# flybirdxx/ComfyUI-SDMatte

Hardware: AMD Instinct MI355X
Metric: alpha mattes/sec at 1024x1024 (higher is better)
Workload: dtype f16x3

## Files before the change

### comfyui-sdmatte_amd/csrc/k_attn.h

```cpp
#pragma once
#include "sdm_common.h"
#include "k_gemm.h"

struct AttnParams {
  const half_t* q; long q_bs; int ldq;
  const half_t* k; long k_bs; int ldk;
  const half_t* vt; long vt_bs; long vt_hs; int ldvt;
  const float* bias; long bias_bs;
  half_t* o; long o_bs; int ldo;
  int o_f32;
  int o_p3; long o_xl_off;
  long q_lo, k_lo, vt_lo;
  int Lq, Lk;
  float scale_log2e;
  const int* tiles; int tiles_bs;
  int nsplit; long part_stride; float* part_ml;
  int batch, heads, nq_blocks, q_chunks;
  int pp_flags;
  int ablate;
};

#define SDM_NEG_BIG (-1.0e30f)
#define SDM_ATTN_SKIP_MARGIN 2000.0f

SDM_DEV_INLINE void attn_store_p3(const AttnParams& p, const unsigned char* stf, int ps, int b, int q0, int head, int lane) {
  unsigned char* base = (unsigned char*)p.o;
#pragma unroll
  for (int pass = 0; pass < 4; ++pass) {
    const int row = (pass >> 1) * 16 + (lane & 15), cch = (pass & 1) * 32 + (lane >> 4) * 8;
    const f32x4 a = *(const f32x4*)(stf + row * ps + cch * 4), c = *(const f32x4*)(stf + row * ps + cch * 4 + 16);
    const float y[8] = {a[0], a[1], a[2], a[3], c[0], c[1], c[2], c[3]};
    if (q0 + row < p.Lq) p3_store8(y, base, base + p.o_xl_off, (size_t)b * p.Lq + q0 + row, p.ldo, head * 64 + cch);
  }
}

#define ATTN64_PK 144
#define ATTN64_PV 136
#define ATTN64_BUF (64 * ATTN64_PK + 64 * ATTN64_PV + 256)
#define ATTN64_SMEM (2 * ATTN64_BUF)
#define ATTN64P_BUF (2 * 64 * ATTN64_PK + 2 * 64 * ATTN64_PV + 256)
#define ATTN64P_SMEM (2 * ATTN64P_BUF)

SDM_DEV_INLINE bool attn_block_coords(const AttnParams& p, int bid, int& b, int& head, int& qblk) {
  const int units = p.batch * p.heads * p.q_chunks;
  const int upx = units / 8;
  const int qb = (p.nq_blocks + p.q_chunks - 1) / p.q_chunks;
  const int xcd = bid & 7, s = bid >> 3;
  const int unit = xcd * upx + s / qb;
  const int bh = unit / p.q_chunks, chunk = unit % p.q_chunks;
  qblk = chunk * qb + s % qb;
  b = bh / p.heads; head = bh % p.heads;
  return qblk < p.nq_blocks;
}

SDM_DEV_INLINE void attn_split_range(const AttnParams& p, const int* tl, int ntiles, int nwalk_all, int sp, int& i0, int& nwalk) {
  i0 = 0; nwalk = nwalk_all;
  if (p.nsplit <= 1) return;
  const int per = (ntiles + p.nsplit - 1) / p.nsplit, t0 = sp * per, t1 = (t0 + per < ntiles) ? t0 + per : ntiles;
  if (!tl) { i0 = t0 < ntiles ? t0 : ntiles; nwalk = t1 > i0 ? t1 - i0 : 0; return; }
// ... 40 lines not shown
  i32x8 q8p[2];
#pragma unroll
  for (int qt = 0; qt < QT; ++qt) {
    int qrow = q0 + qt * 32 + l31;
    if (qrow > p.Lq - 1) qrow = p.Lq - 1;
    const half_t* qp = p.q + (size_t)b * p.q_bs + (size_t)qrow * p.ldq + head * 64 + hi * 8;
#pragma unroll
    for (int ks = 0; ks < 4; ++ks) qf[qt][ks] = *(const f16x8*)(qp + ks * 16);
    if (PREC && !F8Q) {
#pragma unroll
      for (int ks = 0; ks < 4; ++ks) qfl[PREC ? qt : 0][ks] = *(const f16x8*)(qp + p.q_lo + ks * 16);
    }
    if (F8Q) {
      const half_t* qb = p.q + (size_t)b * p.q_bs + p.q_lo + (size_t)qrow * p.ldq + head * 64 + hi * 16;
#pragma unroll
      for (int m = 0; m < 2; ++m) {
        const i32x4 r0 = *(const i32x4*)(qb + m * 32), r1 = *(const i32x4*)(qb + m * 32 + 8);
        q8p[m] = i32x8{r0[1], r0[0], r0[3], r0[2], r1[1], r1[0], r1[3], r1[2]};
      }
    }
    if (p.scale_log2e != 1.0f && !F8Q) {
#pragma unroll
      for (int ks = 0; ks < 4; ++ks)
#pragma unroll
        for (int j = 0; j < 8; ++j) {
          if (PREC) {
            const float qs = ((float)qf[qt][ks][j] + (float)qfl[PREC ? qt : 0][ks][j]) * p.scale_log2e;
            const half_t h = (half_t)qs;
            qf[qt][ks][j] = h;
            qfl[PREC ? qt : 0][ks][j] = (half_t)(qs - (float)h);
          } else {
            qf[qt][ks][j] = (half_t)((float)qf[qt][ks][j] * p.scale_log2e);
          }
        }
    }
  }
  f32x16 o[QT][2], ls[QT];
  float m_i[QT];
  float lsum = 0.0f;
#pragma unroll
  for (int qt = 0; qt < QT; ++qt) {
    m_i[qt] = SDM_NEG_BIG;
#pragma unroll
    for (int r = 0; r < 16; ++r) ls[qt][r] = 0.0f;
#pragma unroll
    for (int dt = 0; dt < 2; ++dt)
#pragma unroll
      for (int r = 0; r < 16; ++r) o[qt][dt][r] = 0.0f;
  }
  f16x8 ones;
#pragma unroll
  for (int j = 0; j < 8; ++j) ones[j] = (half_t)1.0f;

  const half_t* kbase = p.k + (size_t)b * p.k_bs + head * 64;
  const half_t* vbase = p.vt + (size_t)b * p.vt_bs + (size_t)head * p.vt_hs;
  const float* bbase = p.bias ? p.bias + (size_t)b * p.bias_bs : nullptr;
  const int ntiles = (p.Lk + 63) / 64;

  struct Raw {
    f16x8 k[VPT], v[VPT], kl[PREC ? VPT : 1], vl[PVS ? VPT : 1];
    float b;
    bool in;
  };
  constexpr bool AHEAD2 = F8Q && QT == 1 && NW == 8;
  Raw ra, rb;
  ra.b = 0.0f; ra.in = true; rb.b = 0.0f; rb.in = true;
  const float* bsrc = bbase ? bbase : (const float*)(p.k + (size_t)b * p.k_bs);
  auto prefetch = [&](int t, Raw& r) {
    const int k0 = t * 64;
#pragma unroll
    for (int i = 0; i < VPT; ++i) {
      const int v = tid + i * NTH;
      const int row = v >> 3, part = v & 7;
      int kr = k0 + row;
      if (kr > p.Lk - 1) kr = p.Lk - 1;
      r.k[i] = *(const f16x8*)(kbase + (size_t)kr * p.ldk + part * 8);
      r.v[i] = *(const f16x8*)(vbase + (size_t)row * p.ldvt + k0 + part * 8);
      if (PREC) r.kl[PREC ? i : 0] = *(const f16x8*)(kbase + p.k_lo + (size_t)kr * p.ldk + part * 8);
      if (PVS) r.vl[PVS ? i : 0] = *(const f16x8*)(vbase + p.vt_lo + (size_t)row * p.ldvt + k0 + part * 8);
    }
    int kb = k0 + (tid & 63);
    r.in = kb < p.Lk;
    if (!r.in) kb = p.Lk - 1;
    r.b = bsrc[kb];
  };
  auto stage = [&](int buf, const Raw& r) {
    unsigned char* base = smem + buf * BUF;
#pragma unroll
    for (int i = 0; i < VPT; ++i) {
      const int v = tid + i * NTH;
      const int row = v >> 3, part = v & 7;
      *(f16x8*)(base + row * PK + part * 16) = r.k[i];
      f16x4 lo, hi4;
#pragma unroll
      for (int e = 0; e < 4; ++e) { lo[e] = r.v[i][e]; hi4[e] = r.v[i][4 + e]; }
      *(f16x4*)(base + VOFF + row * PV + part * 16) = lo;
      *(f16x4*)(base + VOFF + row * PV + part * 16 + 8) = hi4;
      if (PREC) *(f16x8*)(base + KLO + row * PK + part * 16) = r.kl[PREC ? i : 0];
      if (PVS) {
#pragma unroll
        for (int e = 0; e < 4; ++e) { lo[e] = r.vl[PVS ? i : 0][e]; hi4[e] = r.vl[PVS ? i : 0][4 + e]; }
        *(f16x4*)(base + VOFF + VLO + row * PV + part * 16) = lo;
        *(f16x4*)(base + VOFF + VLO + row * PV + part * 16 + 8) = hi4;
      }
    }
    if (tid < 64) ((float*)(base + BOFF))[tid] = r.in ? (bbase ? r.b : 0.0f) : SDM_NEG_BIG;
  };
// ... 241 lines not shown
    for (int pass = 0; pass < 4; ++pass) {
      const int row = pass * 8 + (lane >> 3), part = lane & 7;
      const int qg = q0 + qt * 32 + row;
      if (qg < p.Lq)
        *(f16x8*)(p.o + (size_t)b * p.o_bs + (size_t)qg * p.ldo + head * 64 + part * 8) = *(const f16x8*)(stg + row * PK + part * 16);
    }
    SDM_WAVE_SYNC();
  }
}

#define ATTN64PIPE_SMEM (3 * ATTN64P_BUF)
#define ATTN64PIPE4_KB (2 * 64 * ATTN64_PK + 256)
#define ATTN64PIPE4_VB (64 * ATTN64_PV)
#define ATTN64PIPE4_SMEM (2 * ATTN64PIPE4_KB + 3 * ATTN64PIPE4_VB)
template <int NW>
__global__ void __launch_bounds__(64 * NW, 2) attn_d64_pipe_kernel(AttnParams p) {
  constexpr int NTH = 64 * NW, VPT = 512 / NTH;
  constexpr bool SPLITBUF = NW == 4;
  SDM_DYN_SMEM(smem);
  constexpr int PK = ATTN64_PK, PV = ATTN64_PV, BUF = ATTN64P_BUF;
  constexpr int KLO = 64 * PK, VOFF = 2 * 64 * PK, BOFF = VOFF + 64 * PV;
  auto k_of = [&](int b3, int b2) { return SPLITBUF ? smem + b2 * ATTN64PIPE4_KB : smem + b3 * BUF; };
  auto v_of = [&](int b3) { return SPLITBUF ? smem + 2 * ATTN64PIPE4_KB + b3 * ATTN64PIPE4_VB : smem + b3 * BUF + VOFF; };
  auto bias_of = [&](int b3, int b2) { return (float*)(SPLITBUF ? smem + b2 * ATTN64PIPE4_KB + 2 * 64 * PK : smem + b3 * BUF + BOFF); };
  const int tid = threadIdx.x, lane = tid & 63, wave = tid >> 6;
  const int hi = lane >> 5, l31 = lane & 31;
  int b, head, qblk;
  if (!attn_block_coords(p, blockIdx.x, b, head, qblk)) return;
  const int q0 = qblk * (32 * NW) + wave * 32;

  f16x8 qf[4];
  i32x8 q8p[2];
  {
    int qrow = q0 + l31;
    if (qrow > p.Lq - 1) qrow = p.Lq - 1;
    const half_t* qp = p.q + (size_t)b * p.q_bs + (size_t)qrow * p.ldq + head * 64 + hi * 8;
#pragma unroll
    for (int ks = 0; ks < 4; ++ks) qf[ks] = *(const f16x8*)(qp + ks * 16);
    const half_t* qb = p.q + (size_t)b * p.q_bs + p.q_lo + (size_t)qrow * p.ldq + head * 64 + hi * 16;
#pragma unroll
    for (int m = 0; m < 2; ++m) {
      const i32x4 r0 = *(const i32x4*)(qb + m * 32), r1 = *(const i32x4*)(qb + m * 32 + 8);
      q8p[m] = i32x8{r0[1], r0[0], r0[3], r0[2], r1[1], r1[0], r1[3], r1[2]};
    }
  }
  f32x16 o[2], ls;
  float m_i = SDM_NEG_BIG;
#pragma unroll
  for (int r = 0; r < 16; ++r) { ls[r] = 0.0f; o[0][r] = 0.0f; o[1][r] = 0.0f; }
  f16x8 ones;
#pragma unroll
  for (int j = 0; j < 8; ++j) ones[j] = (half_t)1.0f;

  const half_t* kbase = p.k + (size_t)b * p.k_bs + head * 64;
  const half_t* vbase = p.vt + (size_t)b * p.vt_bs + (size_t)head * p.vt_hs;
  const float* bbase = p.bias ? p.bias + (size_t)b * p.bias_bs : nullptr;
  const float* bsrc = bbase ? bbase : (const float*)(p.k + (size_t)b * p.k_bs);
  const int ntiles = (p.Lk + 63) / 64;
  const int* tl = p.tiles ? p.tiles + (size_t)b * p.tiles_bs : nullptr;
  const int sp = p.nsplit > 1 ? (int)blockIdx.y : 0;
  int i0, nwalk;
  attn_split_range(p, tl, ntiles, tl ? tl[0] : ntiles, sp, i0, nwalk);
  if (nwalk <= 0) { attn_write_empty_part(p, sp, b, head, q0, lane); return; }
  auto tile_at = [&](int i) { return tl ? tl[1 + i0 + i] : i0 + i; };

  f16x8 rk[VPT], rkl[VPT], rv[VPT];
  float rb = 0.0f;
  bool rin = true;
  auto prefetch = [&](int t) {
    const int k0 = t * 64;
#pragma unroll
    for (int i = 0; i < VPT; ++i) {
      const int v = tid + i * NTH, srow = v >> 3, spart = v & 7;
      int kr = k0 + srow;
      if (kr > p.Lk - 1) kr = p.Lk - 1;
      rk[i] = *(const f16x8*)(kbase + (size_t)kr * p.ldk + spart * 8);
      rv[i] = *(const f16x8*)(vbase + (size_t)srow * p.ldvt + k0 + spart * 8);
      rkl[i] = *(const f16x8*)(kbase + p.k_lo + (size_t)kr * p.ldk + spart * 8);
    }
    int kb = k0 + (tid & 63);
    rin = kb < p.Lk;
    if (!rin) kb = p.Lk - 1;
    rb = bsrc[kb];
  };
  auto stage = [&](int b3, int b2) {
    unsigned char* kb_ = k_of(b3, b2);
    unsigned char* vb_ = v_of(b3);
#pragma unroll
    for (int i = 0; i < VPT; ++i) {
      const int v = tid + i * NTH, srow = v >> 3, spart = v & 7;
      *(f16x8*)(kb_ + srow * PK + spart * 16) = rk[i];
      f16x4 lo, hi4;
#pragma unroll
      for (int e = 0; e < 4; ++e) { lo[e] = rv[i][e]; hi4[e] = rv[i][4 + e]; }
      *(f16x4*)(vb_ + srow * PV + spart * 16) = lo;
      *(f16x4*)(vb_ + srow * PV + spart * 16 + 8) = hi4;
      *(f16x8*)(kb_ + KLO + srow * PK + spart * 16) = rkl[i];
    }
    if (tid < 64) bias_of(b3, b2)[tid] = rin ? (bbase ? rb : 0.0f) : SDM_NEG_BIG;
  };
  auto qk = [&](int b3, int b2, f32x16 (&s)[2]) {
    const unsigned char* Ks = k_of(b3, b2);
    const float* Bs = bias_of(b3, b2);
#pragma unroll
    for (int kt = 0; kt < 2; ++kt)
#pragma unroll
      for (int g = 0; g < 4; ++g) {
// ... 99 lines not shown
#pragma unroll
      for (int e = 0; e < 4; ++e) h[e] = o[dt][4 * g + e] * inv;
      *(f32x4*)(stf + l31 * PS + (dt * 32 + 8 * g + 4 * hi) * 4) = h;
    }
  SDM_WAVE_SYNC();
  if (p.o_p3 && p.nsplit <= 1) { attn_store_p3(p, stf, PS, b, q0, head, lane); return; }
#pragma unroll
  for (int pass = 0; pass < 8; ++pass) {
    const int row = pass * 4 + (lane >> 4), part = lane & 15;
    const int qg = q0 + row;
    if (qg < p.Lq)
      *(f32x4*)(obase + (size_t)qg * p.ldo + head * 64 + part * 4) = *(const f32x4*)(stf + row * PS + part * 16);
  }
}

#define ATTN64PP_SLOT (3 * 8192 + 256)
#define ATTN64PP_SMEM (6 * ATTN64PP_SLOT)
template <int ABL = 0, int BIAS = 1, int LIST = 1, int KE = 0, int DS = 1, int OB = 1>
__global__ void __launch_bounds__(512, 2) attn_d64_pp_kernel(AttnParams p) {
  SDM_DYN_SMEM(smem);
  constexpr int SLOT = ATTN64PP_SLOT, KLO = 8192, VOFF = 16384, BOFF = 24576;
  constexpr int R = KE < 0 ? 4 : 6, D = KE < 0 ? 3 : 4;
  constexpr int NDMA = BIAS ? 4 : 3;
  const int tid = threadIdx.x, lane = tid & 63, wave = SDM_UNIFORM_I(tid >> 6);
  const int grp = wave >> 2;
  const int hi = lane >> 5, l31 = lane & 31;
  int b, head, qblk;
  if (!attn_block_coords(p, blockIdx.x, b, head, qblk)) return;
  const int q0 = qblk * 256 + wave * 32;

  f16x8 qf[4];
  i32x8 q8p[2];
  {
    int qrow = q0 + l31;
    if (qrow > p.Lq - 1) qrow = p.Lq - 1;
    const half_t* qp = p.q + (size_t)b * p.q_bs + (size_t)qrow * p.ldq + head * 64 + hi * 8;
#pragma unroll
    for (int ks = 0; ks < 4; ++ks) qf[ks] = *(const f16x8*)(qp + ks * 16);
    const half_t* qb = p.q + (size_t)b * p.q_bs + p.q_lo + (size_t)qrow * p.ldq + head * 64 + hi * 16;
#pragma unroll
    for (int m = 0; m < 2; ++m) {
      const i32x4 r0 = *(const i32x4*)(qb + m * 32), r1 = *(const i32x4*)(qb + m * 32 + 8);
      q8p[m] = i32x8{r0[1], r0[0], r0[3], r0[2], r1[1], r1[0], r1[3], r1[2]};
    }
  }
  f32x16 o[2], ls;
  float m_i = SDM_NEG_BIG;
#pragma unroll
  for (int r = 0; r < 16; ++r) { ls[r] = 0.0f; o[0][r] = 0.0f; o[1][r] = 0.0f; }
  f16x8 ones;
#pragma unroll
  for (int j = 0; j < 8; ++j) ones[j] = (half_t)1.0f;

  const half_t* kbase = p.k + (size_t)b * p.k_bs + head * 64;
  const half_t* vbase = p.vt + (size_t)b * p.vt_bs + (size_t)head * p.vt_hs;
  const int ntiles = p.Lk / 64;
  const int* tl = (LIST && p.tiles) ? p.tiles + (size_t)b * p.tiles_bs : nullptr;
  const int sp = p.nsplit > 1 ? (int)blockIdx.y : 0;
  int i0, nwalk;
  attn_split_range(p, tl, ntiles, tl ? tl[0] : ntiles, sp, i0, nwalk);
  if (nwalk <= 0) { attn_write_empty_part(p, sp, b, head, q0, lane); return; }
  const int* tlp = tl ? tl + 1 + i0 : nullptr;
  auto tile_at = [&](int i) { if (i > nwalk - 1) i = nwalk - 1; return LIST ? tlp[i] : i0 + i; };

  const sdm_rsrc rsK = sdm_make_rsrc(kbase, (unsigned int)(((size_t)(p.Lk - 1) * p.ldk + 64) * 2));
  const sdm_rsrc rsK8 = sdm_make_rsrc(kbase + p.k_lo, (unsigned int)(((size_t)(p.Lk - 1) * p.ldk + 64) * 2));
  const sdm_rsrc rsV = sdm_make_rsrc(vbase, (unsigned int)(((size_t)63 * p.ldvt + p.Lk) * 2));
  const sdm_rsrc rsB = sdm_make_rsrc(BIAS ? p.bias + (size_t)b * p.bias_bs : (const float*)kbase, (unsigned int)p.Lk * 4u);
  const int rho = 8 * wave + (lane >> 3), cpos = lane & 7;
  const int csrc = cpos ^ ((rho >> 1) & 7);
  const int rr = rho & 31;
  const int pir = (rr & 0x13) | (((rr >> 2) & 1) << 3) | (((rr >> 3) & 1) << 2);
  const unsigned int voffK = (unsigned int)(((rho & 32) + pir) * p.ldk * 2 + csrc * 16);
  const unsigned int voffV = (unsigned int)(rho * p.ldvt * 2 + csrc * 16);
  const int lr = lane & 31;
  const unsigned int voffB = (unsigned int)(((lane & 32) + ((lr & 0x13) | (((lr >> 2) & 1) << 3) | (((lr >> 3) & 1) << 2))) * 4);
  auto dma = [&](int tile, int slot, int from = 0, int to = 4) {
    if (ABL & 8) return;
    unsigned char* sb = smem + slot * SLOT + wave * 1024;
    const unsigned int k0 = (unsigned int)tile * 64u;
    int i = 0;
    if (i >= from && i < to) sdm_glds16_buf(rsV, voffV, k0 * 2u, sb + VOFF);
    ++i;
    if (BIAS) { if (i >= from && i < to) sdm_glds4_buf(rsB, voffB, k0 * 4u, smem + slot * SLOT + BOFF); ++i; }
    if (i >= from && i < to) sdm_glds16_buf(rsK8, voffK, k0 * (unsigned int)(p.ldk * 2), sb + KLO);
    ++i;
    if (i >= from && i < to) sdm_glds16_buf(rsK, voffK, k0 * (unsigned int)(p.ldk * 2), sb);
  };
  const int kxor = (l31 >> 1) & 7;
  const int kx = l31 * 128 + ((hi ^ kxor) << 4);
  const int k8x = l31 * 128 + (((2 * hi) ^ kxor) << 4);
  const int vx = l31 * 128 + ((hi ^ kxor) << 4);
  struct KFrag { f16x8 h[4]; i32x8 f8[2]; };
  auto load_bias = [&](int slot, f32x16 (&s)[2]) {
    if (!BIAS) {
#pragma unroll
      for (int kt = 0; kt < 2; ++kt)
#pragma unroll
        for (int r = 0; r < 16; ++r) s[kt][r] = 0.0f;
      return;
    }
    if (ABL & 32) return;
    const float* Bs = (const float*)(smem + slot * SLOT + BOFF);
#pragma unroll
    for (int kt = 0; kt < 2; ++kt)
#pragma unroll
      for (int g = 0; g < 4; ++g) {
// ... 554 lines not shown
```

### comfyui-sdmatte_amd/csrc/k_misc.h

```cpp
#pragma once
#include "sdm_common.h"

template <typename F>
SDM_DEV_INLINE float resize_aa_sample(F fetch, int in_h, int in_w, int out_h, int out_w, int oy, int ox) {
  const float sy = (float)in_h / (float)out_h, sx = (float)in_w / (float)out_w;
  const float supy = sy >= 1.0f ? sy : 1.0f, supx = sx >= 1.0f ? sx : 1.0f;
  const float invy = sy >= 1.0f ? 1.0f / sy : 1.0f, invx = sx >= 1.0f ? 1.0f / sx : 1.0f;
  const float cy = sy * ((float)oy + 0.5f), cx = sx * ((float)ox + 0.5f);
  int ymin = (int)(cy - supy + 0.5f); if (ymin < 0) ymin = 0;
  int ymax = (int)(cy + supy + 0.5f); if (ymax > in_h) ymax = in_h;
  int xmin = (int)(cx - supx + 0.5f); if (xmin < 0) xmin = 0;
  int xmax = (int)(cx + supx + 0.5f); if (xmax > in_w) xmax = in_w;
  float wys = 0.0f, wxs = 0.0f;
  for (int y = ymin; y < ymax; ++y) { float w = 1.0f - fabsf(((float)y - cy + 0.5f) * invy); wys += w > 0.0f ? w : 0.0f; }
  for (int x = xmin; x < xmax; ++x) { float w = 1.0f - fabsf(((float)x - cx + 0.5f) * invx); wxs += w > 0.0f ? w : 0.0f; }
  float acc = 0.0f;
  for (int y = ymin; y < ymax; ++y) {
    float wy = 1.0f - fabsf(((float)y - cy + 0.5f) * invy); wy = wy > 0.0f ? wy / wys : 0.0f;
    float row = 0.0f;
    for (int x = xmin; x < xmax; ++x) {
      float wx = 1.0f - fabsf(((float)x - cx + 0.5f) * invx); wx = wx > 0.0f ? wx / wxs : 0.0f;
      row += wx * fetch(y, x);
    }
    acc += wy * row;
// ... 65 lines not shown
  const int j = i % wk, ii = (i / wk) % hk, b = i / ((long)hk * wk);
  const float t = plane[((size_t)b * SH + (size_t)8 * s * ii) * SW + 8 * s * j];
  const float m = (t + 1.0f) / 2.0f;
  bias[i] = ((1.0f - m) * mask_value) * mult;
}

__global__ void alpha_out_kernel(const float* __restrict__ dec, float* __restrict__ alpha, long npix) {
  const long i = (long)blockIdx.x * blockDim.x + threadIdx.x;
  if (i >= npix) return;
  const f32x4 d = *(const f32x4*)(dec + (size_t)i * 4);
  float m = (d[0] + d[1] + d[2]) / 3.0f;
  m = fminf(fmaxf(m, -1.0f), 1.0f);
  alpha[i] = (m + 1.0f) / 2.0f;
}

__global__ void resize_planes_kernel(const float* __restrict__ in, float* __restrict__ out, int P, int Hin, int Win, int Hout,
                                     int Wout, int clamp01) {
  const long i = (long)blockIdx.x * blockDim.x + threadIdx.x;
  if (i >= (long)P * Hout * Wout) return;
  const int ox = i % Wout, oy = (i / Wout) % Hout, b = i / ((long)Hout * Wout);
  const float* pl = in + (size_t)b * Hin * Win;
  float x;
  if (Hin == Hout && Win == Wout) x = pl[(size_t)oy * Win + ox];
  else x = resize_aa_sample([&](int y, int xx) { return pl[(size_t)y * Win + xx]; }, Hin, Win, Hout, Wout, oy, ox);
  if (clamp01) x = fminf(fmaxf(x, 0.0f), 1.0f);
  out[i] = x;
}

__global__ void refine_compose_kernel(const float* __restrict__ img, const float* __restrict__ tri, float* __restrict__ alpha,
                                      float* __restrict__ matted, long npix, int mode, int refine, float c, float one_minus_c) {
  const long i = (long)blockIdx.x * blockDim.x + threadIdx.x;
  if (i >= npix) return;
  float a = alpha[i];
  const float t = (refine || mode == 2) ? tri[i] : 0.0f;
  if (refine) {
    const bool fg = t > c, bg = t < one_minus_c, unk = !(fg || bg);
    if (bg) a = 0.0f;
    if (fg) a = fminf(fmaxf(a * 1.2f, 0.0f), 1.0f);
    if (a < 0.3f && unk) a = 0.0f;
    alpha[i] = a;
  }
  const float r = img[i * 3 + 0], g = img[i * 3 + 1], b = img[i * 3 + 2];
  if (mode == 1) {
    f32x4 o = {r, g, b, a};
    *(f32x4*)(matted + i * 4) = o;
  } else if (mode == 2) {
    const float gate = (t > 0.2f && a > 0.1f) ? 1.0f : 0.0f;
    matted[i * 3 + 0] = r * gate; matted[i * 3 + 1] = g * gate; matted[i * 3 + 2] = b * gate;
  } else {
    matted[i * 3 + 0] = 0.0f; matted[i * 3 + 1] = 0.0f; matted[i * 3 + 2] = 0.0f;
  }
}

__global__ void split_planes_kernel(const float* __restrict__ x, half_t* __restrict__ hi, half_t* __restrict__ lo, long n, float mult, int mode) {
  const long i4 = ((long)blockIdx.x * blockDim.x + threadIdx.x) * 4;
  if (i4 >= n) return;
  f16x4 oh, ol;
  float xx[4], xl[4];
#pragma unroll
  for (int e = 0; e < 4; ++e) {
    float y = (i4 + e < n) ? x[i4 + e] * mult : 0.0f;
    if (mode == 3) y = fminf(fmaxf(y, -57344.0f), 57344.0f);
    oh[e] = (half_t)y;
    ol[e] = (half_t)(y - (float)oh[e]);
    xx[e] = y; xl[e] = (y - (float)oh[e]) * 2048.0f;
  }
  *(f16x4*)(hi + i4) = oh;
  if (mode == 3) {
    int a = SDM_CVT_PK_BF8(xx[0], xx[1], 0, false), b = SDM_CVT_PK_BF8(xl[0], xl[1], 0, false);
    a = SDM_CVT_PK_BF8(xx[2], xx[3], a, true); b = SDM_CVT_PK_BF8(xl[2], xl[3], b, true);
    u32x2 pr;
    pr[0] = (unsigned int)a; pr[1] = (unsigned int)b;
    *(u32x2*)(lo + i4) = pr;
  } else {
    *(f16x4*)(lo + i4) = ol;
  }
}

__global__ void scale_copy_kernel(const float* __restrict__ in, float* __restrict__ out, long n, float mult) {
  const long i = (long)blockIdx.x * blockDim.x + threadIdx.x;
  if (i < n) out[i] = in[i] * mult;
}

__global__ void fill_random_f16_kernel(half_t* __restrict__ p, long n, unsigned int seed, float amp) {
  for (long i = (long)blockIdx.x * blockDim.x + threadIdx.x; i < n; i += (long)gridDim.x * blockDim.x) {
    unsigned int h = (unsigned int)i * 2654435761u + seed;
    h ^= h >> 15; h *= 2246822519u; h ^= h >> 13; h *= 3266489917u; h ^= h >> 16;
    p[i] = (half_t)(((float)(h & 0xFFFF) * (1.0f / 32768.0f) - 1.0f) * amp);
  }
}
__global__ void fill_random_f32_kernel(float* __restrict__ p, long n, unsigned int seed, float amp) {
  for (long i = (long)blockIdx.x * blockDim.x + threadIdx.x; i < n; i += (long)gridDim.x * blockDim.x) {
    unsigned int h = (unsigned int)i * 2654435761u + seed;
    h ^= h >> 15; h *= 2246822519u; h ^= h >> 13; h *= 3266489917u; h ^= h >> 16;
    p[i] = ((float)(h & 0xFFFF) * (1.0f / 32768.0f) - 1.0f) * amp;
  }
}

#define SDM_CMASK_EMPTY 0xFFFFFFFFu

__global__ __launch_bounds__(256) void cmask_table_kernel(const float* __restrict__ plane, unsigned int* __restrict__ table, int n0, int H, int W) {
  SDM_SHARED unsigned int tb[4];
  const int b = blockIdx.x, tid = threadIdx.x;
  if (tid < 4) tb[tid] = SDM_CMASK_EMPTY;
  __syncthreads();
  const float* pl = plane + (size_t)b * H * W;
  for (int i = tid; i < 64 * 64; i += 256) {
    const int y = (int)(((long)(i >> 6) * H) >> 6), x = (int)(((long)(i & 63) * W) >> 6);
    const unsigned int bits = __builtin_bit_cast(unsigned int, pl[(size_t)y * W + x]);
    for (int k = 0; k < 4; ++k) {
      unsigned int cur = tb[k];
      if (cur == SDM_CMASK_EMPTY) cur = atomicCAS(&tb[k], SDM_CMASK_EMPTY, bits);
      if (cur == SDM_CMASK_EMPTY || cur == bits) break;
    }
  }
  __syncthreads();
  if (tid < 4) table[(size_t)(n0 + b) * 4 + tid] = tb[tid];
}

__global__ void cmask_init_kernel(const float* __restrict__ plane, unsigned char* __restrict__ mask, const unsigned int* __restrict__ table, int n0, int B, long HW) {
  const long i = (long)blockIdx.x * blockDim.x + threadIdx.x;
  if (i >= (long)B * HW) return;
  const int b = (int)(i / HW);
  const unsigned int bits = __builtin_bit_cast(unsigned int, plane[i]);
  const unsigned int* tb = table + (size_t)(n0 + b) * 4;
  int cls = 0;
#pragma unroll
  for (int k = 3; k >= 0; --k)
// ... 61 lines not shown
```

### comfyui-sdmatte_amd/csrc/sdm_engine.cpp

```cpp
#include "sdm_common.h"
#include "k_conv.h"
#include "k_gemm.h"
#include "k_norm.h"
#include "k_attn.h"
#include "k_misc.h"
#include "k_trimap.h"
#include "k_cclabel.h"
#include "k_foreground.h"
#include "k_guided.h"
#include "k_roi.h"
#include "k_canvas.h"
#include "k_boxes.h"
#include "../../include/sdmatte.h"

#include <algorithm>
#include <cmath>
#include <cstdio>
#include <cstdlib>
#include <cstring>
#include <atomic>
#include <map>
#include <mutex>
#include <shared_mutex>
#include <string>
#include <unordered_map>
#include <vector>

#ifdef SDM_EMU
#include <chrono>
static int dev_malloc(void** p, size_t n) { *p = aligned_alloc(256, ((n + 255) / 256) * 256 + 256); return *p ? 0 : -1; }
static void dev_free(void* p) { free(p); }
static int dev_memcpy_h2d(void* d, const void* s, size_t n, void*) { memcpy(d, s, n); return 0; }
static int dev_memcpy_d2h(void* d, const void* s, size_t n, void*) { memcpy(d, s, n); return 0; }
static int dev_memcpy_d2d(void* d, const void* s, size_t n, void*) { memcpy(d, s, n); return 0; }
static int dev_memset(void* d, int v, size_t n, void*) { memset(d, v, n); return 0; }
static int dev_sync(void*) { return 0; }
static const char* dev_errstr(int) { return "emu"; }
#define SDM_SET_SMEM(kernel, bytes) ((void)0)
#else
static int dev_malloc(void** p, size_t n) { return (int)hipMalloc(p, n); }
static void dev_free(void* p) { (void)hipFree(p); }
static int dev_memcpy_h2d(void* d, const void* s, size_t n, void* st) { return (int)hipMemcpyAsync(d, s, n, hipMemcpyHostToDevice, (hipStream_t)st); }
static int dev_memcpy_d2h(void* d, const void* s, size_t n, void* st) { return (int)hipMemcpyAsync(d, s, n, hipMemcpyDeviceToHost, (hipStream_t)st); }
static int dev_memcpy_d2d(void* d, const void* s, size_t n, void* st) { return (int)hipMemcpyAsync(d, s, n, hipMemcpyDeviceToDevice, (hipStream_t)st); }
static int dev_memset(void* d, int v, size_t n, void* st) { return (int)hipMemsetAsync(d, v, n, (hipStream_t)st); }
static int dev_sync(void* st) { return (int)hipStreamSynchronize((hipStream_t)st); }
static const char* dev_errstr(int e) { return hipGetErrorString((hipError_t)e); }
#define SDM_SET_SMEM(kernel, bytes)                                                                              \
  do {                                                                                                           \
    if ((bytes) > 48 * 1024) {                                                                                   \
      static std::atomic<unsigned long long> done_{0ull};                                                        \
      int dev_ = 0;                                                                                              \
      (void)hipGetDevice(&dev_);                                                                                 \
      const unsigned long long bit_ = 1ull << (dev_ & 63);                                                       \
      if (!(done_.load(std::memory_order_relaxed) & bit_)) {                                                     \
        const hipError_t r_ = hipFuncSetAttribute((const void*)(kernel), hipFuncAttributeMaxDynamicSharedMemorySize, (int)(bytes)); \
        if (r_ != hipSuccess) fprintf(stderr, "[sdmatte] hipFuncSetAttribute(%d bytes of LDS) failed: %s\n", (int)(bytes), hipGetErrorString(r_)); \
        else done_.fetch_or(bit_, std::memory_order_relaxed);                                                    \
      }                                                                                                          \
    }                                                                                                            \
  } while (0)
#endif

static inline int rup(int a, int b) { return ((a + b - 1) / b) * b; }
#ifdef SDM_EMU
static inline void dev_use(int) {}
#else
static inline void dev_use(int device) {
  const hipError_t r = hipSetDevice(device);
  if (r != hipSuccess) fprintf(stderr, "[sdmatte] hipSetDevice(%d) failed: %s\n", device, hipGetErrorString(r));
}
#endif
static inline size_t rupz(size_t a, size_t b) { return ((a + b - 1) / b) * b; }

struct OptEntry { const char* name; int value; int def; const char* what; };
static OptEntry g_opts[] = {
  {"conv_f8", 1, 1, "residual terms of the wide split-precision 3x3 convs on fp8 MFMAs (read when a model is built)"},
  {"gemm_f8", 1, 1, "the same for Linear / 1x1 layers with K >= gemm_f8_min_k (read when a model is built)"},
  {"gemm_f8_min_k", 1024, 1024, "smallest K of a GEMM that takes the 8-wave fp8-residual kernel"},
  {"gemm_p3", 1, 1, "transformer-block Linear layers on the plane-fed GEMM (k_gemm.h): pre-split operand planes from LayerNorm / GroupNorm / attention / GEGLU, LDS-DMA only (the W3 weight copies are built when a model is built)"},
  {"gemm_p3_tile", 0, 0, "row tile of the plane-fed GEMM: 0 by shape, 256 / 128 / 64 forced"},
  {"gemm_p3_attn", 1, 1, "d=64 attention cores write the operand planes of to_out themselves (0: fp32 result + one conversion pass)"},
  {"gemm_p3_persist", 1, 1, "plane-fed GEMM: persistent blocks that prefetch the next tile's first chunk underneath the epilogue (0: one block per tile, n > 1: a grid of n blocks - tests)"},
  {"gemm_p3_ablate", 0, 0, "bench only: 1 no MFMAs, 2 no DMAs behind the prologue, 4 no epilogue (sdm_bench_gemm_p3)"},
  {"conv_up_phase", 1, 1, "up-sampling 3x3 convs (Upsample2D) as four 2x2-tap phase convs on the plane-fed GEMM (k_gemm.h, UP): 0 off (the 3x3 kernels on the up-sampled image), 1 the launches with at least two 256-row tiles per CU (up_phase_wins: measured), 2 every eligible launch (tests).  0 / non-0 is read when a model is built: the phase matrices are a derived weight layout"},
  {"conv_epi", 4, 4, "F8 kernels' epilogue: 4 register-direct stores + residual as accumulator init, 3 residual init only, 0 LDS-staged"},
  {"conv_xtile", 1, 1, "F8 3x3: cross-tile prefetch by the producer waves"},
  {"conv_f8_tpb", 0, 0, "F8: tiles per block (0 = by queue depth)"},
  {"conv_dma", 1, 1, "3x3 stride-1 256x128 tile: weights by LDS-DMA"},
  {"conv_dma_all", 0, 0, "keep a stage-ordered weight copy for every wide 3x3 layer, not only the split-precision ones (read when a model is built)"},
  {"conv_pc", -1, -1, "producer / consumer form of the split-precision DMA kernel: -1 by channel count, 0 off, 1 on"},
  {"conv_pc_min_cin", 256, 256, "conv_pc = -1: smallest Cin that takes the producer / consumer form"},
  {"conv_db", 0, 0, "512x128 double-buffered tile where the queue is deep"},
  {"trimap_skip", 1, 1, "VAE encoder, trimap images: output tiles inside a constant region of the trimap are not multiplied (k_misc.h cmask_*; exact). 0 = every tile"},
  {"conv_band_rows", 0, 0, "tile rows per XCD band of the convs that leave constant tiles out (0 = by image height)"},
  {"trimap_skip_min_rows", 512, 512, "smallest output height at which constant tiles are left out (measured at 1024^2: the 1024- and 512-row levels gain 3.7 + 1.6 ms, the 256-row level loses 0.7: too few of its 32 x 128-pixel tiles lie inside one region)"},
  {"conv_splitk", -1, -1, "split-K of the register-staged conv / GEMM kernels: -1 by shape (few tiles, long K), 0 off, n >= 2 forced where the shape allows"},
  {"force_cfg0", 0, 0, "always the 256x128 tile for 3x3 stride 1 (tests: fused GroupNorm at tiny sizes)"},
  {"no_gn_fuse", 0, 0, "never fuse the GroupNorm apply into the consuming conv"},
  {"split_lds_pad", 0, 0, "extra dynamic LDS of the register-staged split kernels (forces one block per CU)"},
  {"attn_f8", 1, 1, "Q.K^T residual terms of the d=64 split-precision attention on fp8 MFMAs"},
  {"attn_dense", 0, 0, "walk every key tile of the trimap-biased self-attention"},
  {"attn_pv_split", 0, 0, "residual terms of P.V too (fully split attention; tests)"},
  {"attn_nw", 0, 0, "waves per d=64 attention block: 0 by launch size, 4, 8"},
  {"attn_pipe", 1, 1, "8-wave split-precision d=64 attention: two-tile software pipeline"},
  {"attn_pipe4", 1, 1, "the same pipeline for the 4-wave launches (two K / three V^T buffers)"},
  {"attn_pp", 1, 1, "split-precision d=64 attention with fp32 output as a ping-pong of the block's wave halves (attn_d64_pp_kernel, 256 query rows per block): 0 off, 1 on, 2 on without the static priority of the younger half, 3 on with per-segment priority flips"},
  {"attn_pp_min_blocks", 128, 128, "attn_pp: launches with fewer 256-row blocks than this keep the 4-wave pipelines (0 in tests: the ping-pong kernel at any size)"},
  {"attn_ksplit", 0, 0, "key split of the d=64 split-precision attention: 0 by launch size (blocks that do not fill the chip's block slots a whole number of times), 1 off, 2 / 4 forced, 3 forced on the ping-pong kernel (ignored elsewhere: those launches run unsplit)"},
  {"precise_mask", -1, -1, "stages in split precision (-1 = the config's own mask; per-stage attribution experiments; read at sdm_create)"},
#ifdef SDM_EMU
  {"emu_arena_extra", 0, 0, "emulator build only, self-test of the arena check: the launch pass of a stand-alone op allocates one block its sizing pass did not"},
#endif
};
static OptEntry* opt_find(const char* name) {
  for (auto& o : g_opts) if (name && strcmp(o.name, name) == 0) return &o;
  return nullptr;
}
static int opt(const char* name) { OptEntry* o = opt_find(name); return o ? o->value : 0; }
static std::shared_mutex g_opt_mu;
struct OptReadLock { std::shared_lock<std::shared_mutex> l; OptReadLock() : l(g_opt_mu) {} };
static std::mutex g_count_mu;
static std::map<std::string, long> g_kernel_counts;
static void count_kernel(const char* name) { std::lock_guard<std::mutex> g(g_count_mu); g_kernel_counts[name] += 1; }

template <int NTAPS, int STRIDE, int TH, int TW, int BN, int KC, int WM, int WN, int DB = 0, int GNOK = 0>
static void launch_conv_t(const ConvParams& p_in, void* stream) {
  using C = ConvCfg<NTAPS, STRIDE, TH, TW, BN, KC, WM, WN, DB>;
  ConvParams p = p_in;
  p.tiles_m = (NTAPS == 9) ? sdm_cdiv(p.Wout, TW) * sdm_cdiv(p.Hout, TH)
                           : (int)(((p.rows_per_img ? (long)p.rows_per_img : p.M) + C::BM - 1) / C::BM);
  p.tiles_n = sdm_cdiv(p.Cout_pad, BN);
  const long total_m = (long)p.tiles_m * ((NTAPS == 9 || p.rows_per_img) ? p.N : 1);
  p.xcd_chunk = (int)((total_m + 7) / 8);
  const dim3 grid((unsigned)(8L * p.xcd_chunk * p.tiles_n), (unsigned)(p.ksplit > 1 ? p.ksplit : 1), 1);
  const size_t gn_extra = (size_t)(p.C0 + p.C1) * 8;
  if constexpr (!DB) {
    if (p.w_lo) {
      using CS = ConvCfg<NTAPS, STRIDE, TH, TW, BN, KC, WM, WN, 0, 1>;
      const size_t lds_pad = (size_t)opt("split_lds_pad");
      if (GNOK && p.gn_scale) {
        auto k = conv_mfma_kernel<NTAPS, STRIDE, TH, TW, BN, KC, WM, WN, 1, 0, GNOK, 1>;
        SDM_SET_SMEM(k, 160 * 1024);
        SDM_LAUNCH(k, grid, dim3(CS::NTHREADS), (size_t)CS::SMEM + gn_extra + lds_pad, stream, p);
      } else {
        auto k = conv_mfma_kernel<NTAPS, STRIDE, TH, TW, BN, KC, WM, WN, 1, 0, 0, 1>;
        SDM_SET_SMEM(k, 160 * 1024);
        SDM_LAUNCH(k, grid, dim3(CS::NTHREADS), CS::SMEM + lds_pad, stream, p);
      }
      return;
    }
  }
  if (GNOK && p.gn_scale) {
    const size_t smem = (size_t)C::SMEM + gn_extra;
    if (p.in_f32) {
      auto k = conv_mfma_kernel<NTAPS, STRIDE, TH, TW, BN, KC, WM, WN, 1, DB, GNOK>;
      SDM_SET_SMEM(k, C::SMEM + 1024 * 8);
      SDM_LAUNCH(k, grid, dim3(C::NTHREADS), smem, stream, p);
    } else {
      auto k = conv_mfma_kernel<NTAPS, STRIDE, TH, TW, BN, KC, WM, WN, 0, DB, GNOK>;
      SDM_SET_SMEM(k, C::SMEM + 1024 * 8);
      SDM_LAUNCH(k, grid, dim3(C::NTHREADS), smem, stream, p);
// ... 316 lines not shown
  int up = 0;
  size_t wup_off = 0, wup_bytes = 0;
  unsigned char* wup = nullptr;
  int up_exp = 8;
  size_t w_bytes() const { return (size_t)Cin_pad * ntaps * Cout_pad * 2; }
  size_t b_bytes() const { return (size_t)Cout_pad * 4; }
};
static const int kSplitWeightExp = 8;

static ConvL make_layer(const std::string& name, int ntaps, int I, int O, int geglu, int split) {
  ConvL L;
  L.name = name; L.ntaps = ntaps; L.I = I; L.O = O; L.geglu = geglu;
  L.Cin_pad = rup(I, 16);
  L.Cout_pad = rup(O, geglu ? 64 : 32);
  L.split = split ? 1 : 0;
  L.w_exp = split ? kSplitWeightExp : 0;
  return L;
}

static bool layer_takes_dma3x3(const ConvL& L) { return L.ntaps == 9 && L.Cout_pad >= 128 && !L.geglu; }
static bool layer_takes_gemm_f8(const ConvL& L) {
  return L.ntaps == 1 && L.split && L.Cout_pad >= 128 && L.Cin_pad % 32 == 0 && conv_f8_enabled() && gemm_f8_enabled();
}
static bool layer_takes_w3(const ConvL& L) { return L.ntaps == 1 && L.split && L.Cin_pad % 32 == 0 && L.Cin_pad >= 32; }
static bool layer_takes_up_phase(const ConvL& L) {
  return L.ntaps == 9 && L.split && !L.geglu && L.Cin_pad % 32 == 0 && L.Cin_pad >= 32 && conv_f8_enabled() && opt("conv_up_phase") != 0;
}
static bool up_phase_wins(int N, int H, int W, int Cout_pad) {
  if (opt("conv_up_phase") >= 2) return true;
  const long tiles = (long)N * sdm_cdiv((H + 2) * (W + 2), 256) * 4 * sdm_cdiv(Cout_pad, 128);
  return tiles >= 2L * device_cus();
}
static void layer_choose_layouts(ConvL& L, bool want_dma3x3, bool want_gemm_f8, bool want_w3, bool want_up_phase = false) {
  if (want_up_phase && layer_takes_up_phase(L)) L.wup_bytes = (size_t)16 * L.Cin_pad * L.Cout_pad * 4;
  if (want_dma3x3 && layer_takes_dma3x3(L)) {
    L.wdma_bytes = L.w_bytes() * (L.split ? 2 : 1);
    L.f8 = (L.split && L.Cin_pad % 32 == 0 && conv_f8_enabled()) ? 1 : 0;
  }
  if (want_gemm_f8 && layer_takes_gemm_f8(L)) { L.wdma_bytes = L.w_bytes() * 2; L.f8 = 1; }
  if (want_w3 && layer_takes_w3(L)) L.w3_bytes = L.w_bytes() * 2;
}
struct NormL {
  int C = 0;
  size_t g_off = 0, b_off = 0;
  float* g = nullptr;
  float* b = nullptr;
};
enum SlotKind { SLOT_CONV_W, SLOT_CONV_B, SLOT_NORM_G, SLOT_NORM_B, SLOT_HOST };
struct Slot {
  int kind = 0, layer = -1, co_off = 0, ci_off = 0;
  float w_scale = 1.0f;
  std::vector<int64_t> shape;
  size_t host_off = 0;
  bool loaded = false;
};
struct ResB { int norm1 = -1, conv1 = -1, norm2 = -1, conv2 = -1, sc = -1, temb = -1, cin = 0, cout = 0; };
struct VaeAttnB { int gn = -1, qkv = -1, out = -1, C = 0; };
struct TfB { int gn, proj_in, ln1, qkv1, o1, ln2, q2, kv2, o2, ln3, ff1, ff2, proj_out, C, heads; size_t k_hoff, v_hoff; };
struct TembL { size_t w_hoff = 0, b_hoff = 0, cb_hoff = 0; int cout = 0, cout_pad = 0; float* table = nullptr; };

struct T {
  size_t off = 0, bytes = 0;
  void* p = nullptr;
  int N = 0, H = 0, W = 0, C = 0, f32 = 0;
  bool want_stats = false;
  float* stats = nullptr;
  int srows = 0;
  size_t soff = 0, sbytes = 0;
  unsigned char* cmask = nullptr;
  size_t cm_off = 0, cm_bytes = 0;
  int cm_n0 = 0;
  long rows() const { return (long)N * H * W; }
};

static const int kFmtP3 = 4;
static inline size_t fmt_bytes(int f) { return f == kFmtP3 ? 3 : (f ? 4 : 2); }
static const int kMinVariantRows = 8;
struct Variant {
  int trans = 0, kind = 0;
  std::vector<float> c;
  bool operator==(const Variant& o) const { return trans == o.trans && kind == o.kind && c == o.c; }
};

struct ProfRec { std::string name, desc; double flops, bytes;
#ifndef SDM_EMU
  hipEvent_t e0, e1;
#endif
};

struct sdm_ctx {
  sdm_config cfg;
  int device = 0;
  const unsigned char* dbg_cmask = nullptr;
  void* stream = nullptr;
  bool own_stream = false;
  std::string err;
  std::vector<ConvL> convs;
  std::vector<NormL> norms;
  std::unordered_map<std::string, Slot> slots;
  std::vector<std::string> slot_order;
  unsigned char* warena = nullptr;
  size_t warena_bytes = 0, canon_bytes = 0;
  std::vector<float> hostblob;
  int64_t n_loaded = 0, n_ignored = 0;
  std::vector<std::string> missing;
  bool finalized = false;
  void* stage = nullptr;
  size_t stage_bytes = 0;
  struct LoadSlot {
    void* host = nullptr; void* dev = nullptr; size_t cap = 0; bool busy = false;
#ifndef SDM_EMU
// ... 51 lines not shown

#define SDM_FAIL(ctx, code, ...)                       \
  do {                                                 \
    char buf_[512];                                    \
    snprintf(buf_, sizeof(buf_), __VA_ARGS__);         \
    (ctx)->err = buf_;                                 \
    return (code);                                     \
  } while (0)

#define SDM_CHECK_DEV(ctx, expr)                                                              \
  do {                                                                                        \
    int e_ = (expr);                                                                          \
    if (e_ != 0) SDM_FAIL(ctx, SDM_ERR_HIP, "%s failed: %s (%s:%d)", #expr, dev_errstr(e_), __FILE__, __LINE__); \
  } while (0)

#define TRY(x) do { int rc_ = (x); if (rc_) return rc_; } while (0)

struct Builder {
  sdm_ctx* e;
  size_t woff = 0;
  size_t doff = 0;
  int stage = 0;
  explicit Builder(sdm_ctx* c) : e(c) {}
  int conv(const std::string& name, int ntaps, int I_pad16_src, int O, int geglu = 0, int up = 0) {
    ConvL L = make_layer(name, ntaps, I_pad16_src, O, geglu, e->cfg.precise_mask & stage);
    L.stage = stage; L.up = up;
    L.w_off = woff; woff += rupz(L.w_bytes(), 256);
    L.b_off = woff; woff += rupz(L.b_bytes(), 256);
    if (L.split) { L.wlo_off = woff; woff += rupz(L.w_bytes(), 256); }
    layer_choose_layouts(L, L.split || opt("conv_dma_all") != 0, L.Cin_pad >= gemm_f8_min_k(), conv_f8_enabled() && opt("gemm_p3") != 0, up != 0);
    if (L.wdma_bytes) { L.wdma_off = doff; doff += rupz(L.wdma_bytes, 256); }
    if (L.w3_bytes) { L.w3_off = doff; doff += rupz(L.w3_bytes, 256); }
    if (L.wup_bytes) { L.wup_off = doff; doff += rupz(L.wup_bytes, 256); }
    e->convs.push_back(L);
    return (int)e->convs.size() - 1;
  }
  int norm(int C) {
    NormL n; n.C = C;
    n.g_off = woff; woff += rupz((size_t)C * 4, 256);
    n.b_off = woff; woff += rupz((size_t)C * 4, 256);
    e->norms.push_back(n);
    return (int)e->norms.size() - 1;
  }
  void slot(const std::string& key, int kind, int layer, std::vector<int64_t> shape, int co_off = 0, int ci_off = 0) {
    Slot s; s.kind = kind; s.layer = layer; s.co_off = co_off; s.ci_off = ci_off; s.shape = std::move(shape);
    if (kind == SLOT_HOST) {
      size_t n = 1; for (auto d : s.shape) n *= (size_t)d;
      s.host_off = e->hostblob.size();
      e->hostblob.resize(e->hostblob.size() + n, 0.0f);
    }
    e->slots[key] = s;
    e->slot_order.push_back(key);
  }
  int conv_named(const std::string& p, int ntaps, int I, int O, bool bias = true, int ci_off = 0, int Ipad = 0, int up = 0) {
    int id = conv(p, ntaps, Ipad ? Ipad : I, O, 0, up);
    if (ntaps == 9) slot(p + ".weight", SLOT_CONV_W, id, {O, I, 3, 3}, 0, ci_off);
    else slot(p + ".weight", SLOT_CONV_W, id, {O, I}, 0, ci_off);
    if (bias) slot(p + ".bias", SLOT_CONV_B, id, {O});
    return id;
  }
  int norm_named(const std::string& p, int C) {
    int id = norm(C);
    slot(p + ".weight", SLOT_NORM_G, id, {C});
    slot(p + ".bias", SLOT_NORM_B, id, {C});
    return id;
  }
  ResB resnet(const std::string& p, int cin, int cout, int temb_dim) {
    ResB r; r.cin = cin; r.cout = cout;
    r.norm1 = norm_named(p + ".norm1", cin);
    if (temb_dim > 0) {
      r.conv1 = conv(p + ".conv1", 9, cin, cout);
      slot(p + ".conv1.weight", SLOT_CONV_W, r.conv1, {cout, cin, 3, 3});
      TembL t; t.cout = cout; t.cout_pad = e->convs[r.conv1].Cout_pad;
      slot(p + ".conv1.bias", SLOT_HOST, -1, {cout}); t.cb_hoff = e->slots[p + ".conv1.bias"].host_off;
      slot(p + ".time_emb_proj.weight", SLOT_HOST, -1, {cout, temb_dim}); t.w_hoff = e->slots[p + ".time_emb_proj.weight"].host_off;
      slot(p + ".time_emb_proj.bias", SLOT_HOST, -1, {cout}); t.b_hoff = e->slots[p + ".time_emb_proj.bias"].host_off;
      e->tembs.push_back(t);
      r.temb = (int)e->tembs.size() - 1;
    } else {
      r.conv1 = conv_named(p + ".conv1", 9, cin, cout);
    }
    r.norm2 = norm_named(p + ".norm2", cout);
    r.conv2 = conv_named(p + ".conv2", 9, cout, cout);
    if (cin != cout) r.sc = conv_named(p + ".conv_shortcut", 1, cin, cout);
    return r;
  }
  VaeAttnB vae_attn(const std::string& p, int C) {
    const int outer = stage;
    stage = SDM_PRECISE_VAE_ATTN_LIN;
    struct Restore { int& s; int v; ~Restore() { s = v; } } restore{stage, outer};
    VaeAttnB a; a.C = C;
    a.gn = norm_named(p + ".group_norm", C);
    a.qkv = conv(p + ".qkv", 1, C, 3 * C);
    const char* nm[3] = {"to_q", "to_k", "to_v"};
    for (int i = 0; i < 3; ++i) {
      slot(p + "." + nm[i] + ".weight", SLOT_CONV_W, a.qkv, {C, C}, i * C);
      slot(p + "." + nm[i] + ".bias", SLOT_CONV_B, a.qkv, {C}, i * C);
    }
    a.out = conv_named(p + ".to_out.0", 1, C, C);
    return a;
  }
  TfB transformer(const std::string& p, int C, int heads, int ctx) {
    const int outer = stage;
    stage = SDM_PRECISE_UNET_TF;
    struct Restore { int& s; int v; ~Restore() { s = v; } } restore{stage, outer};
    TfB t; t.C = C; t.heads = heads;
    t.gn = norm_named(p + ".norm", C);
    t.proj_in = conv_named(p + ".proj_in", 1, C, C);
    const std::string b = p + ".transformer_blocks.0";
    t.ln1 = norm_named(b + ".norm1", C);
    t.ln2 = norm_named(b + ".norm2", C);
    t.ln3 = norm_named(b + ".norm3", C);
    t.qkv1 = conv(b + ".attn1.qkv", 1, C, 3 * C);
    slot(b + ".attn1.to_q.weight", SLOT_CONV_W, t.qkv1, {C, C}, 0);
    slot(b + ".attn1.to_k.weight", SLOT_CONV_W, t.qkv1, {C, C}, C);
    slot(b + ".attn1.to_v.weight", SLOT_CONV_W, t.qkv1, {C, C}, 2 * C);
    t.o1 = conv_named(b + ".attn1.to_out.0", 1, C, C);
    t.q2 = conv_named(b + ".attn2.to_q", 1, C, C, false);
    e->slots[b + ".attn1.to_q.weight"].w_scale = e->slots[b + ".attn2.to_q.weight"].w_scale = 0.125f * SDM_LOG2E;
    t.kv2 = conv(b + ".attn2.kv_folded", 9, 16, 2 * C);
    slot(b + ".attn2.to_k.weight", SLOT_HOST, -1, {C, ctx}); t.k_hoff = e->slots[b + ".attn2.to_k.weight"].host_off;
    slot(b + ".attn2.to_v.weight", SLOT_HOST, -1, {C, ctx}); t.v_hoff = e->slots[b + ".attn2.to_v.weight"].host_off;
    t.o2 = conv_named(b + ".attn2.to_out.0", 1, C, C);
    t.ff1 = conv(b + ".ff.net.0.proj", 1, C, 8 * C, 1);
    slot(b + ".ff.net.0.proj.weight", SLOT_CONV_W, t.ff1, {8 * C, C});
    slot(b + ".ff.net.0.proj.bias", SLOT_CONV_B, t.ff1, {8 * C});
    t.ff2 = conv_named(b + ".ff.net.2", 1, 4 * C, C);
    t.proj_out = conv_named(p + ".proj_out", 1, C, C);
    return t;
  }
};

static std::string S(int i) { return std::to_string(i); }

static void build_model(sdm_ctx* e) {
  Builder B(e);
  const sdm_config& c = e->cfg;
  const int* vc = c.vae_channels;
  const int lc = 4;
  B.stage = SDM_PRECISE_VAE_ENC;
  e->enc_conv_in = B.conv_named("vae.encoder.conv_in", 9, 3, vc[0]);
  int cprev = vc[0];
  e->enc_res.resize(4);
  for (int i = 0; i < 4; ++i) {
    for (int j = 0; j < c.vae_layers_per_block; ++j)
      e->enc_res[i].push_back(B.resnet("vae.encoder.down_blocks." + S(i) + ".resnets." + S(j), j == 0 ? cprev : vc[i], vc[i], 0));
    cprev = vc[i];
    if (i < 3) e->enc_down.push_back(B.conv_named("vae.encoder.down_blocks." + S(i) + ".downsamplers.0.conv", 9, vc[i], vc[i]));
  }
  const int cm = vc[3];
  e->enc_mid0 = B.resnet("vae.encoder.mid_block.resnets.0", cm, cm, 0);
  e->enc_attn = B.vae_attn("vae.encoder.mid_block.attentions.0", cm);
  e->enc_mid1 = B.resnet("vae.encoder.mid_block.resnets.1", cm, cm, 0);
  e->enc_norm_out = B.norm_named("vae.encoder.conv_norm_out", cm);
  e->enc_conv_out = B.conv_named("vae.encoder.conv_out", 9, cm, 2 * lc);
  e->quant = B.conv_named("vae.quant_conv", 1, 2 * lc, 2 * lc);
  B.stage = SDM_PRECISE_VAE_DEC;
  e->post_quant = B.conv_named("vae.post_quant_conv", 1, lc, lc);
  e->dec_conv_in = B.conv_named("vae.decoder.conv_in", 9, lc, cm);
  e->dec_mid0 = B.resnet("vae.decoder.mid_block.resnets.0", cm, cm, 0);
  e->dec_attn = B.vae_attn("vae.decoder.mid_block.attentions.0", cm);
  e->dec_mid1 = B.resnet("vae.decoder.mid_block.resnets.1", cm, cm, 0);
  e->dec_res.resize(4);
  cprev = vc[3];
  for (int i = 0; i < 4; ++i) {
    const int co = vc[3 - i];
    for (int j = 0; j < c.vae_layers_per_block + 1; ++j)
      e->dec_res[i].push_back(B.resnet("vae.decoder.up_blocks." + S(i) + ".resnets." + S(j), j == 0 ? cprev : co, co, 0));
    cprev = co;
    if (i < 3) e->dec_up.push_back(B.conv_named("vae.decoder.up_blocks." + S(i) + ".upsamplers.0.conv", 9, co, co, true, 0, 0, 1));
  }
  e->dec_norm_out = B.norm_named("vae.decoder.conv_norm_out", vc[0]);
  e->dec_conv_out = B.conv_named("vae.decoder.conv_out", 9, vc[0], 3);
  B.stage = SDM_PRECISE_UNET_RES;
  const int* uc = c.unet_channels;
  const int te = uc[0] * 4, ctx = c.cross_attention_dim;
// ... 316 lines not shown
    const int pc_opt = opt("conv_pc"), pc_min_cin = opt("conv_pc_min_cin");
    if (p.w_dma && L.split) p.pc = pc_opt >= 0 ? (pc_opt == 1) : (L.Cin_pad >= pc_min_cin);
    if (p.w_dma && L.f8) {
      if (p.C1 > 0 && (p.C0 % 32)) { p.w_dma = nullptr; p.pc = 0; }
      else p.f8 = 1;
    }
    if (L.ntaps == 1 && L.f8 && L.w_dma && cfg == 4 && p.in_f32 && gemm_f8_enabled()) { p.w_dma = L.w_dma; p.f8 = 1; }
    if (p.f8) { p.f8_sa = 127 - 11; p.f8_sb = 127 - L.f8_exp; p.acc_scale = 1.0f; }
  }
  int ksplit = 1;
  if (!p.w_dma && !L.geglu && p.out_f32 <= 1 && (L.ntaps == 9 || p.M == (long)p.N * p.Hout * p.Wout)) ksplit = conv_pick_ksplit(L.ntaps, a.stride, cfg, p);
  T ws; ws.bytes = 0;
  const int sk_bpi = sdm_cdiv(p.Hout * p.Wout, kSplitKRows);
  if (ksplit > 1 && (size_t)ksplit * p.M * p.Cout_pad >= (1ull << 31)) ksplit = 1;
  if (a.out->want_stats) {
    if (L.geglu || a.out_ch_off || p.out_f32 >= 2) SDM_FAIL(e, SDM_ERR_INVALID, "conv %s: fused statistics unsupported with this epilogue", L.name.c_str());
    const ConvCfgInfo& ci = conv_cfg_table(L.ntaps, a.stride)[cfg];
    const long tiles = (L.ntaps == 9) ? (long)sdm_cdiv(p.Hout, ci.TH) * sdm_cdiv(p.Wout, ci.TW)
                                      : ((long)p.Hout * p.Wout + ci.TH * ci.TW - 1) / (ci.TH * ci.TW);
    a.out->srows = ksplit > 1 ? sk_bpi : (int)(tiles * ci.WM);
    T sb = talloc(e, 1, 1, 1, (int)((size_t)p.N * a.out->srows * a.out->C * 2), 1);
    a.out->soff = sb.off; a.out->sbytes = sb.bytes; a.out->stats = (float*)sb.p;
    p.stats = a.out->stats;
  }
  if (ksplit > 1) ws = talloc(e, 1, 1, 1, (int)((size_t)ksplit * p.M * p.Cout_pad), 1);
  const bool cm_prop = a.in0->cm_bytes != 0 && !a.in1 && L.ntaps == 9 && !a.up && opt("trimap_skip") != 0 && p.Hout >= opt("trimap_skip_min_rows");
  bool cm_skip = false;
  T cm_flag, cm_rep;
  const int cm_tiles = sdm_cdiv(p.Hout, 8) * sdm_cdiv(p.Wout, 32);
  if (cm_prop) {
    T mb = talloc(e, 1, 1, 1, (int)(((size_t)p.N * p.Hout * p.Wout + 3) / 4), 1);
    a.out->cmask = (unsigned char*)mb.p; a.out->cm_off = mb.off; a.out->cm_bytes = mb.bytes; a.out->cm_n0 = a.in0->cm_n0;
    cm_skip = p.f8 && p.w_dma && cfg == 0 && a.stride == 1 && p.Hout % 8 == 0 && p.Wout % 32 == 0 && p.out_f32 == 1 && !L.geglu && p.out_scale == 1.0f &&
              p.Cout_valid == p.Cout_pad && p.Cout_pad % 128 == 0 && p.Cout_store == p.Cout_pad && p.out_ch_off == 0 && (!p.res || p.res_f32) && ksplit == 1;
    if (cm_skip) {
      cm_flag = talloc(e, 1, 1, 1, (p.N * cm_tiles + 3) / 4, 1);
      cm_rep = talloc(e, 1, 1, 1, p.N * 8, 1);
      p.tile_flag = (const unsigned char*)cm_flag.p; p.tile_rep = (const int*)cm_rep.p;
    }
  }
  if (e->dry) { if (ksplit > 1) tfree(e, ws); if (cm_skip) { tfree(e, cm_rep); tfree(e, cm_flag); } return 0; }
  const double flops = 2.0 * (double)p.M * L.O * L.I * L.ntaps;
  const double bytes = (double)a.in0->rows() * L.Cin_pad * (p.in_f32 ? 4 : 2) + (double)p.M * p.Cout_valid * (p.out_f32 ? 4 : 2) +
                       (double)L.Cin_pad * L.ntaps * L.Cout_pad * 2 + (a.res ? (double)p.M * p.Cout_valid * (p.res_f32 ? 4 : 2) : 0.0);
  if (e->prof_on) {
    char d[256];
    snprintf(d, sizeof(d), "%s N=%d Hout=%d Wout=%d Cin=%d Cout=%d s=%d up=%d f32in=%d cfg=%d", L.name.c_str(), p.N, p.Hout, p.Wout, L.Cin_pad, L.O, a.stride,
             a.up, p.in_f32, cfg);
    const bool thin = (L.ntaps == 9) && (L.I <= 16 || L.O <= 16);
    prof_begin(e, L.ntaps == 9 ? (thin ? "conv3x3_thin" : "conv3x3_mfma") : "gemm_mfma", flops, bytes, d);
  } else {
    prof_begin(e, "conv", flops, bytes);
  }
  int rc = 0;
  if (L.ntaps == 1 && p.stats && p.N > 1) p.rows_per_img = p.Hout * p.Wout;
  if (cm_prop) {
    const int n0 = a.in0->cm_n0;
    if (cm_skip) {
      SDM_CHECK_DEV(e, dev_memset(cm_rep.p, 0x7f, (size_t)p.N * 8 * 4, e->stream));
      if (n0 > 0) SDM_CHECK_DEV(e, dev_memset(cm_flag.p, 0, (size_t)n0 * cm_tiles, e->stream));
    }
    SDM_LAUNCH(cmask_conv_kernel, dim3((unsigned)cm_tiles, (unsigned)(p.N - n0), 1), dim3(256), 0, e->stream, (const unsigned char*)a.in0->cmask, a.in0->H, a.in0->W, a.out->cmask,
               p.Hout, p.Wout, a.stride, p.pad_t, p.pad_l, cm_skip ? (unsigned char*)cm_flag.p : (unsigned char*)nullptr, cm_skip ? (int*)cm_rep.p : (int*)nullptr, n0);
    if (cm_skip) count_kernel("conv3x3_f8_const_tiles");
  }
  if (ksplit > 1) {
    count_kernel(L.ntaps == 9 ? "conv3x3_splitk" : "gemm_splitk");
    rc = launch_conv_splitk(L.ntaps, a.stride, cfg, p, ksplit, (float*)ws.p, e->stream);
    tfree(e, ws);
  } else {
    rc = launch_conv(L.ntaps, a.stride, cfg, p, e->stream);
  }
  if (cm_skip) {
    if (rc == 0) SDM_LAUNCH(const_tile_fill_kernel, dim3((unsigned)cm_tiles, (unsigned)(p.N - a.in0->cm_n0), 1), dim3(256), 0, e->stream, (float*)p.out, p.Cout_store, p.Hout, p.Wout,
                            p.tile_flag, p.tile_rep, p.stats, 2, a.in0->cm_n0);
    tfree(e, cm_rep); tfree(e, cm_flag);
  }
  if (rc != 0) SDM_FAIL(e, SDM_ERR_INVALID, "conv %s: bad cfg", L.name.c_str());
#ifndef SDM_EMU
  { const hipError_t le = hipGetLastError(); if (le != hipSuccess) SDM_FAIL(e, SDM_ERR_HIP, "conv %s: launch failed: %s", L.name.c_str(), hipGetErrorString(le)); }
#endif
  prof_end(e);
  return 0;
}

struct GnGeometry { int threads, ppb, nb, slots; };
static GnGeometry gn_geometry(int C, int N, int HW) {
  GnGeometry g;
  const int CV = C / 8;
  g.slots = std::max(1, 256 / CV);
  g.threads = rup(CV * g.slots, 64);
  g.ppb = rup(std::max(g.slots * 8, sdm_cdiv(HW, 2048 / std::max(1, N))), g.slots);
  g.nb = sdm_cdiv(HW, g.ppb);
  return g;
}

static int gn_scale_shift(sdm_ctx* e, const void* in0, const void* in1, int C0, int C1, int in_f32, int N, int HW, int groups, const float* gamma,
                          const float* beta, float eps, const float* st0, int rows0, const float* st1, int rows1, bool have_stats, T* scratch,
                          float** scale_out, float** shift_out) {
  const int C = C0 + C1;
  if (C % 8 || (C / groups) * groups != C || C0 % 8) SDM_FAIL(e, SDM_ERR_INVALID, "groupnorm: bad channels %d+%d", C0, C1);
  const size_t sum_bytes = (size_t)N * std::max(groups, C) * 16;
  *scratch = talloc(e, 1, 1, 1, (int)((sum_bytes + (size_t)N * C * 8 + 3) / 4), 1);
  *scale_out = nullptr; *shift_out = nullptr;
  if (e->dry) return 0;
  double* sums = (double*)scratch->p;
// ... 18 lines not shown
  return 0;
}

static int op_groupnorm_raw(sdm_ctx* e, const void* in0, const void* in1, int C0, int C1, int in_f32, int N, int HW, int groups,
                            const float* gamma, const float* beta, float eps, int silu, void* out, int out_f32, const float* st0 = nullptr,
                            int rows0 = 0, const float* st1 = nullptr, int rows1 = 0, bool have_stats = false) {
  const int C = C0 + C1;
  T scratch; float* scale; float* shift;
  TRY(gn_scale_shift(e, in0, in1, C0, C1, in_f32, N, HW, groups, gamma, beta, eps, st0, rows0, st1, rows1, have_stats, &scratch, &scale, &shift));
  if (!e->dry) {
    GnSrc s; s.in0 = in0; s.in1 = in1; s.C0 = C0; s.C1 = C1; s.in_f32 = in_f32; s.HW = HW;
    const GnGeometry g = gn_geometry(C, N, HW);
    prof_begin(e, "gn_apply", 0, (double)N * HW * C * (in_f32 ? 4 : 2) + (double)N * HW * C * (double)fmt_bytes(out_f32));
    if (out_f32 == kFmtP3)
      SDM_LAUNCH(gn_apply_p3_kernel, dim3((unsigned)(((long)N * HW + 15) / 16)), dim3(256), 0, e->stream, s, (const float*)scale, (const float*)shift, (unsigned char*)out,
                 silu, (long)N * HW);
    else
    SDM_LAUNCH(gn_apply_kernel, dim3(g.nb, N), dim3(g.threads), 0, e->stream, s, (const float*)scale, (const float*)shift, out, out_f32, silu, g.ppb);
    prof_end(e);
  }
  tfree(e, scratch);
  return 0;
}

static int op_gn(sdm_ctx* e, const NormL& n, const T& x, const T* x2, int silu, float eps, T* out, int out_fmt = -1) {
  const int C = x.C + (x2 ? x2->C : 0);
  if (C != n.C) SDM_FAIL(e, SDM_ERR_INVALID, "groupnorm: C %d != %d", C, n.C);
  *out = talloc(e, x.N, x.H, x.W, C, out_fmt >= 0 ? out_fmt : e->act_f32);
  const bool hs = x.sbytes && (!x2 || x2->sbytes);
  return op_groupnorm_raw(e, x.p, x2 ? x2->p : nullptr, x.C, x2 ? x2->C : 0, x.f32, x.N, x.H * x.W, e->cfg.groups, n.g, n.b, eps, silu,
                          out->p, out->f32, x.stats, x.srows, x2 ? x2->stats : nullptr, x2 ? x2->srows : 0, hs);
}

static int op_ln(sdm_ctx* e, const NormL& n, const T& x, float eps, T* out, int out_fmt = -1) {
  if (x.C != n.C || x.C % 64 || x.C > 64 * SDM_LN_MAXV) SDM_FAIL(e, SDM_ERR_INVALID, "layernorm: unsupported C %d", x.C);
  *out = talloc(e, x.N, x.H, x.W, x.C, out_fmt >= 0 ? out_fmt : e->act_f32);
  if (e->dry) return 0;
  const long rows = x.rows();
  if (out->f32 == kFmtP3) {
    if (x.f32 != 1 || x.C > 128 * SDM_LNP_MAXI) SDM_FAIL(e, SDM_ERR_INVALID, "layernorm (P3): fp32 input, C <= %d expected", 128 * SDM_LNP_MAXI);
    prof_begin(e, "layernorm", 0, (double)rows * x.C * 7);
    SDM_LAUNCH(layernorm_p3_kernel, dim3((unsigned)((rows + 15) / 16)), dim3(256), 0, e->stream, (const float*)x.p, (const float*)n.g, (const float*)n.b,
               (unsigned char*)out->p, rows, x.C, eps);
    prof_end(e);
    return 0;
  }
  prof_begin(e, "layernorm", 0, (double)rows * x.C * ((x.f32 ? 4 : 2) + (out->f32 ? 4 : 2)));
  SDM_LAUNCH(layernorm_kernel, dim3((unsigned)((rows + 3) / 4)), dim3(256), 0, e->stream, (const void*)x.p, x.f32, (const float*)n.g,
             (const float*)n.b, out->p, out->f32, rows, x.C, eps);
  prof_end(e);
  return 0;
}

struct AttnPrec { int prec = 0; long q_lo = 0, k_lo = 0, v_lo = 0; int out_f32 = 0; int out_p3 = 0; bool has_bias = false, has_tiles = false; };

enum AttnKernel { kAttnPP, kAttnPPBias, kAttnPPTiles, kAttnPipe8, kAttnPipe4, kAttnP3W8, kAttnP3W4, kAttnP1W8, kAttnP1W4, kAttnP2W8, kAttnP2W4,
                  kAttnF16W8, kAttnF16W4, kAttnD512 };
struct AttnPlan {
  AttnKernel kernel;
  const char* spec_counter;
  const char* combine_counter;
  int qrows;
  unsigned nblk;
  int nsplit;
  bool walk_tiles, own_list;
  bool pv_split;
  int pp_flags;
};
struct AttnKernelInfo { const char* counter; int threads; size_t smem; void (*launch)(const AttnKernelInfo&, const AttnPlan&, const AttnParams&, void*); };
template <auto K, int LDS_LIMIT = 160 * 1024>
static void attn_launch_t(const AttnKernelInfo& ki, const AttnPlan& pl, const AttnParams& p, void* stream) {
  if constexpr (LDS_LIMIT > 0) SDM_SET_SMEM(K, LDS_LIMIT);
  SDM_LAUNCH(K, dim3(pl.nblk, (unsigned)pl.nsplit, 1), dim3(ki.threads), ki.smem, stream, p);
}
static const AttnKernelInfo kAttnKernels[] = {
  {"attn_d64_pp", 512, ATTN64PP_SMEM, attn_launch_t<attn_d64_pp_kernel<0, 0, 0>>},
  {"attn_d64_pp", 512, ATTN64PP_SMEM, attn_launch_t<attn_d64_pp_kernel<0, 1, 0>>},
  {"attn_d64_pp", 512, ATTN64PP_SMEM, attn_launch_t<attn_d64_pp_kernel<0, 1, 1>>},
  {"attn_d64_pipe<8>", 512, ATTN64PIPE_SMEM, attn_launch_t<attn_d64_pipe_kernel<8>>},
  {"attn_d64_pipe<4>", 256, ATTN64PIPE4_SMEM, attn_launch_t<attn_d64_pipe_kernel<4>>},
  {"attn_d64<prec3,8>", 512, ATTN64P_SMEM, attn_launch_t<attn_d64_kernel<1, 3, 8>>},
  {"attn_d64<prec3,4>", 256, ATTN64P_SMEM, attn_launch_t<attn_d64_kernel<1, 3, 4>>},
  {"attn_d64<prec1,8>", 512, ATTN64P_SMEM, attn_launch_t<attn_d64_kernel<1, 1, 8>>},
  {"attn_d64<prec1,4>", 256, ATTN64P_SMEM, attn_launch_t<attn_d64_kernel<1, 1, 4>>},
  {"attn_d64<prec2,8>", 512, ATTN64P_SMEM, attn_launch_t<attn_d64_kernel<1, 2, 8>>},
  {"attn_d64<prec2,4>", 256, ATTN64P_SMEM, attn_launch_t<attn_d64_kernel<1, 2, 4>>},
  {"attn_d64<fp16,8>", 512, ATTN64P_SMEM, attn_launch_t<attn_d64_kernel<1, 0, 8>>},
  {"attn_d64<fp16,4>", 256, ATTN64_SMEM, attn_launch_t<attn_d64_kernel<1, 0, 4>, 0>},
  {"attn_d512", 512, ATTN512P_SMEM, attn_launch_t<attn_d512_kernel<0>, ATTN512P_SMEM>},
};
static AttnPlan attn_plan(int B, int heads, int Lq, int Lk, int D, int prec, int out_f32, bool has_bias, bool has_tiles, int cus) {
  AttnPlan pl;
  memset(&pl, 0, sizeof(pl));
  pl.nsplit = 1;
  bool nw8 = true, pp = false;
  if (D != 64) {
    pl.kernel = kAttnD512; pl.qrows = 128;
  } else {
    pl.walk_tiles = has_bias && opt("attn_dense") == 0;
    pl.own_list = pl.walk_tiles && !has_tiles;
    pl.pv_split = prec == 1 && opt("attn_pv_split") != 0;
    const int force_nw = opt("attn_nw");
    const long blocks256 = (long)B * heads * sdm_cdiv(Lq, 256);
    pp = prec == 2 && out_f32 && opt("attn_pp") != 0 && !force_nw && Lk % 64 == 0 &&
         blocks256 >= opt("attn_pp_min_blocks");
    nw8 = pp || (force_nw ? (force_nw == 8) : (prec && blocks256 >= 1024));
    pl.qrows = nw8 ? 256 : 128;
    if (prec == 2) {
      const bool pipe = out_f32 && opt(nw8 ? "attn_pipe" : "attn_pipe4") != 0;
      if (pp) pl.kernel = pl.walk_tiles ? kAttnPPTiles : (has_bias ? kAttnPPBias : kAttnPP);
      else if (pipe) pl.kernel = nw8 ? kAttnPipe8 : kAttnPipe4;
      else pl.kernel = nw8 ? kAttnP3W8 : kAttnP3W4;
    } else if (prec) {
      pl.kernel = pl.pv_split ? (nw8 ? kAttnP1W8 : kAttnP1W4) : (nw8 ? kAttnP2W8 : kAttnP2W4);
    } else {
      pl.kernel = nw8 ? kAttnF16W8 : kAttnF16W4;
    }
    if (pp) {
      pl.spec_counter = pl.walk_tiles ? "attn_pp<0,1,1>" : (has_bias ? "attn_pp<0,1,0>" : "attn_pp<0,0,0>");
      pl.pp_flags = opt("attn_pp") == 1 ? 1 : (opt("attn_pp") == 3 ? 2 : 0);
    }
  }
  pl.nblk = (unsigned)(B * heads * 8 * sdm_cdiv(sdm_cdiv(Lq, pl.qrows), 8));
  if (D == 64 && prec && out_f32 && !pl.pv_split) {
    const long blocks = pl.nblk, slots = (long)cus * (nw8 ? 1 : 2);
    const int o = opt("attn_ksplit"), ntiles64 = sdm_cdiv(Lk, 64);
    if (o >= 2) pl.nsplit = (o == 2 || o == 4 || (o == 3 && pp)) ? o : 1;
    else if (o == 0) {
      auto rounds = [&](int s) { return (double)((blocks * s + slots - 1) / slots) / s; };
      for (int s = 2; s <= 4; ++s)
        if ((s != 3 || pp) && ntiles64 / s >= 32 && rounds(s) < 0.85 * rounds(pl.nsplit)) pl.nsplit = s;
    }
    if (pl.nsplit > 1) pl.combine_counter = pl.nsplit == 2 ? "attn_combine/n=2" : (pl.nsplit == 3 ? "attn_combine/n=3" : "attn_combine/n=4");
  }
  return pl;
}

static int op_attention_raw(sdm_ctx* e, const half_t* q, int ldq, const half_t* k, int ldk, const half_t* v, int ldv, const float* bias_l2,
                            int B, int heads, int Lq, int Lk, int D, void* out, int ldo, bool q_prescaled = false, const int* tiles = nullptr,
                            AttnPrec ap = AttnPrec()) {
  if (!(D == 64 || (D == 512 && heads == 1))) SDM_FAIL(e, SDM_ERR_INVALID, "attention: unsupported head dim %d x %d heads", D, heads);
  if ((ldq | ldk | ldv | ldo) % 8) SDM_FAIL(e, SDM_ERR_INVALID, "attention: row strides must be multiples of 8");
  if (ap.prec && D != 64) SDM_FAIL(e, SDM_ERR_INVALID, "attention: the split-precision variant exists for head dim 64 only");
  if (ap.prec == 2 && !q_prescaled) SDM_FAIL(e, SDM_ERR_INVALID, "attention: the fp8-residual form takes pre-scaled queries");
  if (!e->dry && (ap.has_bias != (bias_l2 != nullptr) || ap.has_tiles != (tiles != nullptr)))
    SDM_FAIL(e, SDM_ERR_STATE, "attention: bias / tile list do not match what the sizing pass was told");
  const AttnPlan pl = attn_plan(B, heads, Lq, Lk, D, ap.prec, ap.out_f32, ap.has_bias, ap.has_tiles, device_cus());
  const AttnKernelInfo& ki = kAttnKernels[pl.kernel];
  const int nsplit = pl.nsplit;
  const int ldvt = rup(Lk, 64);
  T vt = talloc(e, (ap.prec ? 2 : 1) * B, heads, D, ldvt, 0);
  const int ntiles64 = sdm_cdiv(Lk, 64);
  T tl_own, part_o, part_ml;
  if (pl.own_list) tl_own = talloc(e, B, 1, 1, ntiles64 + 1, 1);
  if (nsplit > 1) {
    part_o = talloc(e, nsplit * B, Lq, 1, ldo, 1);
    part_ml = talloc(e, nsplit * B, heads, Lq, 2, 1);
  }
  if (!e->dry) {
    if (pl.own_list) {
      SDM_LAUNCH(attn_active_tiles_kernel, dim3(B), dim3(256), 0, e->stream, bias_l2, Lk, ntiles64, (int*)tl_own.p, ntiles64 + 1, SDM_ATTN_SKIP_MARGIN);
      tiles = (const int*)tl_own.p;
    }
    if (!pl.walk_tiles) tiles = nullptr;
    const long vt_hs = (long)D * ldvt, vt_bs = (long)heads * vt_hs;
    prof_begin(e, "transpose_v", 0, (double)B * Lk * heads * D * 4);
    SDM_LAUNCH(transpose_v_kernel, dim3(ldvt / 64, heads * (D / 64), B), dim3(256), 0, e->stream, v, (long)Lk * ldv, ldv, (half_t*)vt.p, vt_bs,
               vt_hs, ldvt, Lk, D);
    if (pl.pv_split)
      SDM_LAUNCH(transpose_v_kernel, dim3(ldvt / 64, heads * (D / 64), B), dim3(256), 0, e->stream, v + ap.v_lo, (long)Lk * ldv, ldv,
                 (half_t*)vt.p + (size_t)B * vt_bs, vt_bs, vt_hs, ldvt, Lk, D);
    prof_end(e);
    AttnParams p;
    memset(&p, 0, sizeof(p));
    p.q = q; p.q_bs = (long)Lq * ldq; p.ldq = ldq;
    p.k = k; p.k_bs = (long)Lk * ldk; p.ldk = ldk;
    p.vt = (const half_t*)vt.p; p.vt_bs = vt_bs; p.vt_hs = vt_hs; p.ldvt = ldvt;
    p.bias = bias_l2; p.bias_bs = Lk;
    p.tiles = tiles; p.tiles_bs = ntiles64 + 1;
    p.o = (half_t*)out; p.o_bs = (long)Lq * ldo; p.ldo = ldo; p.o_f32 = ap.out_f32;
    if (ap.out_p3) {
      if (!ap.out_f32 || Lq % 32 || ldo % 32 || D != 64) SDM_FAIL(e, SDM_ERR_INVALID, "attention: plane output needs d = 64, Lq %% 32 == 0 and C %% 32 == 0");
      p.o_p3 = 1; p.o_xl_off = (long)(p3_rows_pad((size_t)B * Lq) * ldo * 2);
    }
    p.q_lo = ap.q_lo; p.k_lo = ap.k_lo; p.vt_lo = (long)B * vt_bs;
    p.Lq = Lq; p.Lk = Lk;
    p.scale_log2e = q_prescaled ? 1.0f : (1.0f / sqrtf((float)D)) * SDM_LOG2E;
    if (nsplit > 1) { p.nsplit = nsplit; p.o = (half_t*)part_o.p; p.part_stride = (long)B * p.o_bs; p.part_ml = (float*)part_ml.p; }
    p.batch = B; p.heads = heads; p.nq_blocks = sdm_cdiv(Lq, pl.qrows); p.q_chunks = 8;
    p.pp_flags = pl.pp_flags;
    double flops = 4.0 * B * heads * (double)Lq * Lk * D;
    const double bytes = 2.0 * B * heads * D * (2.0 * Lq + 2.0 * Lk);
    std::string adesc = "B=" + std::to_string(B) + " h=" + std::to_string(heads) + " Lq=" + std::to_string(Lq) + " Lk=" + std::to_string(Lk);
    if (e->prof_on && tiles) {
      std::vector<int> hl((size_t)B * (ntiles64 + 1));
      (void)dev_sync(e->stream);
      (void)dev_memcpy_d2h(hl.data(), tiles, hl.size() * sizeof(int), e->stream);
      (void)dev_sync(e->stream);
      long act = 0;
      for (int bi = 0; bi < B; ++bi) act += hl[(size_t)bi * (ntiles64 + 1)];
      const double frac = (double)act / ((double)B * ntiles64);
      flops *= frac;
      char fb[48];
      snprintf(fb, sizeof(fb), " active_key_tiles=%.3f", frac);
      adesc += fb;
    }
    if (D == 64) {
      prof_begin(e, "attn_d64", flops, bytes, adesc);
      count_kernel(ki.counter);
      if (pl.spec_counter) count_kernel(pl.spec_counter);
      ki.launch(ki, pl, p, e->stream);
      if (nsplit > 1) {
        count_kernel("attn_combine");
        count_kernel(pl.combine_counter);
        if (ap.out_p3) count_kernel("attn_combine_p3");
        const long nthr = (long)B * Lq * heads * 16;
        if (ap.out_p3)
          SDM_LAUNCH(attn_combine_p3_kernel, dim3((unsigned)((nthr / 2 + 255) / 256)), dim3(256), 0, e->stream, (const float*)part_o.p, (const float*)part_ml.p,
                     (unsigned char*)out, (long)(p3_rows_pad((size_t)B * Lq) * ldo * 2), nsplit, (long)B * (long)Lq * ldo, B, heads, Lq, (long)Lq * ldo, ldo);
        else
        SDM_LAUNCH(attn_combine_kernel, dim3((unsigned)((nthr + 255) / 256)), dim3(256), 0, e->stream, (const float*)part_o.p, (const float*)part_ml.p, (float*)out,
                   nsplit, (long)B * (long)Lq * ldo, B, heads, Lq, (long)Lq * ldo, ldo);
      }
      prof_end(e);
    } else {
      prof_begin(e, "attn_d512", flops, bytes);
      ki.launch(ki, pl, p, e->stream);
      prof_end(e);
    }
  }
  if (nsplit > 1) { tfree(e, part_ml); tfree(e, part_o); }
  if (pl.own_list) tfree(e, tl_own);
  tfree(e, vt);
  return 0;
}


static int conv_simple(sdm_ctx* e, int layer, const T& in, T* out, int Cout_store, int out_f32, int stride = 1, int pad_mode = 0, int up = 0,
                       const T* res = nullptr, float scale = 1.0f, bool want_stats = false, int lo_cols = -1) {
  const ConvL& L = e->convs[layer];
  int Ho = in.H << up, Wo = in.W << up;
  if (stride == 2) { Ho /= 2; Wo /= 2; }
  *out = talloc(e, in.N, Ho, Wo, Cout_store, out_f32);
  if (want_stats) TRY(tstats(e, *out));
  ConvArgs a; a.in0 = &in; a.out = out; a.stride = stride; a.pad_mode = pad_mode; a.up = up; a.res = res; a.out_scale = scale; a.lo_cols = lo_cols;
  return op_conv(e, L, a);
}

static int gn_conv(sdm_ctx* e, const NormL& n, const ConvL& L, const T& x, const T* x2, int silu, float eps, ConvArgs a) {
  const int C = x.C + (x2 ? x2->C : 0);
  if (C != n.C) SDM_FAIL(e, SDM_ERR_INVALID, "groupnorm: C %d != %d", C, n.C);
  int cfg = -1;
  if (!opt("no_gn_fuse") && L.ntaps == 9 && a.stride == 1 && C <= 1024 && C == L.Cin_pad) {
    ConvParams p;
    memset(&p, 0, sizeof(p));
    conv_shape_params(p, L, x, x2, *a.out, a.stride);
    cfg = conv_pick_cfg(L.ntaps, a.stride, p);
  }
  if (cfg == 0 || cfg == 4 || cfg == 5) {
    const bool hs = x.sbytes && (!x2 || x2->sbytes);
    T scratch; float* scale; float* shift;
    TRY(gn_scale_shift(e, x.p, x2 ? x2->p : nullptr, x.C, x2 ? x2->C : 0, x.f32, x.N, x.H * x.W, e->cfg.groups, n.g, n.b, eps, x.stats, x.srows,
                       x2 ? x2->stats : nullptr, x2 ? x2->srows : 0, hs, &scratch, &scale, &shift));
    a.in0 = &x; a.in1 = x2;
    a.gn_scale = e->dry ? (const float*)16 : scale; a.gn_shift = shift; a.gn_silu = silu;
    a.force_cfg = cfg;
    int rc = op_conv(e, L, a);
    tfree(e, scratch);
    return rc;
  }
  T h;
  TRY(op_gn(e, n, x, x2, silu, eps, &h));
  a.in0 = &h; a.in1 = nullptr;
  int rc = op_conv(e, L, a);
  tfree(e, h);
  return rc;
}

static int resblock(sdm_ctx* e, const ResB& r, const T& x, const T* x2, float eps, T* out) {
  const int sf = e->cfg.stream_f32;
  T h1 = talloc(e, x.N, x.H, x.W, r.cout, e->act_f32);
  TRY(tstats(e, h1));
  {
    ConvArgs a; a.out = &h1;
    if (r.temb >= 0) { a.bias_override = e->tembs[r.temb].table; a.bias_sel = e->d_bias_sel; }
    TRY(gn_conv(e, e->norms[r.norm1], e->convs[r.conv1], x, x2, 1, eps, a));
// ... 62 lines not shown
    prof_begin(e, "conv", flops, bytes);
  }
  count_kernel("gemm_p3");
  launch_gemm_p3(p, epi, e->stream);
#ifndef SDM_EMU
  { const hipError_t le = hipGetLastError(); if (le != hipSuccess) SDM_FAIL(e, SDM_ERR_HIP, "gemm %s: launch failed: %s", L.name.c_str(), hipGetErrorString(le)); }
#endif
  prof_end(e);
  return 0;
}

static int op_to_p3(sdm_ctx* e, const T& x, T* out) {
  if (x.f32 != 1 || x.C % 32) SDM_FAIL(e, SDM_ERR_INVALID, "to_p3: fp32 input with C %% 32 == 0 expected (C = %d)", x.C);
  *out = talloc(e, x.N, x.H, x.W, x.C, kFmtP3);
  if (e->dry) return 0;
  const long units = ((x.rows() + 31) / 32) * (x.C / 32);
  prof_begin(e, "to_p3", 0, (double)x.rows() * x.C * 7);
  SDM_LAUNCH(to_p3_kernel, dim3((unsigned)std::min<long>((units + 3) / 4, 1 << 20)), dim3(256), 0, e->stream, (const float*)x.p, (unsigned char*)out->p, x.rows(), x.C);
  prof_end(e);
  return 0;
}

static int linear(sdm_ctx* e, int layer, const T& in, T* out, int Cout, int out_f32, const T* res = nullptr, bool want_stats = false, int lo_cols = -1) {
  *out = talloc(e, in.N, in.H, in.W, Cout, out_f32);
  if (want_stats) TRY(tstats(e, *out));
  if (in.f32 == kFmtP3) return op_gemm_p3(e, e->convs[layer], in, out, res, lo_cols);
  ConvArgs a; a.in0 = &in; a.out = out; a.res = res; a.lo_cols = lo_cols;
  return op_conv(e, e->convs[layer], a);
}

static int vae_attention(sdm_ctx* e, const VaeAttnB& a, const T& x, T* out) {
  T hn, qkv, ao;
  const int pa = ((e->cfg.precise_mask & SDM_PRECISE_UNET_ATTN) && a.C == 64) ? 1 : 0;
  const int pf = pa ? 2 : 0;
  const bool need_vlo = pf == 2 && opt("attn_pv_split") != 0;
  const int L = x.H * x.W;
  const bool p3 = pf == 0 && e->cfg.stream_f32 == 1 && L % 32 == 0 && a.C % 32 == 0 && p3_ok(e, e->convs[a.qkv]) && p3_ok(e, e->convs[a.out]);
  TRY(op_gn(e, e->norms[a.gn], x, nullptr, 0, e->cfg.vae_eps, &hn, p3 ? kFmtP3 : -1));
  TRY(linear(e, a.qkv, hn, &qkv, 3 * a.C, pf, nullptr, false, need_vlo ? -1 : 2 * a.C));
  tfree(e, hn);
  ao = talloc(e, x.N, x.H, x.W, a.C, e->act_f32);
  const half_t* q = (const half_t*)qkv.p;
  AttnPrec ap; ap.out_f32 = ao.f32; ap.prec = pa ? pf - 1 : 0;
  ap.q_lo = ap.k_lo = ap.v_lo = (long)qkv.rows() * qkv.C;
  TRY(op_attention_raw(e, q, 3 * a.C, q ? q + a.C : nullptr, 3 * a.C, q ? q + 2 * a.C : nullptr, 3 * a.C, nullptr, x.N, 1, L, L, a.C,
                       ao.p, a.C, false, nullptr, ap));
  tfree(e, qkv);
  if (p3) { T ap3; TRY(op_to_p3(e, ao, &ap3)); tfree(e, ao); ao = ap3; }
  TRY(linear(e, a.out, ao, out, a.C, e->cfg.stream_f32, &x, true));
  tfree(e, ao);
  return 0;
}

static int transformer(sdm_ctx* e, const TfB& t, const T& x, const T& uin, bool masked, const float* bias, const int* tiles, T* out) {
  const int sf = e->cfg.stream_f32;
  const int C = t.C, L = x.H * x.W, L0 = uin.H * uin.W;
  T hn, h, n, qkv, ao, h2, q2, kv, f;
  const int pa = (e->cfg.precise_mask & SDM_PRECISE_UNET_ATTN) ? 1 : 0;
  const int pf = pa ? (attn_f8_enabled() ? 3 : 2) : 0;
  const bool need_vlo = pf == 2 && opt("attn_pv_split") != 0;
  bool p3 = sf == 1 && pf == 3 && C % 32 == 0;
  for (int l : {t.proj_in, t.qkv1, t.o1, t.q2, t.o2, t.ff1, t.ff2, t.proj_out}) p3 = p3 && p3_ok(e, e->convs[l]);
  const int nf = p3 ? kFmtP3 : -1;
  const bool p3a = p3 && L % 32 == 0 && opt("gemm_p3_attn") != 0;
  auto attn_out = [&](T& a) -> int {
    if (!p3 || p3a) return 0;
    T ap;
    TRY(op_to_p3(e, a, &ap));
    tfree(e, a);
    a = ap;
    return 0;
  };
  TRY(op_gn(e, e->norms[t.gn], x, nullptr, 0, e->cfg.unet_tf_gn_eps, &hn, nf));
  TRY(linear(e, t.proj_in, hn, &h, C, sf));
  tfree(e, hn);
  TRY(op_ln(e, e->norms[t.ln1], h, e->cfg.unet_ln_eps, &n, nf));
  TRY(linear(e, t.qkv1, n, &qkv, 3 * C, pf, nullptr, false, need_vlo ? -1 : 2 * C));
  tfree(e, n);
  ao = talloc(e, x.N, x.H, x.W, C, p3a ? kFmtP3 : e->act_f32);
  {
    const half_t* q = (const half_t*)qkv.p;
    AttnPrec ap; ap.prec = pa ? pf - 1 : 0; ap.out_f32 = p3a ? 1 : ao.f32; ap.out_p3 = p3a ? 1 : 0; ap.has_bias = ap.has_tiles = masked;
    ap.q_lo = ap.k_lo = ap.v_lo = (long)qkv.rows() * qkv.C;
    TRY(op_attention_raw(e, q, 3 * C, q ? q + C : nullptr, 3 * C, q ? q + 2 * C : nullptr, 3 * C, bias, x.N, t.heads, L, L, 64, ao.p, C, true, tiles, ap));
  }
  tfree(e, qkv);
  TRY(attn_out(ao));
  TRY(linear(e, t.o1, ao, &h2, C, sf, &h));
  tfree(e, ao); tfree(e, h);
  TRY(op_ln(e, e->norms[t.ln2], h2, e->cfg.unet_ln_eps, &n, nf));
  TRY(linear(e, t.q2, n, &q2, C, pf));
  tfree(e, n);
  TRY(conv_simple(e, t.kv2, uin, &kv, 2 * C, pf, 1, 0, 0, nullptr, 1.0f, false, need_vlo ? -1 : C));
  ao = talloc(e, x.N, x.H, x.W, C, p3a ? kFmtP3 : e->act_f32);
  {
    const half_t* kk = (const half_t*)kv.p;
    AttnPrec ap; ap.prec = pa ? pf - 1 : 0; ap.out_f32 = p3a ? 1 : ao.f32; ap.out_p3 = p3a ? 1 : 0;
    ap.q_lo = (long)q2.rows() * q2.C; ap.k_lo = ap.v_lo = (long)kv.rows() * kv.C;
    TRY(op_attention_raw(e, (const half_t*)q2.p, C, kk, 2 * C, kk ? kk + C : nullptr, 2 * C, nullptr, x.N, t.heads, L, L0, 64, ao.p, C, true, nullptr, ap));
  }
  tfree(e, q2); tfree(e, kv);
  TRY(attn_out(ao));
  TRY(linear(e, t.o2, ao, &h, C, sf, &h2));
  tfree(e, ao); tfree(e, h2);
  TRY(op_ln(e, e->norms[t.ln3], h, e->cfg.unet_ln_eps, &n, nf));
  TRY(linear(e, t.ff1, n, &f, 4 * C, p3 ? kFmtP3 : e->act_f32));
  tfree(e, n);
  TRY(linear(e, t.ff2, f, &h2, C, (p3 && L % 32 == 0) ? kFmtP3 : sf, &h));
  tfree(e, f); tfree(e, h);
  TRY(linear(e, t.proj_out, h2, out, C, sf, &x, true));
  tfree(e, h2);
  return 0;
}

static void sincos_embed(float t, int dim, float* out) {
  const int half = dim / 2;
  for (int i = 0; i < half; ++i) {
    const float f = expf(-logf(10000.0f) * (float)i / (float)half);
    const float a = t * f;
    out[i] = cosf(a);
    out[half + i] = sinf(a);
  }
  if (dim & 1) out[dim - 1] = 0.0f;
}
static int point_pad_len(int N, int P) {
  for (int i = N; i < P; ++i)
    if (i > 0 && P % i == 0) return i;
  return 0;
}
static void host_linear(const float* W, const float* b, const float* x, int O, int I, float* y) {
  for (int o = 0; o < O; ++o) {
    double acc = b ? (double)b[o] : 0.0;
    const float* w = W + (size_t)o * I;
    for (int i = 0; i < I; ++i) acc += (double)w[i] * (double)x[i];
    y[o] = (float)acc;
  }
}
static inline float host_silu(float x) { return x / (1.0f + expf(-x)); }

static int compute_variant_tables(sdm_ctx* e, int vidx) {
  const Variant& v = e->variants[vidx];
  const sdm_config& c = e->cfg;
  const int c0 = c.unet_channels[0], te = c0 * 4, bd = c.bbox_embeddings_input_dim;
  const float* H = e->hostblob.data();
  std::vector<float> tp(c0), t1(te), op(te), ce(bd), b1(te), aug(te), se(te);
  sincos_embed((float)v.trans, c0, tp.data());
  host_linear(H + e->h_time1w, H + e->h_time1b, tp.data(), te, c0, t1.data());
  for (auto& x : t1) x = host_silu(x);
  host_linear(H + e->h_time2w, H + e->h_time2b, t1.data(), te, te, op.data());
  if (v.kind == 0) {
    for (int k = 0; k < 4; ++k) sincos_embed(v.c[k], bd / 4, ce.data() + k * (bd / 4));
    host_linear(H + e->h_bbox1w, H + e->h_bbox1b, ce.data(), te, bd, b1.data());
    for (auto& x : b1) x = host_silu(x);
    host_linear(H + e->h_bbox2w, H + e->h_bbox2b, b1.data(), te, te, aug.data());
  } else {
    const int P = c.point_embeddings_input_dim, npad = point_pad_len((int)v.c.size(), P), ch = P / npad;
    std::vector<float> pe((size_t)P, 0.0f);
// ... 87 lines not shown
  T h, t;
  T xin = x16;
  const bool cm = plane && opt("trimap_skip") != 0 && e->act_f32 && x16.N == 2 * plane->N && plane->H == x16.H && plane->W == x16.W;
  if (cm) {
    const long hw = (long)x16.H * x16.W;
    T mb = talloc(e, 1, 1, 1, (int)(((size_t)x16.N * hw + 3) / 4), 1);
    xin.cmask = (unsigned char*)mb.p; xin.cm_off = mb.off; xin.cm_bytes = mb.bytes; xin.cm_n0 = plane->N;
    T tab = talloc(e, 1, 1, 1, x16.N * 4, 1);
    if (!e->dry) {
      SDM_LAUNCH(cmask_table_kernel, dim3((unsigned)plane->N), dim3(256), 0, e->stream, (const float*)plane->p, (unsigned int*)tab.p, plane->N, x16.H, x16.W);
      SDM_LAUNCH(cmask_init_kernel, dim3((unsigned)((plane->N * hw + 255) / 256)), dim3(256), 0, e->stream, (const float*)plane->p, xin.cmask, (const unsigned int*)tab.p,
                 plane->N, plane->N, hw);
    }
    tfree(e, tab);
  }
  TRY(conv_simple(e, e->enc_conv_in, xin, &h, e->cfg.vae_channels[0], e->cfg.stream_f32, 1, 0, 0, nullptr, 1.0f, true));
  if (cm) tfree_raw(e, xin.cm_off, xin.cm_bytes);
  for (int i = 0; i < 4; ++i) {
    for (auto& r : e->enc_res[i]) { TRY(resblock(e, r, h, nullptr, eps, &t)); tfree(e, h); h = t; }
    if (i < 3) { TRY(conv_simple(e, e->enc_down[i], h, &t, e->cfg.vae_channels[i], e->cfg.stream_f32, 2, 1, 0, nullptr, 1.0f, true)); tfree(e, h); h = t; }
  }
  TRY(resblock(e, e->enc_mid0, h, nullptr, eps, &t)); tfree(e, h); h = t;
  TRY(vae_attention(e, e->enc_attn, h, &t)); tfree(e, h); h = t;
  TRY(resblock(e, e->enc_mid1, h, nullptr, eps, &t)); tfree(e, h); h = t;
  *moments = talloc(e, h.N, h.H, h.W, 16, e->act_f32);
  { ConvArgs a; a.out = moments; TRY(gn_conv(e, e->norms[e->enc_norm_out], e->convs[e->enc_conv_out], h, nullptr, 1, eps, a)); }
  tfree(e, h);
  return 0;
}

static int vae_decode(sdm_ctx* e, const T& z, T* dec) {
  const float eps = e->cfg.vae_eps;
  T h, t;
  TRY(conv_simple(e, e->dec_conv_in, z, &h, e->cfg.vae_channels[3], e->cfg.stream_f32, 1, 0, 0, nullptr, 1.0f, true));
  TRY(resblock(e, e->dec_mid0, h, nullptr, eps, &t)); tfree(e, h); h = t;
  TRY(vae_attention(e, e->dec_attn, h, &t)); tfree(e, h); h = t;
  TRY(resblock(e, e->dec_mid1, h, nullptr, eps, &t)); tfree(e, h); h = t;
  for (int i = 0; i < 4; ++i) {
    for (auto& r : e->dec_res[i]) { TRY(resblock(e, r, h, nullptr, eps, &t)); tfree(e, h); h = t; }
    if (i < 3) { TRY(conv_simple(e, e->dec_up[i], h, &t, e->cfg.vae_channels[3 - i], e->cfg.stream_f32, 1, 0, 1, nullptr, 1.0f, true)); tfree(e, h); h = t; }
  }
  *dec = talloc(e, h.N, h.H, h.W, 4, 1);
  { ConvArgs a; a.out = dec; TRY(gn_conv(e, e->norms[e->dec_norm_out], e->convs[e->dec_conv_out], h, nullptr, 1, eps, a)); }
  tfree(e, h);
  return 0;
}

static int unet_forward(sdm_ctx* e, const T& uin, bool masked, float* const* bias_lvl, int* const* tiles_lvl, T* out) {
  const sdm_config& c = e->cfg;
  const float eps = c.unet_res_eps;
  const int sf = c.stream_f32;
  std::vector<T> skips;
  T h, t;
  TRY(conv_simple(e, e->u_conv_in, uin, &h, c.unet_channels[0], sf, 1, 0, 0, nullptr, 1.0f, true));
  skips.push_back(h);
  for (int i = 0; i < 4; ++i) {
    for (size_t j = 0; j < e->u_down_res[i].size(); ++j) {
      TRY(resblock(e, e->u_down_res[i][j], h, nullptr, eps, &t));
      if (i < 3) {
        T t2;
        TRY(transformer(e, e->u_down_tf[i][j], t, uin, masked, bias_lvl[i], tiles_lvl[i], &t2));
        tfree(e, t); t = t2;
      }
      h = t;
      skips.push_back(h);
    }
    if (i < 3) {
      TRY(conv_simple(e, e->u_down_ds[i], h, &t, c.unet_channels[i], sf, 2, 0, 0, nullptr, 1.0f, true));
      h = t;
      skips.push_back(h);
    }
  }
  TRY(resblock(e, e->u_mid0, h, nullptr, eps, &t)); h = t;
  TRY(transformer(e, e->u_midtf, h, uin, masked, bias_lvl[3], tiles_lvl[3], &t)); tfree(e, h); h = t;
  TRY(resblock(e, e->u_mid1, h, nullptr, eps, &t)); tfree(e, h); h = t;
  for (int i = 0; i < 4; ++i) {
    for (size_t j = 0; j < e->u_up_res[i].size(); ++j) {
      T s = skips.back(); skips.pop_back();
      TRY(resblock(e, e->u_up_res[i][j], h, &s, eps, &t));
      tfree(e, h); tfree(e, s); h = t;
      if (i > 0) {
        TRY(transformer(e, e->u_up_tf[i][j], h, uin, masked, bias_lvl[3 - i], tiles_lvl[3 - i], &t));
        tfree(e, h); h = t;
      }
    }
    if (i < 3) { TRY(conv_simple(e, e->u_up_us[i], h, &t, c.unet_channels[3 - i], sf, 1, 0, 1, nullptr, 1.0f, true)); tfree(e, h); h = t; }
  }
  *out = talloc(e, h.N, h.H, h.W, 16, e->act_f32);
  { ConvArgs a; a.out = out; a.out_scale = 1.0f / c.vae_scaling_factor; TRY(gn_conv(e, e->norms[e->u_norm_out], e->convs[e->u_conv_out], h, nullptr, 1, eps, a)); }
  tfree(e, h);
  return 0;
}

static int run_model(sdm_ctx* e, const T& x16, const T& plane, int B, int SH, int SW, bool use_mask, T* alpha) {
  const sdm_config& c = e->cfg;
  const int lh = SH / 8, lw = SW / 8;
  T biasbuf[4], tilebuf[4];
  float* bias_lvl[4];
  int* tiles_lvl[4];
  for (int k = 0; k < 4; ++k) {
    const int lk2 = (lh >> k) * (lw >> k), nt = sdm_cdiv(lk2, 64);
    biasbuf[k] = talloc(e, B, 1, 1, lk2, 1);
    tilebuf[k] = talloc(e, B, 1, 1, nt + 1, 1);
    bias_lvl[k] = (float*)biasbuf[k].p;
    tiles_lvl[k] = (int*)tilebuf[k].p;
    if (!e->dry && use_mask) {
      SDM_LAUNCH(mask_bias_kernel, dim3(sdm_cdiv(B * lk2, 256)), dim3(256), 0, e->stream, (const float*)plane.p, bias_lvl[k], B, SH, SW, k,
                 c.attn_mask_value, SDM_LOG2E);
      SDM_LAUNCH(attn_active_tiles_kernel, dim3(B), dim3(256), 0, e->stream, (const float*)bias_lvl[k], lk2, nt, tiles_lvl[k], nt + 1,
                 SDM_ATTN_SKIP_MARGIN);
    }
    if (!use_mask) { bias_lvl[k] = nullptr; tiles_lvl[k] = nullptr; }
  }
  T moments;
  TRY(vae_encode(e, x16, &moments, &plane));
  T uin = talloc(e, B, lh, lw, 16, e->act_f32);
  if (!e->dry) SDM_CHECK_DEV(e, dev_memset(uin.p, 0, uin.bytes, e->stream));
  for (int half = 0; half < 2; ++half) {
    T mv = moments; mv.N = B;
    if (!e->dry) mv.p = (unsigned char*)moments.p + (size_t)half * B * lh * lw * 16 * fmt_bytes(moments.f32);
    ConvArgs a; a.in0 = &mv; a.out = &uin; a.out_ch_off = half * 4; a.cout_valid = 4; a.out_scale = c.vae_scaling_factor;
    TRY(op_conv(e, e->convs[e->quant], a));
  }
  tfree(e, moments);
  T lat;
  TRY(unet_forward(e, uin, use_mask, bias_lvl, tiles_lvl, &lat));
  tfree(e, uin);
  for (int k = 3; k >= 0; --k) { tfree(e, tilebuf[k]); tfree(e, biasbuf[k]); }
  T z;
  TRY(conv_simple(e, e->post_quant, lat, &z, 16, e->act_f32)); tfree(e, lat);
  T dec;
  TRY(vae_decode(e, z, &dec)); tfree(e, z);
  *alpha = talloc(e, B, SH, SW, 1, 1);
  if (!e->dry)
    SDM_LAUNCH(alpha_out_kernel, dim3((unsigned)(((long)B * SH * SW + 255) / 256)), dim3(256), 0, e->stream, (const float*)dec.p, (float*)alpha->p,
               (long)B * SH * SW);
  tfree(e, dec);
  return 0;
}

static int trimap_check(sdm_ctx* e, int B, int H, int W, int erode_px, int dilate_px) {
  if (B <= 0 || H <= 0 || W <= 0) SDM_FAIL(e, SDM_ERR_INVALID, "trimap from mask: bad mask size %dx%dx%d", B, H, W);
  if (erode_px < 0 || erode_px > SDM_TRIMAP_MAX_RADIUS || dilate_px < 0 || dilate_px > SDM_TRIMAP_MAX_RADIUS)
// ... 348 lines not shown
  SDM_LAUNCH(pack_bias_kernel, dim3(sdm_cdiv(L.Cout_pad, 256)), dim3(256), 0, e->stream, src, L.b, n, L.Cout_pad, co_off, L.geglu);
}

int sdm_load_tensor(sdm_ctx* e, const char* name, int dtype, int ndim, const int64_t* shape, const void* host_ptr) {
  if (e) dev_use(e->device);
  if (!e || !name || !host_ptr) return SDM_ERR_INVALID;
  std::string key(name);
  static const char* legacy[4][2] = {{".query.", ".to_q."}, {".key.", ".to_k."}, {".value.", ".to_v."}, {".proj_attn.", ".to_out.0."}};
  if (key.find("mid_block.attentions.0") != std::string::npos)
    for (auto& l : legacy) { size_t pos = key.find(l[0]); if (pos != std::string::npos) key.replace(pos, strlen(l[0]), l[1]); }
  auto it = e->slots.find(key);
  if (it == e->slots.end()) { e->n_ignored++; return 0; }
  Slot& s = it->second;
  size_t n = 1, nexp = 1;
  for (int i = 0; i < ndim; ++i) n *= (size_t)shape[i];
  for (auto d : s.shape) nexp *= (size_t)d;
  bool ok = (n == nexp);
  if (ok && (s.kind == SLOT_CONV_W)) {
    ok = ndim >= 2 && shape[0] == s.shape[0] && shape[1] == s.shape[1];
  }
  if (!ok) SDM_FAIL(e, SDM_ERR_INVALID, "size mismatch for %s: checkpoint has %zu elements, model expects %zu", name, n, nexp);
  e->finalized = false;
  if (s.kind == SLOT_HOST) {
    float* dst = e->hostblob.data() + s.host_off;
    for (size_t i = 0; i < n; ++i) dst[i] = to_f32(host_ptr, dtype, i);
  } else {
    float* dsrc = nullptr;
#ifndef SDM_EMU
    sdm_ctx::LoadSlot& sl = e->load_ring[e->load_next];
    e->load_next = (e->load_next + 1) % sdm_ctx::kLoadSlots;
    if (sl.busy) { SDM_CHECK_DEV(e, (int)hipEventSynchronize(sl.done)); sl.busy = false; }
    if (sl.cap < n * 4) {
      if (sl.host) (void)hipHostFree(sl.host);
      if (sl.dev) dev_free(sl.dev);
      sl.host = sl.dev = nullptr; sl.cap = 0;
      const size_t cap = std::max(rupz(n * 4, (size_t)1 << 20), (size_t)8 << 20);
      if (hipHostMalloc(&sl.host, cap, hipHostMallocDefault) != hipSuccess || dev_malloc(&sl.dev, cap) != 0) SDM_FAIL(e, SDM_ERR_NOMEM, "weight staging alloc failed");
      sl.cap = cap;
      if (!sl.done) SDM_CHECK_DEV(e, (int)hipEventCreateWithFlags(&sl.done, hipEventDisableTiming));
    }
    float* hs = (float*)sl.host;
    if (dtype == SDM_F32) memcpy(hs, host_ptr, n * 4);
    else for (size_t i = 0; i < n; ++i) hs[i] = to_f32(host_ptr, dtype, i);
    SDM_CHECK_DEV(e, dev_memcpy_h2d(sl.dev, hs, n * 4, e->stream));
    dsrc = (float*)sl.dev;
#else
    if (ensure_buf(e, &e->stage, &e->stage_bytes, std::max(n * 4, (size_t)1 << 20)) != 0) return SDM_ERR_NOMEM;
    std::vector<float> tmp;
    const void* src = host_ptr;
    if (dtype != SDM_F32) { tmp.resize(n); for (size_t i = 0; i < n; ++i) tmp[i] = to_f32(host_ptr, dtype, i); src = tmp.data(); }
    SDM_CHECK_DEV(e, dev_memcpy_h2d(e->stage, src, n * 4, e->stream));
    dsrc = (float*)e->stage;
#endif
    if (s.kind == SLOT_CONV_W) {
      pack_layer_weight(e, e->convs[s.layer], dsrc, (int)s.shape[0], (int)s.shape[1], s.ci_off, s.co_off, s.w_scale);
    } else if (s.kind == SLOT_CONV_B) {
      pack_layer_bias(e, e->convs[s.layer], dsrc, (int)s.shape[0], s.co_off);
    } else {
      NormL& nn = e->norms[s.layer];
      SDM_CHECK_DEV(e, dev_memcpy_d2d(s.kind == SLOT_NORM_G ? nn.g : nn.b, dsrc, n * 4, e->stream));
    }
#ifndef SDM_EMU
    SDM_CHECK_DEV(e, (int)hipEventRecord(sl.done, (hipStream_t)e->stream));
    sl.busy = true;
#else
    SDM_CHECK_DEV(e, dev_sync(e->stream));
#endif
  }
  if (!s.loaded) { s.loaded = true; e->n_loaded++; }
  return 1;
}

static int fold_cross_kv(sdm_ctx* e) {
  const sdm_config& c = e->cfg;
  const int ctx = c.cross_attention_dim;
  const float* H = e->hostblob.data();
  std::vector<double> wa((size_t)36 * ctx), ba(ctx);
  for (int m = 0; m < ctx; ++m) {
    ba[m] = H[e->h_auxb + m];
    for (int j = 0; j < 36; ++j) wa[(size_t)j * ctx + m] = H[e->h_auxw + (size_t)m * 36 + j];
  }
  std::vector<const TfB*> blocks;
  for (auto& v : e->u_down_tf) for (auto& t : v) blocks.push_back(&t);
  blocks.push_back(&e->u_midtf);
  for (auto& v : e->u_up_tf) for (auto& t : v) blocks.push_back(&t);
  std::vector<float> wf, bf;
  for (const TfB* t : blocks) {
    const int C = t->C;
    ConvL& L = e->convs[t->kv2];
    wf.assign((size_t)2 * C * 36, 0.f); bf.assign((size_t)2 * C, 0.f);
    for (int o = 0; o < 2 * C; ++o) {
      const float* wrow = H + (o < C ? t->k_hoff + (size_t)o * ctx : t->v_hoff + (size_t)(o - C) * ctx);
      double b = 0.0;
      for (int m = 0; m < ctx; ++m) b += (double)wrow[m] * ba[m];
      bf[o] = (float)b;
      for (int j = 0; j < 36; ++j) {
        const double* wj = wa.data() + (size_t)j * ctx;
        double acc = 0.0;
        for (int m = 0; m < ctx; ++m) acc += (double)wrow[m] * wj[m];
        wf[(size_t)o * 36 + j] = (float)acc;
      }
    }
    if (ensure_buf(e, &e->stage, &e->stage_bytes, std::max(wf.size() * 4, (size_t)1 << 20)) != 0) return SDM_ERR_NOMEM;
    SDM_CHECK_DEV(e, dev_memset(L.w, 0, L.w_bytes(), e->stream));
    if (L.w_lo) SDM_CHECK_DEV(e, dev_memset(L.w_lo, 0, L.w_bytes(), e->stream));
    SDM_CHECK_DEV(e, dev_memcpy_h2d(e->stage, wf.data(), wf.size() * 4, e->stream));
    pack_layer_weight(e, L, (const float*)e->stage, 2 * C, 4, 4, 0, 1.0f);
    SDM_CHECK_DEV(e, dev_sync(e->stream));
    SDM_CHECK_DEV(e, dev_memcpy_h2d(e->stage, bf.data(), bf.size() * 4, e->stream));
    pack_layer_bias(e, L, (const float*)e->stage, 2 * C, 0);
    SDM_CHECK_DEV(e, dev_sync(e->stream));
  }
  return 0;
}

static int derive_layers(sdm_ctx* e, std::vector<ConvL*>& layers) {
  std::vector<ConvL*> f8;
  for (ConvL* L : layers) if ((L->w_dma && L->f8) || L->w3) f8.push_back(L);
  const size_t n_own = f8.size();
  for (ConvL* L : layers) if (L->wup) f8.push_back(L);
  if (!f8.empty()) {
    const size_t tb = rupz(f8.size() * 4, 256);
    if (ensure_buf(e, &e->stage, &e->stage_bytes, std::max(tb, (size_t)1 << 20)) != 0) return SDM_ERR_NOMEM;
    SDM_CHECK_DEV(e, dev_memset(e->stage, 0, tb, e->stream));
    for (size_t i = 0; i < f8.size(); ++i) {
      const size_t n = (size_t)f8[i]->Cin_pad * f8[i]->ntaps * f8[i]->Cout_pad;
      if (i >= n_own) {
        SDM_LAUNCH(up_phase_absmax_kernel, dim3(2048), dim3(256), 0, e->stream, (const half_t*)f8[i]->w, (const half_t*)f8[i]->w_lo, f8[i]->Cin_pad, f8[i]->Cout_pad,
                   (unsigned int*)e->stage + i);
        continue;
      }
      SDM_LAUNCH(absmax_f16_kernel, dim3((unsigned)std::min<size_t>((n + 255) / 256, 2048)), dim3(256), 0, e->stream, (const half_t*)f8[i]->w, n,
                 (unsigned int*)e->stage + i);
    }
    std::vector<float> mx(f8.size());
    SDM_CHECK_DEV(e, dev_memcpy_d2h(mx.data(), e->stage, f8.size() * 4, e->stream));
    SDM_CHECK_DEV(e, dev_sync(e->stream));
    for (size_t i = 0; i < f8.size(); ++i) {
      const float wmax = ldexpf(mx[i], -f8[i]->w_exp);
      int ex = 8;
      if (wmax > 0.0f && std::isfinite(wmax)) {
        ex = (int)floorf(log2f(448.0f / wmax));
        while (ldexpf(wmax, ex) > 448.0f) --ex;
        ex = std::max(-60, std::min(60, ex));
      }
      if (i >= n_own) f8[i]->up_exp = ex; else f8[i]->f8_exp = ex;
    }
  }
  for (ConvL* L : layers) {
    if (L->w3)
      SDM_LAUNCH(derive_gemm_w3_kernel<0>, dim3((unsigned)std::min<size_t>(((size_t)L->Cin_pad * L->Cout_pad / 4 + 255) / 256, 65535)), dim3(256), 0, e->stream,
                 (const half_t*)L->w, (const half_t*)L->w_lo, L->w3, L->Cin_pad, L->Cout_pad, ldexpf(1.0f, -L->w_exp), ldexpf(1.0f, L->f8_exp));
    if (L->wup)
      SDM_LAUNCH(derive_gemm_w3_kernel<1>, dim3((unsigned)std::min<size_t>(((size_t)L->Cin_pad * L->Cout_pad * 4 + 255) / 256, 65535)), dim3(256), 0, e->stream,
                 (const half_t*)L->w, (const half_t*)L->w_lo, L->wup, L->Cin_pad, L->Cout_pad, ldexpf(1.0f, -L->w_exp), ldexpf(1.0f, L->up_exp));
    if (!L->w_dma) continue;
    const size_t total = (size_t)L->Cin_pad * L->ntaps * L->Cout_pad;
    if (L->f8)
      SDM_LAUNCH(derive_conv_weight_f8_kernel, dim3((unsigned)std::min<size_t>((total / 4 + 255) / 256, 65535)), dim3(256), 0, e->stream,
                 (const half_t*)L->w, (const half_t*)L->w_lo, (unsigned char*)L->w_dma, L->Cin_pad, L->Cout_pad, L->ntaps, ldexpf(1.0f, -L->w_exp),
                 ldexpf(1.0f, L->f8_exp));
    else
      SDM_LAUNCH(derive_conv_weight_dma_kernel, dim3((unsigned)std::min<size_t>((total * (L->split ? 2 : 1) + 255) / 256, 65535)), dim3(256), 0, e->stream,
                 (const half_t*)L->w, (const half_t*)L->w_lo, L->w_dma, L->Cin_pad, L->Cout_pad, L->split ? 2 : 1);
// ... 688 lines not shown
```

### comfyui-sdmatte_amd/csrc/sdm_hooks.h

```cpp
#pragma once

struct DevBuf {
  void* p = nullptr;
  DevBuf() = default;
  DevBuf(DevBuf&& o) noexcept : p(o.p) { o.p = nullptr; }
  ~DevBuf() { if (p) dev_free(p); }
  int alloc(size_t n) { return dev_malloc(&p, n); }
  int alloc0(size_t n, void* stream) { const int rc = alloc(n); return rc ? rc : dev_memset(p, 0, n, stream); }
};

struct RestoreInt { int& s; int v; ~RestoreInt() { s = v; } };

struct TempLayer {
  enum { kDma = 1, kW3 = 2, kUp = 4 };
  sdm_ctx* e;
  ConvL L;
  DevBuf w, w_lo, b, w_dma, w3, wup;
  explicit TempLayer(sdm_ctx* c) : e(c) {}
  ~TempLayer() { dev_sync(e->stream); }
  int init(const char* name, int ntaps, int I, int O, int geglu, int split, int layouts, const float* wsrc, const float* bias) {
    L = make_layer(name, ntaps, I, O, geglu, split);
    layer_choose_layouts(L, layouts & kDma, layouts & kDma, layouts & kW3, layouts & kUp);
    SDM_CHECK_DEV(e, w.alloc0(L.w_bytes(), e->stream));
    SDM_CHECK_DEV(e, b.alloc0(L.b_bytes(), e->stream));
// ... 304 lines not shown
    }
    p.ablate = ablate & 255;
  }
  return time_launches(e, iters, [&]() { run(p); });
#endif
}

float sdm_bench_attn(sdm_ctx* e, int B, int heads, int Lq, int Lk, int qt, int ablate, int iters) {
  if (e) dev_use(e->device);
  if (!e) return -1.f;
#ifdef SDM_EMU
  return -1.f;
#else
  if (qt & 64) {
    const int ldvt5 = rup(Lk, 64);
    DevBuf q5, k5, v5, o5;
    if (q5.alloc((size_t)B * Lq * 512 * 2) || k5.alloc((size_t)B * Lk * 512 * 2) || v5.alloc((size_t)B * 512 * ldvt5 * 2) || o5.alloc((size_t)B * Lq * 512 * 4)) return -2.f;
    SDM_LAUNCH(fill_random_f16_kernel, dim3(4096), dim3(256), 0, e->stream, (half_t*)q5.p, (long)B * Lq * 512, 3u, 0.3f);
    SDM_LAUNCH(fill_random_f16_kernel, dim3(4096), dim3(256), 0, e->stream, (half_t*)k5.p, (long)B * Lk * 512, 7u, 0.3f);
    SDM_LAUNCH(fill_random_f16_kernel, dim3(4096), dim3(256), 0, e->stream, (half_t*)v5.p, (long)B * 512 * ldvt5, 11u, 1.0f);
    AttnParams p5;
    memset(&p5, 0, sizeof(p5));
    p5.q = (const half_t*)q5.p; p5.q_bs = (long)Lq * 512; p5.ldq = 512; p5.k = (const half_t*)k5.p; p5.k_bs = (long)Lk * 512; p5.ldk = 512;
    p5.vt = (const half_t*)v5.p; p5.vt_hs = (long)512 * ldvt5; p5.vt_bs = p5.vt_hs; p5.ldvt = ldvt5; p5.o = (half_t*)o5.p; p5.o_bs = (long)Lq * 512; p5.ldo = 512; p5.o_f32 = 1;
    p5.Lq = Lq; p5.Lk = Lk; p5.scale_log2e = 0.0441941738f * SDM_LOG2E;
    p5.batch = B; p5.heads = 1; p5.nq_blocks = sdm_cdiv(Lq, 128); p5.q_chunks = 8;
    const unsigned nb5 = (unsigned)(B * p5.q_chunks * sdm_cdiv(p5.nq_blocks, p5.q_chunks));
    return time_launches(e, iters, [&]() {
#define SDM_D512_ABL(A) case A: { auto kp = attn_d512_kernel<A>; SDM_SET_SMEM(kp, ATTN512P_SMEM); SDM_LAUNCH(kp, dim3(nb5), dim3(512), ATTN512P_SMEM, e->stream, p5); } break;
      switch (ablate) { SDM_D512_ABL(0) SDM_D512_ABL(1) SDM_D512_ABL(6) SDM_D512_ABL(7) SDM_D512_ABL(8) SDM_D512_ABL(32) SDM_D512_ABL(40) SDM_D512_ABL(41) default: break; }
#undef SDM_D512_ABL
    });
  }
  const int C = heads * 64, ldvt = rup(Lk, 64);
  const int prec = (qt & 2) ? 1 : 0, nw8 = (qt & 4) ? 1 : 0;
  DevBuf q, k, vt, o;
  if (q.alloc((size_t)B * Lq * C * 2 * (1 + prec)) || k.alloc((size_t)B * Lk * C * 2 * (1 + prec)) ||
      vt.alloc((size_t)B * heads * 64 * ldvt * 2 * (1 + prec)) || o.alloc((size_t)B * Lq * C * (prec ? 4 : 2) + 4096)) return -2.f;
  if (prec) {
    SDM_LAUNCH(fill_random_f16_kernel, dim3(4096), dim3(256), 0, e->stream, (half_t*)q.p + (size_t)B * Lq * C, (long)B * Lq * C, 13u, 0.0003f);
    SDM_LAUNCH(fill_random_f16_kernel, dim3(4096), dim3(256), 0, e->stream, (half_t*)k.p + (size_t)B * Lk * C, (long)B * Lk * C, 17u, 0.0003f);
    SDM_LAUNCH(fill_random_f16_kernel, dim3(4096), dim3(256), 0, e->stream, (half_t*)vt.p + (size_t)B * heads * 64 * ldvt, (long)B * heads * 64 * ldvt, 19u, 0.0003f);
  }
  if (prec && (qt & 16)) {
    (void)hipMemsetAsync((half_t*)q.p + (size_t)B * Lq * C, 0, (size_t)B * Lq * C * 2, (hipStream_t)e->stream);
    (void)hipMemsetAsync((half_t*)k.p + (size_t)B * Lk * C, 0, (size_t)B * Lk * C * 2, (hipStream_t)e->stream);
  }
  SDM_LAUNCH(fill_random_f16_kernel, dim3(4096), dim3(256), 0, e->stream, (half_t*)q.p, (long)B * Lq * C, 3u, 1.0f);
  SDM_LAUNCH(fill_random_f16_kernel, dim3(4096), dim3(256), 0, e->stream, (half_t*)k.p, (long)B * Lk * C, 7u, 1.0f);
  SDM_LAUNCH(fill_random_f16_kernel, dim3(4096), dim3(256), 0, e->stream, (half_t*)vt.p, (long)B * heads * 64 * ldvt, 11u, 1.0f);
  AttnParams p;
  memset(&p, 0, sizeof(p));
  p.q = (const half_t*)q.p; p.q_bs = (long)Lq * C; p.ldq = C; p.k = (const half_t*)k.p; p.k_bs = (long)Lk * C; p.ldk = C;
  p.vt = (const half_t*)vt.p; p.vt_hs = (long)64 * ldvt; p.vt_bs = heads * p.vt_hs; p.ldvt = ldvt; p.o = (half_t*)o.p; p.o_bs = (long)Lq * C; p.ldo = C;
  p.Lq = Lq; p.Lk = Lk; p.scale_log2e = 0.125f * SDM_LOG2E; p.ablate = ablate;
  if (prec) { p.q_lo = (long)B * Lq * C; p.k_lo = (long)B * Lk * C; p.vt_lo = (long)B * p.vt_bs; p.o_f32 = 1; }
  p.batch = B; p.heads = heads; p.nq_blocks = sdm_cdiv(Lq, nw8 ? 256 : 128); p.q_chunks = 8;
  const unsigned nblk = (unsigned)(B * heads * p.q_chunks * sdm_cdiv(p.nq_blocks, p.q_chunks));
  const float ms = time_launches(e, iters, [&]() {
    if (qt & 16) {
      p.pp_flags = (qt & 32) ? 0 : 1;
      p.part_ml = (float*)((unsigned char*)o.p + (size_t)B * Lq * C * 4);
      if (qt & 128) p.pp_flags |= 2;
#define SDM_PP_ABL(A) case A: { auto kp = attn_d64_pp_kernel<A, 0, 0>; SDM_SET_SMEM(kp, 160 * 1024); SDM_LAUNCH(kp, dim3(nblk), dim3(512), ATTN64PP_SMEM + 4096, e->stream, p); } break;
#define SDM_PP_DS(A, S, V) case V: { auto kp = attn_d64_pp_kernel<A, 0, 0, 0, S, 0>; SDM_SET_SMEM(kp, 160 * 1024); SDM_LAUNCH(kp, dim3(nblk), dim3(512), ATTN64PP_SMEM + 4096, e->stream, p); } break;
#define SDM_PP_KE(K, V) case V: { auto kp = attn_d64_pp_kernel<0, 0, 0, K, 1, 0>; SDM_SET_SMEM(kp, 160 * 1024); SDM_LAUNCH(kp, dim3(nblk), dim3(512), ATTN64PP_SMEM, e->stream, p); } break;
      switch (ablate) { SDM_PP_ABL(0) SDM_PP_ABL(1) SDM_PP_ABL(6) SDM_PP_ABL(7) SDM_PP_ABL(8) SDM_PP_ABL(32) SDM_PP_ABL(56) SDM_PP_ABL(63)
                        SDM_PP_KE(-1, 100) SDM_PP_KE(2, 101) SDM_PP_KE(1, 102) SDM_PP_ABL(64)
                        SDM_PP_DS(0, 0, 110) SDM_PP_DS(0, 1, 111) SDM_PP_DS(0, 2, 112) SDM_PP_DS(0, 3, 113) SDM_PP_DS(64, 0, 114) SDM_PP_DS(64, 2, 116) SDM_PP_DS(64, 3, 117) default: break; }
#undef SDM_PP_ABL
#undef SDM_PP_KE
#undef SDM_PP_DS
    }
    else if (prec && (qt & 8) && nw8) { auto kp = attn_d64_kernel<1, 2, 8>; SDM_SET_SMEM(kp, 160 * 1024); SDM_LAUNCH(kp, dim3(nblk), dim3(512), ATTN64P_SMEM, e->stream, p); }
    else if (prec && (qt & 8)) { auto kp = attn_d64_kernel<1, 2, 4>; SDM_SET_SMEM(kp, 160 * 1024); SDM_LAUNCH(kp, dim3(nblk), dim3(256), ATTN64P_SMEM, e->stream, p); }
    else if (prec && nw8) { auto kp = attn_d64_kernel<1, 1, 8>; SDM_SET_SMEM(kp, 160 * 1024); SDM_LAUNCH(kp, dim3(nblk), dim3(512), ATTN64P_SMEM, e->stream, p); }
    else if (prec) { auto kp = attn_d64_kernel<1, 1, 4>; SDM_SET_SMEM(kp, 160 * 1024); SDM_LAUNCH(kp, dim3(nblk), dim3(256), ATTN64P_SMEM, e->stream, p); }
    else if (nw8) { auto kf = attn_d64_kernel<1, 0, 8>; SDM_SET_SMEM(kf, 160 * 1024); SDM_LAUNCH(kf, dim3(nblk), dim3(512), ATTN64P_SMEM, e->stream, p); }
    else { SDM_LAUNCH((attn_d64_kernel<1, 0, 4>), dim3(nblk), dim3(256), ATTN64_SMEM, e->stream, p); }
  });
  if ((qt & 16) && (ablate == 64 || (ablate >= 114 && ablate <= 117))) {
    std::vector<unsigned long long> tr(2 * 8 * 28);
    (void)hipMemcpy(tr.data(), (unsigned char*)o.p + (size_t)B * Lq * C * 4, tr.size() * 8, hipMemcpyDeviceToHost);
    for (int g = 0; g < 2; ++g) {
      double dm = 0, sm = 0, vr = 0, wa = 0, mx = 0, wb = 0; int n = 0;
      for (int t = 5; t < 27; ++t) {
        const unsigned long long* c = &tr[(size_t)g * 224 + (size_t)t * 8];
        const unsigned long long prev3 = tr[(size_t)g * 224 + (size_t)(t - 1) * 8 + 3];
        dm += (double)(c[4] - prev3); sm += (double)(c[5] - c[4]); vr += (double)(c[0] - c[5]); wa += (double)(c[1] - c[0]); mx += (double)(c[2] - c[1]); wb += (double)(c[3] - c[2]); ++n;
      }
      fprintf(stderr, "[attn_pp trace] wave %d: DMA issue %.0f | softmax VALU %.0f | V^T reads + lgkmcnt(0) %.0f | wait at barrier %.0f | matrix segment %.0f | wait at barrier %.0f  (cycles per tile, mean of %d tiles; each stamp costs an s_memtime round trip)\n",
              g * 4, dm / n, sm / n, vr / n, wa / n, mx / n, wb / n, n);
    }
  }
  return ms;
#endif
}

int sdm_op_groupnorm(sdm_ctx* e, const void* in0, const void* in1, int C0, int C1, int in_f32, int N, int HW, int groups, const float* gamma,
                     const float* beta, float eps, int silu, void* out) {
  if (e) dev_use(e->device);
  if (!e || !in0 || !out) return SDM_ERR_INVALID;
  return run_two_pass(e, [&]() { return op_groupnorm_raw(e, in0, in1, C0, C1, in_f32, N, HW, groups, gamma, beta, eps, silu, out, 0); });
}

int sdm_op_layernorm(sdm_ctx* e, const void* x, int in_f32, long rows, int C, const float* gamma, const float* beta, float eps, void* out) {
// ... 13 lines not shown
    T b2 = talloc(e, B, 1, 1, Lk, 1);
    AttnPrec ap; ap.has_bias = bias != nullptr;
    if (bias && !e->dry) {
      SDM_LAUNCH(scale_copy_kernel, dim3(sdm_cdiv(B * Lk, 256)), dim3(256), 0, e->stream, bias, (float*)b2.p, (long)B * Lk, SDM_LOG2E);
    }
    int rc = op_attention_raw(e, (const half_t*)q, ldq, (const half_t*)k, ldk, (const half_t*)v, ldv, bias ? (const float*)b2.p : nullptr,
                              B, heads, Lq, Lk, D, (half_t*)out, ldo, false, nullptr, ap);
    tfree(e, b2);
    return rc;
  });
}

int sdm_op_attention_split(sdm_ctx* e, const float* q, const float* k, const float* v, const float* bias, int B, int heads, int Lq, int Lk, float* out) {
  return sdm_op_attention_split_ex(e, q, k, v, bias, nullptr, B, heads, Lq, Lk, 0, out, nullptr);
}

int sdm_op_attention_split_ex(sdm_ctx* e, const float* q, const float* k, const float* v, const float* bias, const int* tiles, int B, int heads, int Lq,
                              int Lk, int out_p3, float* out, void* planes) {
  if (e) dev_use(e->device);
  if (!e || !q || !k || !v || !out) return SDM_ERR_INVALID;
  if (out_p3 < 0 || out_p3 > 2 || (tiles && !bias)) SDM_FAIL(e, SDM_ERR_INVALID, "sdm_op_attention_split_ex: out_p3 0..2; a tile list needs the bias");
  const int C = heads * 64;
  const int mode = (attn_f8_enabled() && !opt("attn_pv_split")) ? 3 : 2;
  return run_two_pass(e, [&]() -> int {
    T b2 = talloc(e, B, 1, 1, Lk, 1);
    T qp = talloc(e, B, 1, Lq, C, mode), kp = talloc(e, B, 1, Lk, C, mode), vp = talloc(e, B, 1, Lk, C, mode);
    const long nq = (long)B * Lq * C, nk = (long)B * Lk * C;
    if (!e->dry) {
      if (bias) SDM_LAUNCH(scale_copy_kernel, dim3(sdm_cdiv(B * Lk, 256)), dim3(256), 0, e->stream, bias, (float*)b2.p, (long)B * Lk, SDM_LOG2E);
      SDM_LAUNCH(split_planes_kernel, dim3((unsigned)((nq / 4 + 255) / 256)), dim3(256), 0, e->stream, q, (half_t*)qp.p, (half_t*)qp.p + nq, nq, 0.125f * SDM_LOG2E, mode);
      SDM_LAUNCH(split_planes_kernel, dim3((unsigned)((nk / 4 + 255) / 256)), dim3(256), 0, e->stream, k, (half_t*)kp.p, (half_t*)kp.p + nk, nk, 1.0f, mode);
      SDM_LAUNCH(split_planes_kernel, dim3((unsigned)((nk / 4 + 255) / 256)), dim3(256), 0, e->stream, v, (half_t*)vp.p, (half_t*)vp.p + nk, nk, 1.0f, 2);
    }
    T to, pl;
    if (out_p3) to = talloc(e, B, 1, Lq, C, out_p3 == 1 ? kFmtP3 : 1);
    AttnPrec ap; ap.prec = mode - 1; ap.q_lo = nq; ap.k_lo = nk; ap.v_lo = nk; ap.out_f32 = 1; ap.out_p3 = out_p3 == 1;
    ap.has_bias = bias != nullptr; ap.has_tiles = tiles != nullptr;
    TRY(op_attention_raw(e, (const half_t*)qp.p, C, (const half_t*)kp.p, C, (const half_t*)vp.p, C, bias ? (const float*)b2.p : nullptr, B, heads, Lq, Lk, 64,
                         out_p3 ? to.p : (void*)out, C, true, tiles, ap));
    if (out_p3 == 2) TRY(op_to_p3(e, to, &pl));
    const T& p3 = out_p3 == 2 ? pl : to;
    if (out_p3 && !e->dry) {
      SDM_LAUNCH(from_p3_kernel, dim3((unsigned)std::min<long>(((long)B * Lq * C + 255) / 256, 1 << 20)), dim3(256), 0, e->stream, (const unsigned char*)p3.p, out,
                 (long)B * Lq, C);
      if (planes) SDM_CHECK_DEV(e, dev_memcpy_d2d(planes, p3.p, p3_rows_pad((size_t)B * Lq) * C * 3, e->stream));
    }
    if (out_p3 == 2) tfree(e, pl);
    if (out_p3) tfree(e, to);
    tfree(e, vp); tfree(e, kp); tfree(e, qp); tfree(e, b2);
    return 0;
  });
}

int sdm_debug_attn_plan(int B, int heads, int Lq, int Lk, int D, int prec, int out_f32, int has_bias, int has_tiles, int cus, char* kernel, int cap,
                        int* nsplit) {
  if (B < 1 || heads < 1 || Lq < 1 || Lk < 1 || cus < 1 || prec < 0 || prec > 2 || !(D == 64 || (D == 512 && heads == 1 && !prec))) return SDM_ERR_INVALID;
  OptReadLock opt_lock;
  const AttnPlan pl = attn_plan(B, heads, Lq, Lk, D, prec, out_f32, has_bias != 0, has_tiles != 0, cus);
  if (kernel && cap > 0) snprintf(kernel, (size_t)cap, "%s", kAttnKernels[pl.kernel].counter);
  if (nsplit) *nsplit = pl.nsplit;
  return SDM_OK;
}

int sdm_op_resize_aa(sdm_ctx* e, const float* in, int P, int Hin, int Win, float* out, int Hout, int Wout) {
  if (e) dev_use(e->device);
  if (!e || !in || !out) return SDM_ERR_INVALID;
  SDM_LAUNCH(resize_planes_kernel, dim3((unsigned)(((long)P * Hout * Wout + 255) / 256)), dim3(256), 0, e->stream, in, out, P, Hin, Win, Hout, Wout, 0);
  SDM_CHECK_DEV(e, dev_sync(e->stream));
  return 0;
}

int sdm_op_mask_bias(sdm_ctx* e, const float* plane, int B, int S, int level, float* out) {
  if (e) dev_use(e->device);
  if (!e || !plane || !out) return SDM_ERR_INVALID;
  const int lk = (S / 8) >> level;
  SDM_LAUNCH(mask_bias_kernel, dim3(sdm_cdiv(B * lk * lk, 256)), dim3(256), 0, e->stream, plane, out, B, S, S, level, e->cfg.attn_mask_value, 1.0f);
  SDM_CHECK_DEV(e, dev_sync(e->stream));
  return 0;
}

}
```

### comfyui-sdmatte_amd/engine.py

```python
import ctypes as C
import os

import numpy as np
import torch

from .config import SDMatteConfig

_HERE = os.path.dirname(os.path.abspath(__file__))
LIB_PATH = os.path.join(_HERE, "csrc", "libsdmatte_hip.so")

SDM_PTR_HOST, SDM_PTR_DEVICE = 0, 1
SDM_F32, SDM_F16, SDM_BF16 = 0, 1, 2
_DT = {torch.float32: SDM_F32, torch.float16: SDM_F16, torch.bfloat16: SDM_BF16}


class SdmConfig(C.Structure):
    _fields_ = [
        ("vae_channels", C.c_int32 * 4), ("vae_layers_per_block", C.c_int32),
        ("unet_channels", C.c_int32 * 4), ("unet_heads", C.c_int32 * 4), ("unet_layers_per_block", C.c_int32),
        ("cross_attention_dim", C.c_int32), ("unet_in_channels", C.c_int32), ("unet_out_channels", C.c_int32),
        ("bbox_embeddings_input_dim", C.c_int32), ("groups", C.c_int32),
        ("vae_eps", C.c_float), ("unet_res_eps", C.c_float), ("unet_tf_gn_eps", C.c_float), ("unet_ln_eps", C.c_float),
        ("vae_scaling_factor", C.c_float), ("attn_mask_value", C.c_float),
        ("stream_f32", C.c_int32), ("point_embeddings_input_dim", C.c_int32), ("precise_mask", C.c_int32), ("reserved", C.c_int32 * 5),
    ]


PRECISE_VAE_ENC, PRECISE_VAE_DEC, PRECISE_VAE_ATTN_LIN, PRECISE_UNET_RES, PRECISE_UNET_TF, PRECISE_UNET_ATTN = 1, 2, 4, 8, 16, 32
PRECISE_ALL = 63
PRECISIONS = {
    "fp16": 0,
    "fp16x3": PRECISE_ALL,
}
DEFAULT_PRECISION = os.environ.get("SDMATTE_PRECISION", "fp16x3")


def precise_mask_of(precision) -> int:
    if precision is None:
        precision = DEFAULT_PRECISION
    if isinstance(precision, int):
        return precision & PRECISE_ALL
    if precision not in PRECISIONS:
        raise ValueError(f"unknown precision {precision!r}; expected one of {sorted(PRECISIONS)} or a stage bit mask")
    return PRECISIONS[precision]


def to_c_config(cfg: SDMatteConfig, stream_f32: bool = True, precision=None) -> SdmConfig:
    c = SdmConfig()
    for i in range(4):
        c.vae_channels[i] = cfg.vae_channels[i]
        c.unet_channels[i] = cfg.unet_channels[i]
        c.unet_heads[i] = cfg.unet_heads[i]
    c.vae_layers_per_block = cfg.vae_layers_per_block
    c.unet_layers_per_block = cfg.unet_layers_per_block
    c.cross_attention_dim = cfg.cross_attention_dim
    c.unet_in_channels = cfg.unet_in_channels
    c.unet_out_channels = cfg.unet_out_channels
    c.bbox_embeddings_input_dim = cfg.bbox_embeddings_input_dim
    c.groups = cfg.unet_groups
    c.vae_eps, c.unet_res_eps = cfg.vae_eps, cfg.unet_res_eps
    c.unet_tf_gn_eps, c.unet_ln_eps = cfg.unet_tf_gn_eps, cfg.unet_ln_eps
    c.vae_scaling_factor, c.attn_mask_value = cfg.vae_scaling_factor, cfg.attn_mask_value
    c.stream_f32 = 1 if stream_f32 else 0
    c.point_embeddings_input_dim = cfg.point_embeddings_input_dim
    c.precise_mask = precise_mask_of(precision)
    return c


EXPORTS = [
    "sdm_default_config", "sdm_create", "sdm_destroy", "sdm_last_error", "sdm_load_tensor", "sdm_finalize_weights",
    "sdm_weight_stats", "sdm_missing_key", "sdm_weight_blob_bytes", "sdm_export_weight_blob", "sdm_import_weight_blob",
    "sdm_host_blob_bytes", "sdm_export_host_blob", "sdm_import_host_blob", "sdm_forward", "sdm_forward_ex", "sdm_forward_rect", "sdm_apply_matte", "sdm_apply_matte_node",
    "sdm_make_trimap", "sdm_clean_mask", "sdm_apply_matte_mask", "sdm_subject_roi", "sdm_apply_matte_roi", "sdm_subject_boxes", "sdm_apply_matte_boxes", "sdm_estimate_foreground", "sdm_refine_alpha_guided", "sdm_compose_canvas",
    "sdm_synchronize", "sdm_release_memory", "sdm_resident_bytes", "sdm_weight_bytes", "sdm_last_forward_ms", "sdm_profile_enable", "sdm_profile_count", "sdm_profile_get", "sdm_profile_dump",
    "sdm_op_conv", "sdm_op_conv_ex", "sdm_op_conv_up_stats", "sdm_op_gemm_p3", "sdm_debug_run_layer", "sdm_debug_set_input_cmask", "sdm_debug_temb_row", "sdm_conv_num_cfgs", "sdm_bench_conv", "sdm_bench_attn", "sdm_bench_gemm_p3", "sdm_op_groupnorm", "sdm_op_layernorm", "sdm_op_attention", "sdm_op_attention_split", "sdm_op_attention_split_ex", "sdm_debug_attn_plan", "sdm_op_resize_aa",
    "sdm_op_mask_bias",
    "sdm_set_option", "sdm_get_option", "sdm_reset_options", "sdm_option_name", "sdm_option_help", "sdm_kernel_counts", "sdm_kernel_counts_reset",
]


class Bindings:

    def __init__(self, cdll):
        self.dll = cdll
        vp, i32, i64, f32 = C.c_void_p, C.c_int, C.c_int64, C.c_float
        sig = {
            "sdm_default_config": (None, [C.POINTER(SdmConfig)]),
            "sdm_create": (i32, [C.POINTER(vp), i32, C.POINTER(SdmConfig)]),
            "sdm_destroy": (None, [vp]),
            "sdm_last_error": (C.c_char_p, [vp]),
            "sdm_load_tensor": (i32, [vp, C.c_char_p, i32, i32, C.POINTER(i64), vp]),
            "sdm_finalize_weights": (i32, [vp]),
            "sdm_weight_stats": (i32, [vp, C.POINTER(i64), C.POINTER(i64), C.POINTER(i64)]),
            "sdm_missing_key": (C.c_char_p, [vp, i64]),
            "sdm_weight_blob_bytes": (i64, [vp]),
            "sdm_export_weight_blob": (i32, [vp, vp]),
            "sdm_import_weight_blob": (i32, [vp, vp]),
            "sdm_host_blob_bytes": (i64, [vp]),
            "sdm_export_host_blob": (i32, [vp, vp]),
            "sdm_import_host_blob": (i32, [vp, vp]),
            "sdm_forward": (i32, [vp, vp, vp, i32, i32, vp, vp, vp, i32, vp]),
            "sdm_forward_ex": (i32, [vp, vp, vp, i32, i32, vp, vp, i32, i32, i32, vp, i32, vp]),
            "sdm_forward_rect": (i32, [vp, vp, vp, i32, i32, i32, vp, vp, i32, i32, i32, vp, i32, vp]),
            "sdm_apply_matte": (i32, [vp, vp, vp, i32, i32, i32, i32, i32, vp, i32, vp]),
            "sdm_apply_matte_node": (i32, [vp, vp, vp, i32, i32, i32, i32, i32, i32, i32, i32, i32, C.c_double, vp, vp, i32, vp]),
            "sdm_make_trimap": (i32, [vp, vp, i32, i32, i32, f32, i32, i32, vp, i32, vp]),
            "sdm_clean_mask": (i32, [vp, vp, i32, i32, i32, f32, i32, i32, i32, i32, vp, vp, i32, vp]),
            "sdm_apply_matte_mask": (i32, [vp, vp, vp, i32, i32, i32, i32, i32, i32, i32, f32, i32, i32, i32, i32, C.c_double, vp, vp, vp, i32, vp]),
            "sdm_subject_roi": (i32, [vp, vp, i32, i32, i32, f32, i32, i32, i32, vp, i32, vp]),
            "sdm_apply_matte_roi": (i32, [vp, vp, vp, i32, i32, i32, i32, i32, i32, f32, i32, i32, f32, i32, i32, i32, i32, i32, C.c_double, vp, vp, vp, vp, i32, vp]),
            "sdm_subject_boxes": (i32, [vp, vp, i32, i32, i32, f32, i32, i32, i32, i32, i32, vp, vp, i32, vp]),
            "sdm_apply_matte_boxes": (i32, [vp, vp, vp, i32, i32, i32, i32, i32, vp, i32, i32, i32, C.c_double, vp, vp, i32, vp]),
            "sdm_estimate_foreground": (i32, [vp, vp, vp, i32, i32, i32, f32, f32, i32, i32, vp, i32, vp, i32, vp]),
            "sdm_refine_alpha_guided": (i32, [vp, vp, vp, i32, i32, i32, i32, i32, f32, vp, i32, vp]),
            "sdm_compose_canvas": (i32, [vp, vp, vp, i32, i32, i32, f32, i32, i32, i32, i32, i32, vp, vp, i32, f32, f32, i32, i32, vp, i32, vp, i32, vp]),
            "sdm_synchronize": (i32, [vp]),
            "sdm_release_memory": (i32, [vp]),
            "sdm_resident_bytes": (i64, [vp]),
            "sdm_weight_bytes": (i64, [vp]),
            "sdm_last_forward_ms": (f32, [vp]),
            "sdm_profile_enable": (i32, [vp, i32]),
            "sdm_profile_count": (i32, [vp]),
            "sdm_profile_dump": (C.c_char_p, [vp]),
            "sdm_profile_get": (i32, [vp, i32, C.POINTER(C.c_char_p), C.POINTER(f32), C.POINTER(i64), C.POINTER(C.c_double),
                                      C.POINTER(C.c_double)]),
            "sdm_op_conv": (i32, [vp, vp, vp, i32, i32, i32, i32, i32, i32, i32, i32, i32, i32, vp, vp, i32, vp, i32, vp, i32, i32,
                                  f32, i32]),
            "sdm_op_conv_ex": (i32, [vp, vp, vp, i32, i32, i32, i32, i32, i32, i32, i32, i32, i32, vp, vp, i32, vp, i32, vp, i32, i32,
                                     f32, i32, i32, vp, vp, f32, i32, i32]),
            "sdm_op_gemm_p3": (i32, [vp, vp, i32, i32, i32, i32, vp, vp, i32, i32, vp, vp, vp, f32, i32, vp, vp, C.POINTER(i32)]),
            "sdm_op_conv_up_stats": (i32, [vp, vp, i32, i32, i32, i32, vp, vp, i32, vp, vp, C.POINTER(i32)]),
            "sdm_debug_run_layer": (i32, [vp, C.c_char_p, vp, i32, i32, i32, vp, i32]),
            "sdm_debug_set_input_cmask": (i32, [vp, vp]),
            "sdm_debug_temb_row": (i32, [vp, i32, i32, vp, vp, i32]),
            "sdm_conv_num_cfgs": (i32, [i32, i32]),
            "sdm_bench_conv": (f32, [vp] + [i32] * 11),
            "sdm_bench_attn": (f32, [vp] + [i32] * 7),
            "sdm_bench_gemm_p3": (f32, [vp, C.c_long, i32, i32, i32, i32]),
            "sdm_op_groupnorm": (i32, [vp, vp, vp, i32, i32, i32, i32, i32, i32, vp, vp, f32, i32, vp]),
            "sdm_op_layernorm": (i32, [vp, vp, i32, C.c_long, i32, vp, vp, f32, vp]),
            "sdm_op_attention": (i32, [vp, vp, i32, vp, i32, vp, i32, vp, i32, i32, i32, i32, i32, vp, i32]),
            "sdm_op_attention_split": (i32, [vp, vp, vp, vp, vp, i32, i32, i32, i32, vp]),
            "sdm_op_attention_split_ex": (i32, [vp, vp, vp, vp, vp, vp, i32, i32, i32, i32, i32, vp, vp]),
            "sdm_debug_attn_plan": (i32, [i32] * 10 + [C.c_char_p, i32, C.POINTER(i32)]),
            "sdm_op_resize_aa": (i32, [vp, vp, i32, i32, i32, vp, i32, i32]),
            "sdm_op_mask_bias": (i32, [vp, vp, i32, i32, i32, vp]),
            "sdm_set_option": (i32, [C.c_char_p, i32]),
            "sdm_get_option": (i32, [C.c_char_p, C.POINTER(i32)]),
            "sdm_reset_options": (None, []),
            "sdm_option_name": (C.c_char_p, [i32]),
            "sdm_option_help": (C.c_char_p, [i32]),
            "sdm_kernel_counts": (i32, [C.c_char_p, i32]),
            "sdm_kernel_counts_reset": (None, []),
        }
        for name in EXPORTS:
            fn = getattr(cdll, name)
            fn.restype, fn.argtypes = sig[name]
            setattr(self, name, fn)

    def set_option(self, name, value):
        if self.sdm_set_option(name.encode(), int(value)) != 0:
            raise KeyError(f"unknown engine option {name!r}; known: {', '.join(self.options())}")

    def get_option(self, name):
        v = C.c_int(0)
        if self.sdm_get_option(name.encode(), C.byref(v)) != 0:
            raise KeyError(name)
        return v.value

    def options(self):
        out, i = {}, 0
        while True:
            n = self.sdm_option_name(i)
            if n is None:
                return out
            out[n.decode()] = self.sdm_option_help(i).decode()
            i += 1

    def reset_options(self):
        self.sdm_reset_options()

    def attn_plan(self, B, heads, Lq, Lk, cus, D=64, prec=2, out_f32=True, has_bias=False, has_tiles=False):
        buf, ns = C.create_string_buffer(64), C.c_int(0)
        if self.sdm_debug_attn_plan(B, heads, Lq, Lk, D, prec, int(out_f32), int(has_bias), int(has_tiles), cus, buf, 64, C.byref(ns)) != 0:
            raise ValueError(f"sdm_debug_attn_plan: unsupported attention B={B} heads={heads} Lq={Lq} Lk={Lk} D={D} prec={prec}")
        return buf.value.decode(), ns.value

    def kernel_counts(self, reset=False):
        n = self.sdm_kernel_counts(None, 0)
        buf = C.create_string_buffer(n + 1)
        self.sdm_kernel_counts(buf, n + 1)
        out = {}
        for item in buf.value.decode().split(";"):
            if item:
                k, v = item.rsplit("=", 1)
                out[k] = int(v)
        if reset:
            self.sdm_kernel_counts_reset()
        return out
# ... 621 lines not shown
        out = np.zeros(cout, np.float32)
        co = None if coords is None else np.ascontiguousarray(np.asarray(coords, np.float32).reshape(4))
        self._check(self.lib.sdm_debug_temb_row(self.h, index, int(is_trans), co.ctypes.data_as(C.c_void_p) if co is not None else None,
                                                out.ctypes.data_as(C.c_void_p), cout), "sdm_debug_temb_row")
        return torch.from_numpy(out)

    def bench_conv(self, N, H, W, Cin, Cout, ntaps=9, stride=1, in_f32=0, tile_cfg=-1, ablate=0, iters=10):
        return float(self.lib.sdm_bench_conv(self.h, N, H, W, Cin, Cout, ntaps, stride, in_f32, tile_cfg, ablate, iters))

    def bench_gemm_p3(self, M, K, O, epi=0, res=False, iters=10):
        return float(self.lib.sdm_bench_gemm_p3(self.h, M, K, O, epi | (256 if res else 0), iters))

    def bench_attn(self, B, heads, Lq, Lk, qt=1, ablate=0, iters=10):
        return float(self.lib.sdm_bench_attn(self.h, B, heads, Lq, Lk, qt, ablate, iters))

    def op_groupnorm(self, x0, gamma, beta, eps, silu, groups=32, x1=None):
        N, H, W_, C0 = x0.shape
        C1 = x1.shape[-1] if x1 is not None else 0
        out = torch.empty(N, H, W_, C0 + C1, dtype=torch.float16, device=x0.device)
        self._check(self.lib.sdm_op_groupnorm(self.h, _ptr(x0), _ptr(x1), C0, C1, int(x0.dtype == torch.float32), N, H * W_, groups,
                                              _ptr(gamma), _ptr(beta), float(eps), int(silu), _ptr(out)), "sdm_op_groupnorm")
        return out

    def op_layernorm(self, x, gamma, beta, eps):
        rows, Cc = x.numel() // x.shape[-1], x.shape[-1]
        out = torch.empty(x.shape, dtype=torch.float16, device=x.device)
        self._check(self.lib.sdm_op_layernorm(self.h, _ptr(x), int(x.dtype == torch.float32), rows, Cc, _ptr(gamma), _ptr(beta),
                                              float(eps), _ptr(out)), "sdm_op_layernorm")
        return out

    def op_attention(self, q, k, v, heads, bias=None):
        B, Lq, HD = q.shape
        Lk = k.shape[1]
        D = HD // heads
        out = torch.empty(B, Lq, HD, dtype=torch.float16, device=q.device)
        self._check(self.lib.sdm_op_attention(self.h, _ptr(q), q.stride(1), _ptr(k), k.stride(1), _ptr(v), v.stride(1), _ptr(bias), B,
                                              heads, Lq, Lk, D, _ptr(out), HD), "sdm_op_attention")
        return out

    def op_attention_split(self, q, k, v, heads, bias=None, out_p3=0, tiles=None, planes=False):
        B, Lq, HD = q.shape
        Lk = k.shape[1]
        qf, kf, vf = q.float().contiguous(), k.float().contiguous(), v.float().contiguous()
        out = torch.empty(B, Lq, HD, dtype=torch.float32, device=q.device)
        if not out_p3 and tiles is None:
            self._check(self.lib.sdm_op_attention_split(self.h, _ptr(qf), _ptr(kf), _ptr(vf), _ptr(bias), B, heads, Lq, Lk, _ptr(out)), "sdm_op_attention_split")
            return out
        tl = tiles.to(torch.int32).contiguous() if tiles is not None else None
        raw = torch.zeros(((B * Lq + 31) // 32) * 32 * HD * 3, dtype=torch.uint8, device=q.device) if (planes and out_p3) else None
        self._check(self.lib.sdm_op_attention_split_ex(self.h, _ptr(qf), _ptr(kf), _ptr(vf), _ptr(bias), _ptr(tl), B, heads, Lq, Lk, int(out_p3),
                                                       _ptr(out), _ptr(raw)), "sdm_op_attention_split_ex")
        return (out, raw) if raw is not None else out

    def op_resize_aa(self, planes, Hout, Wout):
        P, Hin, Win = planes.shape
        out = torch.empty(P, Hout, Wout, dtype=torch.float32, device=planes.device)
        self._check(self.lib.sdm_op_resize_aa(self.h, _ptr(planes), P, Hin, Win, _ptr(out), Hout, Wout), "sdm_op_resize_aa")
        return out

    def op_mask_bias(self, plane_bss, level):
        B, S, _ = plane_bss.shape
        lk = (S // 8) >> level
        out = torch.empty(B, lk * lk, dtype=torch.float32, device=plane_bss.device)
        self._check(self.lib.sdm_op_mask_bias(self.h, _ptr(plane_bss), B, S, level, _ptr(out)), "sdm_op_mask_bias")
        return out
```

### include/sdmatte.h

```cpp
#ifndef SDMATTE_H_
#define SDMATTE_H_

#include <stddef.h>
#include <stdint.h>

#ifdef __cplusplus
extern "C" {
#endif

typedef struct sdm_ctx sdm_ctx;

enum sdm_status {
  SDM_OK = 0,
  SDM_ERR_INVALID = -1,
  SDM_ERR_HIP = -2,
  SDM_ERR_STATE = -3,
  SDM_ERR_NOMEM = -4,
  SDM_ERR_NODEVICE = -5,
  SDM_ERR_ARENA = -6
};

enum sdm_ptr_kind { SDM_PTR_HOST = 0, SDM_PTR_DEVICE = 1 };
enum sdm_dtype { SDM_F32 = 0, SDM_F16 = 1, SDM_BF16 = 2 };

// ... 116 lines not shown
int sdm_compose_canvas(sdm_ctx* ctx, const float* fg_bhw3, const float* alpha_bhw, int B, int H, int W, float roi_threshold, int canvas_h, int canvas_w,
                       int fill_pct, int valign, int bg_mode, const float* bg_rgb3, const float* bg_image, int bg_batch, float shadow_opacity,
                       float shadow_sigma, int shadow_dy, int shadow_dx, float* out, int out_channels, int32_t* place_out, int ptr_kind, void* stream);

int64_t sdm_resident_bytes(sdm_ctx* ctx);
int64_t sdm_weight_bytes(sdm_ctx* ctx);
int sdm_release_memory(sdm_ctx* ctx);

int sdm_set_option(const char* name, int value);
int sdm_get_option(const char* name, int* value);
void sdm_reset_options(void);
const char* sdm_option_name(int i);
const char* sdm_option_help(int i);
int sdm_kernel_counts(char* buf, int cap);
void sdm_kernel_counts_reset(void);

int sdm_synchronize(sdm_ctx* ctx);

float sdm_last_forward_ms(sdm_ctx* ctx);

int sdm_profile_enable(sdm_ctx* ctx, int on);
int sdm_profile_count(sdm_ctx* ctx);
const char* sdm_profile_dump(sdm_ctx* ctx);
int sdm_profile_get(sdm_ctx* ctx, int i, const char** name, float* ms, int64_t* launches, double* flops, double* bytes);


int sdm_op_conv(sdm_ctx* ctx, const void* in0, const void* in1, int C0, int C1, int in_f32, int N, int Hin, int Win, int up,
                int stride, int pad_mode, int ntaps, const float* w, const float* bias, int O, void* out, int out_f32,
                const void* res, int res_f32, int geglu, float out_scale, int tile_cfg);
int sdm_conv_num_cfgs(int ntaps, int stride);
int sdm_op_conv_ex(sdm_ctx* ctx, const void* in0, const void* in1, int C0, int C1, int in_f32, int N, int Hin, int Win, int up,
                   int stride, int pad_mode, int ntaps, const float* w, const float* bias, int O, void* out, int out_f32,
                   const void* res, int res_f32, int geglu, float out_scale, int tile_cfg, int split, const float* gn_gamma,
                   const float* gn_beta, float gn_eps, int gn_groups, int gn_silu);
float sdm_bench_gemm_p3(sdm_ctx* ctx, long M, int K, int O, int epi_flags, int iters);
int sdm_op_gemm_p3(sdm_ctx* ctx, const float* x, int N, int H, int W, int K, const float* w, const float* bias, int O, int mode, const float* res,
                   const float* ln_gamma, const float* ln_beta, float ln_eps, int lo_cols, void* out, float* stats, int* srows);
int sdm_op_conv_up_stats(sdm_ctx* ctx, const float* x, int N, int H, int W, int C, const float* w, const float* bias, int O, float* out, float* stats,
                         int* srows);
int sdm_debug_set_input_cmask(sdm_ctx* ctx, const unsigned char* mask);
int sdm_debug_run_layer(sdm_ctx* ctx, const char* layer_name, const float* x_nhwc, int N, int H, int W, float* out_nhwc, int Cout);
int sdm_debug_temb_row(sdm_ctx* ctx, int temb_index, int is_trans, const float* coords4, float* out_host, int cout);
float sdm_bench_attn(sdm_ctx* ctx, int B, int heads, int Lq, int Lk, int qt, int ablate, int iters);
float sdm_bench_conv(sdm_ctx* ctx, int N, int H, int W, int Cin, int Cout, int ntaps, int stride, int in_f32, int tile_cfg, int ablate, int iters);
int sdm_op_groupnorm(sdm_ctx* ctx, const void* in0, const void* in1, int C0, int C1, int in_f32, int N, int HW, int groups,
                     const float* gamma, const float* beta, float eps, int silu, void* out_f16);
int sdm_op_layernorm(sdm_ctx* ctx, const void* x, int in_f32, long rows, int C, const float* gamma, const float* beta,
                     float eps, void* out_f16);
int sdm_op_attention(sdm_ctx* ctx, const void* q, int ldq, const void* k, int ldk, const void* v, int ldv, const float* bias,
                     int B, int heads, int Lq, int Lk, int D, void* out, int ldo);
int sdm_op_attention_split(sdm_ctx* ctx, const float* q, const float* k, const float* v, const float* bias, int B, int heads, int Lq, int Lk, float* out);
int sdm_op_attention_split_ex(sdm_ctx* ctx, const float* q, const float* k, const float* v, const float* bias, const int* tiles, int B, int heads, int Lq,
                              int Lk, int out_p3, float* out, void* planes);
int sdm_debug_attn_plan(int B, int heads, int Lq, int Lk, int D, int prec, int out_f32, int has_bias, int has_tiles, int cus, char* kernel, int cap,
                        int* nsplit);
int sdm_op_resize_aa(sdm_ctx* ctx, const float* in, int P, int Hin, int Win, float* out, int Hout, int Wout);
int sdm_op_mask_bias(sdm_ctx* ctx, const float* trimap_plane, int B, int S, int level, float* bias_out);

#ifdef __cplusplus
}
#endif
#endif
```

Baseline: 21.39.

## Share one patch-matrix key/value across heads in UNet cross-attention

Cross-attention K/V are linear in the 3x3 patch matrix of the 4-channel trimap latent (36 values padded to 64). The per-head K|V projection weights are therefore folded into new q_shared and out_shared linears, and every head attends over one shared key/value operand built once per forward by a new cross_patch_planes_kernel. This removes the per-block kv conv and transpose_v launches and cuts the K/V memory traffic, which is why the kernels gain a head stride for K (zero when shared). The cost is precomputed folded weights built on the host, a different numerical path through the folded projections, and a restriction to the fp8-pair plane format with head dim 64.

```diff
diff --git a/comfyui-sdmatte_amd/csrc/k_attn.h b/comfyui-sdmatte_amd/csrc/k_attn.h
--- a/comfyui-sdmatte_amd/csrc/k_attn.h
+++ b/comfyui-sdmatte_amd/csrc/k_attn.h
@@ -5,6 +5,7 @@
 struct AttnParams {
   const half_t* q; long q_bs; int ldq;
   const half_t* k; long k_bs; int ldk;
+  int k_hs;
   const half_t* vt; long vt_bs; long vt_hs; int ldvt;
   const float* bias; long bias_bs;
   half_t* o; long o_bs; int ldo;
@@ -151,7 +152,7 @@
 #pragma unroll
   for (int j = 0; j < 8; ++j) ones[j] = (half_t)1.0f;
 
-  const half_t* kbase = p.k + (size_t)b * p.k_bs + head * 64;
+  const half_t* kbase = p.k + (size_t)b * p.k_bs + head * p.k_hs;
   const half_t* vbase = p.vt + (size_t)b * p.vt_bs + (size_t)head * p.vt_hs;
   const float* bbase = p.bias ? p.bias + (size_t)b * p.bias_bs : nullptr;
   const int ntiles = (p.Lk + 63) / 64;
@@ -499,7 +500,7 @@
 #pragma unroll
   for (int j = 0; j < 8; ++j) ones[j] = (half_t)1.0f;
 
-  const half_t* kbase = p.k + (size_t)b * p.k_bs + head * 64;
+  const half_t* kbase = p.k + (size_t)b * p.k_bs + head * p.k_hs;
   const half_t* vbase = p.vt + (size_t)b * p.vt_bs + (size_t)head * p.vt_hs;
   const float* bbase = p.bias ? p.bias + (size_t)b * p.bias_bs : nullptr;
   const float* bsrc = bbase ? bbase : (const float*)(p.k + (size_t)b * p.k_bs);
@@ -705,7 +706,7 @@
 #pragma unroll
   for (int j = 0; j < 8; ++j) ones[j] = (half_t)1.0f;
 
-  const half_t* kbase = p.k + (size_t)b * p.k_bs + head * 64;
+  const half_t* kbase = p.k + (size_t)b * p.k_bs + head * p.k_hs;
   const half_t* vbase = p.vt + (size_t)b * p.vt_bs + (size_t)head * p.vt_hs;
   const int ntiles = p.Lk / 64;
   const int* tl = (LIST && p.tiles) ? p.tiles + (size_t)b * p.tiles_bs : nullptr;
diff --git a/comfyui-sdmatte_amd/csrc/k_misc.h b/comfyui-sdmatte_amd/csrc/k_misc.h
--- a/comfyui-sdmatte_amd/csrc/k_misc.h
+++ b/comfyui-sdmatte_amd/csrc/k_misc.h
@@ -141,28 +141,83 @@
   }
 }
 
+SDM_DEV_INLINE u32x2 sdm_pair_plane4(const float (&x)[4], f16x4& oh) {
+  float xx[4], xl[4];
+#pragma unroll
+  for (int e = 0; e < 4; ++e) {
+    const float y = fminf(fmaxf(x[e], -57344.0f), 57344.0f);
+    oh[e] = (half_t)y; xx[e] = y; xl[e] = (y - (float)oh[e]) * 2048.0f;
+  }
+  int a = SDM_CVT_PK_BF8(xx[0], xx[1], 0, false), b = SDM_CVT_PK_BF8(xl[0], xl[1], 0, false);
+  a = SDM_CVT_PK_BF8(xx[2], xx[3], a, true); b = SDM_CVT_PK_BF8(xl[2], xl[3], b, true);
+  u32x2 pr;
+  pr[0] = (unsigned int)a; pr[1] = (unsigned int)b;
+  return pr;
+}
+
 __global__ void split_planes_kernel(const float* __restrict__ x, half_t* __restrict__ hi, half_t* __restrict__ lo, long n, float mult, int mode) {
   const long i4 = ((long)blockIdx.x * blockDim.x + threadIdx.x) * 4;
   if (i4 >= n) return;
+  float y[4];
+#pragma unroll
+  for (int e = 0; e < 4; ++e) y[e] = (i4 + e < n) ? x[i4 + e] * mult : 0.0f;
   f16x4 oh, ol;
-  float xx[4], xl[4];
-#pragma unroll
-  for (int e = 0; e < 4; ++e) {
-    float y = (i4 + e < n) ? x[i4 + e] * mult : 0.0f;
-    if (mode == 3) y = fminf(fmaxf(y, -57344.0f), 57344.0f);
-    oh[e] = (half_t)y;
-    ol[e] = (half_t)(y - (float)oh[e]);
-    xx[e] = y; xl[e] = (y - (float)oh[e]) * 2048.0f;
-  }
-  *(f16x4*)(hi + i4) = oh;
   if (mode == 3) {
-    int a = SDM_CVT_PK_BF8(xx[0], xx[1], 0, false), b = SDM_CVT_PK_BF8(xl[0], xl[1], 0, false);
-    a = SDM_CVT_PK_BF8(xx[2], xx[3], a, true); b = SDM_CVT_PK_BF8(xl[2], xl[3], b, true);
-    u32x2 pr;
-    pr[0] = (unsigned int)a; pr[1] = (unsigned int)b;
+    const u32x2 pr = sdm_pair_plane4(y, oh);
+    *(f16x4*)(hi + i4) = oh;
     *(u32x2*)(lo + i4) = pr;
   } else {
+#pragma unroll
+    for (int e = 0; e < 4; ++e) { oh[e] = (half_t)y[e]; ol[e] = (half_t)(y[e] - (float)oh[e]); }
+    *(f16x4*)(hi + i4) = oh;
     *(f16x4*)(lo + i4) = ol;
+  }
+}
+
+SDM_DEV_INLINE float cross_patch_value(const float* __restrict__ uin, int H, int W, long b, int key, int j) {
+  if (j >= 36 || key >= H * W) return 0.0f;
+  const int ci = j / 9, tap = j - ci * 9, ky = tap / 3, kx = tap - ky * 3;
+  const int y = key / W + ky - 1, x = key - (key / W) * W + kx - 1;
+  if ((unsigned)y >= (unsigned)H || (unsigned)x >= (unsigned)W) return 0.0f;
+  return uin[((size_t)b * H * W + (size_t)y * W + x) * 16 + 4 + ci];
+}
+__global__ void __launch_bounds__(256) cross_patch_planes_kernel(const float* __restrict__ uin, int B, int H, int W, half_t* __restrict__ k_hi,
+                                                                 half_t* __restrict__ k_pair, half_t* __restrict__ vt, int ldvt) {
+  const long t = (long)blockIdx.x * blockDim.x + threadIdx.x;
+  const int Lk = H * W;
+  if (blockIdx.y == 0) {
+    if (t >= (long)B * Lk * 8) return;
+    const int oct = (int)(t & 7), key = (int)((t >> 3) % Lk);
+    const long b = (t >> 3) / Lk;
+    u32x4 hv, pv;
+#pragma unroll
+    for (int g = 0; g < 2; ++g) {
+      float x[4];
+#pragma unroll
+      for (int e = 0; e < 4; ++e) x[e] = cross_patch_value(uin, H, W, b, key, oct * 8 + g * 4 + e);
+      f16x4 oh;
+      const u32x2 pr = sdm_pair_plane4(x, oh);
+      const u32x2 hw = __builtin_bit_cast(u32x2, oh);
+      hv[2 * g] = hw[0]; hv[2 * g + 1] = hw[1]; pv[2 * g] = pr[0]; pv[2 * g + 1] = pr[1];
+    }
+    const size_t o = ((size_t)b * Lk + key) * 64 + oct * 8;
+    *(u32x4*)(k_hi + o) = hv;
+    *(u32x4*)(k_pair + o) = pv;
+  } else {
+    const int cpr = ldvt / 8;
+    if (t >= (long)B * 64 * cpr) return;
+    const int chunk = (int)(t % cpr), j = (int)((t / cpr) & 63);
+    const long b = t / cpr / 64;
+    u32x4 hv;
+#pragma unroll
+    for (int g = 0; g < 2; ++g) {
+      f16x4 oh;
+#pragma unroll
+      for (int e = 0; e < 4; ++e) oh[e] = (half_t)fminf(fmaxf(cross_patch_value(uin, H, W, b, chunk * 8 + g * 4 + e, j), -57344.0f), 57344.0f);
+      const u32x2 hw = __builtin_bit_cast(u32x2, oh);
+      hv[2 * g] = hw[0]; hv[2 * g + 1] = hw[1];
+    }
+    *(u32x4*)(vt + ((size_t)b * 64 + j) * ldvt + chunk * 8) = hv;
   }
 }
 
diff --git a/comfyui-sdmatte_amd/csrc/sdm_engine.cpp b/comfyui-sdmatte_amd/csrc/sdm_engine.cpp
--- a/comfyui-sdmatte_amd/csrc/sdm_engine.cpp
+++ b/comfyui-sdmatte_amd/csrc/sdm_engine.cpp
@@ -23,6 +23,7 @@
 #include <mutex>
 #include <shared_mutex>
 #include <string>
+#include <thread>
 #include <unordered_map>
 #include <vector>
 
@@ -108,6 +109,7 @@
   {"attn_pp", 1, 1, "split-precision d=64 attention with fp32 output as a ping-pong of the block's wave halves (attn_d64_pp_kernel, 256 query rows per block): 0 off, 1 on, 2 on without the static priority of the younger half, 3 on with per-segment priority flips"},
   {"attn_pp_min_blocks", 128, 128, "attn_pp: launches with fewer 256-row blocks than this keep the 4-wave pipelines (0 in tests: the ping-pong kernel at any size)"},
   {"attn_ksplit", 0, 0, "key split of the d=64 split-precision attention: 0 by launch size (blocks that do not fill the chip's block slots a whole number of times), 1 off, 2 / 4 forced, 3 forced on the ping-pong kernel (ignored elsewhere: those launches run unsplit)"},
+  {"cross_shared", 1, 1, "cross-attention on ONE key / value operand per forward, the patch matrix of the trimap latent (cross_patch_planes_kernel), with the K|V fold moved into q_shared / out_shared: 0 = every block's own kv_folded conv + transpose.  Read per forward"},
   {"precise_mask", -1, -1, "stages in split precision (-1 = the config's own mask; per-stage attribution experiments; read at sdm_create)"},
 #ifdef SDM_EMU
   {"emu_arena_extra", 0, 0, "emulator build only, self-test of the arena check: the launch pass of a stand-alone op allocates one block its sizing pass did not"},
@@ -530,11 +532,13 @@
   float w_scale = 1.0f;
   std::vector<int64_t> shape;
   size_t host_off = 0;
+  bool host_too = false;
   bool loaded = false;
 };
 struct ResB { int norm1 = -1, conv1 = -1, norm2 = -1, conv2 = -1, sc = -1, temb = -1, cin = 0, cout = 0; };
 struct VaeAttnB { int gn = -1, qkv = -1, out = -1, C = 0; };
-struct TfB { int gn, proj_in, ln1, qkv1, o1, ln2, q2, kv2, o2, ln3, ff1, ff2, proj_out, C, heads; size_t k_hoff, v_hoff; };
+struct TfB { int gn, proj_in, ln1, qkv1, o1, ln2, q2, kv2, o2, ln3, ff1, ff2, proj_out, C, heads; size_t k_hoff, v_hoff;
+             int q2s, o2s; size_t q_hoff, o_hoff, ob_hoff; };
 struct TembL { size_t w_hoff = 0, b_hoff = 0, cb_hoff = 0; int cout = 0, cout_pad = 0; float* table = nullptr; };
 
 struct T {
@@ -692,6 +696,13 @@
     e->slots[key] = s;
     e->slot_order.push_back(key);
   }
+  size_t keep_host(const std::string& key) {
+    Slot& s = e->slots[key];
+    size_t n = 1; for (auto d : s.shape) n *= (size_t)d;
+    s.host_too = true; s.host_off = e->hostblob.size();
+    e->hostblob.resize(e->hostblob.size() + n, 0.0f);
+    return s.host_off;
+  }
   int conv_named(const std::string& p, int ntaps, int I, int O, bool bias = true, int ci_off = 0, int Ipad = 0, int up = 0) {
     int id = conv(p, ntaps, Ipad ? Ipad : I, O, 0, up);
     if (ntaps == 9) slot(p + ".weight", SLOT_CONV_W, id, {O, I, 3, 3}, 0, ci_off);
@@ -762,6 +773,11 @@
     slot(b + ".attn2.to_k.weight", SLOT_HOST, -1, {C, ctx}); t.k_hoff = e->slots[b + ".attn2.to_k.weight"].host_off;
     slot(b + ".attn2.to_v.weight", SLOT_HOST, -1, {C, ctx}); t.v_hoff = e->slots[b + ".attn2.to_v.weight"].host_off;
     t.o2 = conv_named(b + ".attn2.to_out.0", 1, C, C);
+    t.q2s = conv(b + ".attn2.q_shared", 1, C, C);
+    t.o2s = conv(b + ".attn2.out_shared", 1, C, C);
+    t.q_hoff = keep_host(b + ".attn2.to_q.weight");
+    t.o_hoff = keep_host(b + ".attn2.to_out.0.weight");
+    t.ob_hoff = keep_host(b + ".attn2.to_out.0.bias");
     t.ff1 = conv(b + ".ff.net.0.proj", 1, C, 8 * C, 1);
     slot(b + ".ff.net.0.proj.weight", SLOT_CONV_W, t.ff1, {8 * C, C});
     slot(b + ".ff.net.0.proj.bias", SLOT_CONV_B, t.ff1, {8 * C});
@@ -1184,6 +1200,7 @@
   } else {
     prof_begin(e, "conv", flops, bytes);
   }
+  if (L.ntaps == 9 && (L.I <= 16 || L.O <= 16)) count_kernel("conv3x3_thin");
   int rc = 0;
   if (L.ntaps == 1 && p.stats && p.N > 1) p.rows_per_img = p.Hout * p.Wout;
   if (cm_prop) {
@@ -1308,7 +1325,7 @@
   return 0;
 }
 
-struct AttnPrec { int prec = 0; long q_lo = 0, k_lo = 0, v_lo = 0; int out_f32 = 0; int out_p3 = 0; bool has_bias = false, has_tiles = false; };
+struct AttnPrec { int prec = 0; long q_lo = 0, k_lo = 0, v_lo = 0; int out_f32 = 0; int out_p3 = 0; bool has_bias = false, has_tiles = false; bool shared_kv = false; };
 
 enum AttnKernel { kAttnPP, kAttnPPBias, kAttnPPTiles, kAttnPipe8, kAttnPipe4, kAttnP3W8, kAttnP3W4, kAttnP1W8, kAttnP1W4, kAttnP2W8, kAttnP2W4,
                   kAttnF16W8, kAttnF16W4, kAttnD512 };
@@ -1405,7 +1422,9 @@
   const AttnKernelInfo& ki = kAttnKernels[pl.kernel];
   const int nsplit = pl.nsplit;
   const int ldvt = rup(Lk, 64);
-  T vt = talloc(e, (ap.prec ? 2 : 1) * B, heads, D, ldvt, 0);
+  if (ap.shared_kv && (D != 64 || pl.pv_split || ldk != 64)) SDM_FAIL(e, SDM_ERR_INVALID, "attention: a shared key / value operand is [key][64] at head dim 64, without the residual terms of P.V");
+  T vt;
+  if (!ap.shared_kv) vt = talloc(e, (ap.prec ? 2 : 1) * B, heads, D, ldvt, 0);
   const int ntiles64 = sdm_cdiv(Lk, 64);
   T tl_own, part_o, part_ml;
   if (pl.own_list) tl_own = talloc(e, B, 1, 1, ntiles64 + 1, 1);
@@ -1419,19 +1438,22 @@
       tiles = (const int*)tl_own.p;
     }
     if (!pl.walk_tiles) tiles = nullptr;
-    const long vt_hs = (long)D * ldvt, vt_bs = (long)heads * vt_hs;
-    prof_begin(e, "transpose_v", 0, (double)B * Lk * heads * D * 4);
-    SDM_LAUNCH(transpose_v_kernel, dim3(ldvt / 64, heads * (D / 64), B), dim3(256), 0, e->stream, v, (long)Lk * ldv, ldv, (half_t*)vt.p, vt_bs,
-               vt_hs, ldvt, Lk, D);
-    if (pl.pv_split)
-      SDM_LAUNCH(transpose_v_kernel, dim3(ldvt / 64, heads * (D / 64), B), dim3(256), 0, e->stream, v + ap.v_lo, (long)Lk * ldv, ldv,
-                 (half_t*)vt.p + (size_t)B * vt_bs, vt_bs, vt_hs, ldvt, Lk, D);
-    prof_end(e);
+    const long vt_hs = ap.shared_kv ? 0 : (long)D * ldvt, vt_bs = ap.shared_kv ? (long)D * ldvt : (long)heads * vt_hs;
+    if (!ap.shared_kv) {
+      prof_begin(e, "transpose_v", 0, (double)B * Lk * heads * D * 4);
+      count_kernel("transpose_v");
+      SDM_LAUNCH(transpose_v_kernel, dim3(ldvt / 64, heads * (D / 64), B), dim3(256), 0, e->stream, v, (long)Lk * ldv, ldv, (half_t*)vt.p, vt_bs,
+                 vt_hs, ldvt, Lk, D);
+      if (pl.pv_split)
+        SDM_LAUNCH(transpose_v_kernel, dim3(ldvt / 64, heads * (D / 64), B), dim3(256), 0, e->stream, v + ap.v_lo, (long)Lk * ldv, ldv,
+                   (half_t*)vt.p + (size_t)B * vt_bs, vt_bs, vt_hs, ldvt, Lk, D);
+      prof_end(e);
+    }
     AttnParams p;
     memset(&p, 0, sizeof(p));
     p.q = q; p.q_bs = (long)Lq * ldq; p.ldq = ldq;
-    p.k = k; p.k_bs = (long)Lk * ldk; p.ldk = ldk;
-    p.vt = (const half_t*)vt.p; p.vt_bs = vt_bs; p.vt_hs = vt_hs; p.ldvt = ldvt;
+    p.k = k; p.k_bs = (long)Lk * ldk; p.ldk = ldk; p.k_hs = ap.shared_kv ? 0 : 64;
+    p.vt = ap.shared_kv ? v : (const half_t*)vt.p; p.vt_bs = vt_bs; p.vt_hs = vt_hs; p.ldvt = ldvt;
     p.bias = bias_l2; p.bias_bs = Lk;
     p.tiles = tiles; p.tiles_bs = ntiles64 + 1;
     p.o = (half_t*)out; p.o_bs = (long)Lq * ldo; p.ldo = ldo; p.o_f32 = ap.out_f32;
@@ -1487,7 +1509,7 @@
   }
   if (nsplit > 1) { tfree(e, part_ml); tfree(e, part_o); }
   if (pl.own_list) tfree(e, tl_own);
-  tfree(e, vt);
+  if (!ap.shared_kv) tfree(e, vt);
   return 0;
 }
 
@@ -1656,15 +1678,78 @@
   return 0;
 }
 
-static int transformer(sdm_ctx* e, const TfB& t, const T& x, const T& uin, bool masked, const float* bias, const int* tiles, T* out) {
+static int unet_attn_plane_fmt(const sdm_ctx* e) { return (e->cfg.precise_mask & SDM_PRECISE_UNET_ATTN) ? (attn_f8_enabled() ? 3 : 2) : 0; }
+
+struct CrossPlanes { bool on = false; T k, vt; };
+static int cross_planes_build(sdm_ctx* e, const T& uin, CrossPlanes* cp) {
+  cp->on = opt("cross_shared") != 0 && unet_attn_plane_fmt(e) == 3 && uin.f32 == 1 && uin.C == 16;
+  if (!cp->on) return 0;
+  const int B = uin.N, Lk = uin.H * uin.W, ldvt = rup(Lk, 64);
+  cp->k = talloc(e, 2 * B, 1, Lk, 64, 0);
+  cp->vt = talloc(e, B, 1, 64, ldvt, 0);
+  if (e->dry) return 0;
+  prof_begin(e, "cross_patch_planes", 0, (double)B * Lk * (16.0 + 64 * 6));
+  count_kernel("cross_patch_planes");
+  const long nthr = std::max((long)B * Lk * 8, (long)B * 64 * (ldvt / 8));
+  SDM_LAUNCH(cross_patch_planes_kernel, dim3((unsigned)((nthr + 255) / 256), 2, 1), dim3(256), 0, e->stream, (const float*)uin.p, B, uin.H, uin.W,
+             (half_t*)cp->k.p, (half_t*)cp->k.p + (size_t)B * Lk * 64, (half_t*)cp->vt.p, ldvt);
+  prof_end(e);
+  return 0;
+}
+static void cross_planes_free(sdm_ctx* e, CrossPlanes* cp) {
+  if (!cp->on) return;
+  tfree(e, cp->vt); tfree(e, cp->k);
+}
+
+static bool transformer_p3(sdm_ctx* e, const TfB& t, int pf) {
+  bool p3 = e->cfg.stream_f32 == 1 && pf == 3 && t.C % 32 == 0;
+  for (int l : {t.proj_in, t.qkv1, t.o1, t.q2, t.o2, t.q2s, t.o2s, t.ff1, t.ff2, t.proj_out}) p3 = p3 && p3_ok(e, e->convs[l]);
+  return p3;
+}
+
+static int cross_attention(sdm_ctx* e, const TfB& t, T& n, const T& uin, const CrossPlanes& cp, int pf, bool p3, bool p3a, const T* res, T* out) {
+  const int C = t.C, N = n.N, H = n.H, W = n.W, L = H * W, L0 = uin.H * uin.W, sf = e->cfg.stream_f32;
+  const int pa = pf ? 1 : 0;
+  const bool need_vlo = pf == 2 && opt("attn_pv_split") != 0;
+  T q2, kv, ao;
+  TRY(linear(e, cp.on ? t.q2s : t.q2, n, &q2, C, pf));
+  tfree(e, n);
+  if (!cp.on) TRY(conv_simple(e, t.kv2, uin, &kv, 2 * C, pf, 1, 0, 0, nullptr, 1.0f, false, need_vlo ? -1 : C));
+  ao = talloc(e, N, H, W, C, p3a ? kFmtP3 : e->act_f32);
+  {
+    AttnPrec ap; ap.prec = pa ? pf - 1 : 0; ap.out_f32 = p3a ? 1 : ao.f32; ap.out_p3 = p3a ? 1 : 0;
+    ap.q_lo = (long)q2.rows() * q2.C;
+    if (cp.on) {
+      const half_t* kk = (const half_t*)cp.k.p;
+      ap.shared_kv = true; ap.k_lo = (long)N * L0 * 64;
+      TRY(op_attention_raw(e, (const half_t*)q2.p, C, kk, 64, (const half_t*)cp.vt.p, 64, nullptr, N, t.heads, L, L0, 64, ao.p, C, true, nullptr, ap));
+    } else {
+      const half_t* kk = (const half_t*)kv.p;
+      ap.k_lo = ap.v_lo = (long)kv.rows() * kv.C;
+      TRY(op_attention_raw(e, (const half_t*)q2.p, C, kk, 2 * C, kk ? kk + C : nullptr, 2 * C, nullptr, N, t.heads, L, L0, 64, ao.p, C, true, nullptr, ap));
+    }
+  }
+  tfree(e, q2);
+  if (!cp.on) tfree(e, kv);
+  if (p3 && !p3a) {
+    T ap3;
+    TRY(op_to_p3(e, ao, &ap3));
+    tfree(e, ao);
+    ao = ap3;
+  }
+  TRY(linear(e, cp.on ? t.o2s : t.o2, ao, out, C, sf, res));
+  tfree(e, ao);
+  return 0;
+}
+
+static int transformer(sdm_ctx* e, const TfB& t, const T& x, const T& uin, const CrossPlanes& cp, bool masked, const float* bias, const int* tiles, T* out) {
   const int sf = e->cfg.stream_f32;
-  const int C = t.C, L = x.H * x.W, L0 = uin.H * uin.W;
-  T hn, h, n, qkv, ao, h2, q2, kv, f;
-  const int pa = (e->cfg.precise_mask & SDM_PRECISE_UNET_ATTN) ? 1 : 0;
-  const int pf = pa ? (attn_f8_enabled() ? 3 : 2) : 0;
+  const int C = t.C, L = x.H * x.W;
+  T hn, h, n, qkv, ao, h2, f;
+  const int pf = unet_attn_plane_fmt(e);
+  const int pa = pf ? 1 : 0;
   const bool need_vlo = pf == 2 && opt("attn_pv_split") != 0;
-  bool p3 = sf == 1 && pf == 3 && C % 32 == 0;
-  for (int l : {t.proj_in, t.qkv1, t.o1, t.q2, t.o2, t.ff1, t.ff2, t.proj_out}) p3 = p3 && p3_ok(e, e->convs[l]);
+  const bool p3 = transformer_p3(e, t, pf);
   const int nf = p3 ? kFmtP3 : -1;
   const bool p3a = p3 && L % 32 == 0 && opt("gemm_p3_attn") != 0;
   auto attn_out = [&](T& a) -> int {
@@ -1693,20 +1778,8 @@
   TRY(linear(e, t.o1, ao, &h2, C, sf, &h));
   tfree(e, ao); tfree(e, h);
   TRY(op_ln(e, e->norms[t.ln2], h2, e->cfg.unet_ln_eps, &n, nf));
-  TRY(linear(e, t.q2, n, &q2, C, pf));
-  tfree(e, n);
-  TRY(conv_simple(e, t.kv2, uin, &kv, 2 * C, pf, 1, 0, 0, nullptr, 1.0f, false, need_vlo ? -1 : C));
-  ao = talloc(e, x.N, x.H, x.W, C, p3a ? kFmtP3 : e->act_f32);
-  {
-    const half_t* kk = (const half_t*)kv.p;
-    AttnPrec ap; ap.prec = pa ? pf - 1 : 0; ap.out_f32 = p3a ? 1 : ao.f32; ap.out_p3 = p3a ? 1 : 0;
-    ap.q_lo = (long)q2.rows() * q2.C; ap.k_lo = ap.v_lo = (long)kv.rows() * kv.C;
-    TRY(op_attention_raw(e, (const half_t*)q2.p, C, kk, 2 * C, kk ? kk + C : nullptr, 2 * C, nullptr, x.N, t.heads, L, L0, 64, ao.p, C, true, nullptr, ap));
-  }
-  tfree(e, q2); tfree(e, kv);
-  TRY(attn_out(ao));
-  TRY(linear(e, t.o2, ao, &h, C, sf, &h2));
-  tfree(e, ao); tfree(e, h2);
+  TRY(cross_attention(e, t, n, uin, cp, pf, p3, p3a, &h2, &h));
+  tfree(e, h2);
   TRY(op_ln(e, e->norms[t.ln3], h, e->cfg.unet_ln_eps, &n, nf));
   TRY(linear(e, t.ff1, n, &f, 4 * C, p3 ? kFmtP3 : e->act_f32));
   tfree(e, n);
@@ -1900,6 +1973,8 @@
   const int sf = c.stream_f32;
   std::vector<T> skips;
   T h, t;
+  CrossPlanes cp;
+  TRY(cross_planes_build(e, uin, &cp));
   TRY(conv_simple(e, e->u_conv_in, uin, &h, c.unet_channels[0], sf, 1, 0, 0, nullptr, 1.0f, true));
   skips.push_back(h);
   for (int i = 0; i < 4; ++i) {
@@ -1907,7 +1982,7 @@
       TRY(resblock(e, e->u_down_res[i][j], h, nullptr, eps, &t));
       if (i < 3) {
         T t2;
-        TRY(transformer(e, e->u_down_tf[i][j], t, uin, masked, bias_lvl[i], tiles_lvl[i], &t2));
+        TRY(transformer(e, e->u_down_tf[i][j], t, uin, cp, masked, bias_lvl[i], tiles_lvl[i], &t2));
         tfree(e, t); t = t2;
       }
       h = t;
@@ -1920,7 +1995,7 @@
     }
   }
   TRY(resblock(e, e->u_mid0, h, nullptr, eps, &t)); h = t;
-  TRY(transformer(e, e->u_midtf, h, uin, masked, bias_lvl[3], tiles_lvl[3], &t)); tfree(e, h); h = t;
+  TRY(transformer(e, e->u_midtf, h, uin, cp, masked, bias_lvl[3], tiles_lvl[3], &t)); tfree(e, h); h = t;
   TRY(resblock(e, e->u_mid1, h, nullptr, eps, &t)); tfree(e, h); h = t;
   for (int i = 0; i < 4; ++i) {
     for (size_t j = 0; j < e->u_up_res[i].size(); ++j) {
@@ -1928,7 +2003,7 @@
       TRY(resblock(e, e->u_up_res[i][j], h, &s, eps, &t));
       tfree(e, h); tfree(e, s); h = t;
       if (i > 0) {
-        TRY(transformer(e, e->u_up_tf[i][j], h, uin, masked, bias_lvl[3 - i], tiles_lvl[3 - i], &t));
+        TRY(transformer(e, e->u_up_tf[i][j], h, uin, cp, masked, bias_lvl[3 - i], tiles_lvl[3 - i], &t));
         tfree(e, h); h = t;
       }
     }
@@ -1937,6 +2012,7 @@
   *out = talloc(e, h.N, h.H, h.W, 16, e->act_f32);
   { ConvArgs a; a.out = out; a.out_scale = 1.0f / c.vae_scaling_factor; TRY(gn_conv(e, e->norms[e->u_norm_out], e->convs[e->u_conv_out], h, nullptr, 1, eps, a)); }
   tfree(e, h);
+  cross_planes_free(e, &cp);
   return 0;
 }
 
@@ -2391,6 +2467,10 @@
     SDM_CHECK_DEV(e, dev_memcpy_h2d(e->stage, src, n * 4, e->stream));
     dsrc = (float*)e->stage;
 #endif
+    if (s.host_too) {
+      float* dst = e->hostblob.data() + s.host_off;
+      for (size_t i = 0; i < n; ++i) dst[i] = to_f32(host_ptr, dtype, i);
+    }
     if (s.kind == SLOT_CONV_W) {
       pack_layer_weight(e, e->convs[s.layer], dsrc, (int)s.shape[0], (int)s.shape[1], s.ci_off, s.co_off, s.w_scale);
     } else if (s.kind == SLOT_CONV_B) {
@@ -2410,6 +2490,72 @@
   return 1;
 }
 
+struct CrossFold { std::vector<float> wf, bf, wq, wo, bo; };
+static void fold_cross_block(const sdm_ctx* e, const TfB& t, const std::vector<double>& wa, const std::vector<double>& ba, CrossFold& f) {
+  const int ctx = e->cfg.cross_attention_dim, C = t.C;
+  const float* H = e->hostblob.data();
+  std::vector<double> wfd((size_t)2 * C * 36), bfd((size_t)2 * C);
+  for (int o = 0; o < 2 * C; ++o) {
+    const float* wrow = H + (o < C ? t.k_hoff + (size_t)o * ctx : t.v_hoff + (size_t)(o - C) * ctx);
+    double b = 0.0;
+    for (int m = 0; m < ctx; ++m) b += (double)wrow[m] * ba[m];
+    bfd[o] = b;
+    for (int j = 0; j < 36; ++j) {
+      const double* wj = wa.data() + (size_t)j * ctx;
+      double acc = 0.0;
+      for (int m = 0; m < ctx; ++m) acc += (double)wrow[m] * wj[m];
+      wfd[(size_t)o * 36 + j] = acc;
+    }
+  }
+  f.wf.resize(wfd.size()); f.bf.resize(bfd.size());
+  for (size_t i = 0; i < wfd.size(); ++i) f.wf[i] = (float)wfd[i];
+  for (size_t i = 0; i < bfd.size(); ++i) f.bf[i] = (float)bfd[i];
+  const float* Wq = H + t.q_hoff;
+  const float* Wo = H + t.o_hoff;
+  const double s = (double)(0.125f * SDM_LOG2E);
+  f.wq.assign((size_t)C * C, 0.f); f.wo.assign((size_t)C * C, 0.f); f.bo.assign((size_t)C, 0.f);
+  std::vector<double> acc((size_t)C);
+  for (int h = 0; h < t.heads; ++h)
+    for (int j = 0; j < 36; ++j) {
+      std::fill(acc.begin(), acc.end(), 0.0);
+      for (int d = 0; d < 64; ++d) {
+        const double a = wfd[(size_t)(h * 64 + d) * 36 + j];
+        const float* row = Wq + (size_t)(h * 64 + d) * C;
+        for (int c = 0; c < C; ++c) acc[c] += a * (double)row[c];
+      }
+      float* dst = f.wq.data() + (size_t)(h * 64 + j) * C;
+      for (int c = 0; c < C; ++c) dst[c] = (float)(s * acc[c]);
+    }
+  for (int c = 0; c < C; ++c) {
+    const float* row = Wo + (size_t)c * C;
+    double b = (double)H[t.ob_hoff + c];
+    for (int hd = 0; hd < C; ++hd) b += (double)row[hd] * bfd[(size_t)C + hd];
+    f.bo[c] = (float)b;
+    for (int h = 0; h < t.heads; ++h) {
+      double a36[36] = {0.0};
+      for (int d = 0; d < 64; ++d) {
+        const double w = (double)row[h * 64 + d];
+        const double* v = wfd.data() + (size_t)(C + h * 64 + d) * 36;
+        for (int j = 0; j < 36; ++j) a36[j] += w * v[j];
+      }
+      for (int j = 0; j < 36; ++j) f.wo[(size_t)c * C + h * 64 + j] = (float)a36[j];
+    }
+  }
+}
+static int upload_folded(sdm_ctx* e, ConvL& L, const std::vector<float>& w, int O, int I, int ci_off, const std::vector<float>* bias) {
+  if (ensure_buf(e, &e->stage, &e->stage_bytes, std::max(w.size() * 4, (size_t)1 << 20)) != 0) return SDM_ERR_NOMEM;
+  SDM_CHECK_DEV(e, dev_memset(L.w, 0, L.w_bytes(), e->stream));
+  if (L.w_lo) SDM_CHECK_DEV(e, dev_memset(L.w_lo, 0, L.w_bytes(), e->stream));
+  SDM_CHECK_DEV(e, dev_memcpy_h2d(e->stage, w.data(), w.size() * 4, e->stream));
+  pack_layer_weight(e, L, (const float*)e->stage, O, I, ci_off, 0, 1.0f);
+  SDM_CHECK_DEV(e, dev_sync(e->stream));
+  if (bias) {
+    SDM_CHECK_DEV(e, dev_memcpy_h2d(e->stage, bias->data(), bias->size() * 4, e->stream));
+    pack_layer_bias(e, L, (const float*)e->stage, O, 0);
+    SDM_CHECK_DEV(e, dev_sync(e->stream));
+  }
+  return 0;
+}
 static int fold_cross_kv(sdm_ctx* e) {
   const sdm_config& c = e->cfg;
   const int ctx = c.cross_attention_dim;
@@ -2423,32 +2569,24 @@
   for (auto& v : e->u_down_tf) for (auto& t : v) blocks.push_back(&t);
   blocks.push_back(&e->u_midtf);
   for (auto& v : e->u_up_tf) for (auto& t : v) blocks.push_back(&t);
-  std::vector<float> wf, bf;
-  for (const TfB* t : blocks) {
+  std::vector<CrossFold> folds(blocks.size());
+  {
+    const unsigned hw = std::thread::hardware_concurrency();
+    const size_t nthr = std::max<size_t>(1, std::min<size_t>(std::min<size_t>(hw ? hw : 1, 8), blocks.size()));
+    std::atomic<size_t> next{0};
+    auto work = [&]() { for (size_t i; (i = next.fetch_add(1)) < blocks.size();) fold_cross_block(e, *blocks[i], wa, ba, folds[i]); };
+    std::vector<std::thread> pool;
+    for (size_t i = 1; i < nthr; ++i) pool.emplace_back(work);
+    work();
+    for (auto& th : pool) th.join();
+  }
+  for (size_t i = 0; i < blocks.size(); ++i) {
+    const TfB* t = blocks[i];
     const int C = t->C;
-    ConvL& L = e->convs[t->kv2];
-    wf.assign((size_t)2 * C * 36, 0.f); bf.assign((size_t)2 * C, 0.f);
-    for (int o = 0; o < 2 * C; ++o) {
-      const float* wrow = H + (o < C ? t->k_hoff + (size_t)o * ctx : t->v_hoff + (size_t)(o - C) * ctx);
-      double b = 0.0;
-      for (int m = 0; m < ctx; ++m) b += (double)wrow[m] * ba[m];
-      bf[o] = (float)b;
-      for (int j = 0; j < 36; ++j) {
-        const double* wj = wa.data() + (size_t)j * ctx;
-        double acc = 0.0;
-        for (int m = 0; m < ctx; ++m) acc += (double)wrow[m] * wj[m];
-        wf[(size_t)o * 36 + j] = (float)acc;
-      }
-    }
-    if (ensure_buf(e, &e->stage, &e->stage_bytes, std::max(wf.size() * 4, (size_t)1 << 20)) != 0) return SDM_ERR_NOMEM;
-    SDM_CHECK_DEV(e, dev_memset(L.w, 0, L.w_bytes(), e->stream));
-    if (L.w_lo) SDM_CHECK_DEV(e, dev_memset(L.w_lo, 0, L.w_bytes(), e->stream));
-    SDM_CHECK_DEV(e, dev_memcpy_h2d(e->stage, wf.data(), wf.size() * 4, e->stream));
-    pack_layer_weight(e, L, (const float*)e->stage, 2 * C, 4, 4, 0, 1.0f);
-    SDM_CHECK_DEV(e, dev_sync(e->stream));
-    SDM_CHECK_DEV(e, dev_memcpy_h2d(e->stage, bf.data(), bf.size() * 4, e->stream));
-    pack_layer_bias(e, L, (const float*)e->stage, 2 * C, 0);
-    SDM_CHECK_DEV(e, dev_sync(e->stream));
+    TRY(upload_folded(e, e->convs[t->kv2], folds[i].wf, 2 * C, 4, 4, &folds[i].bf));
+    TRY(upload_folded(e, e->convs[t->q2s], folds[i].wq, C, C, 0, nullptr));
+    TRY(upload_folded(e, e->convs[t->o2s], folds[i].wo, C, C, 0, &folds[i].bo));
+    folds[i] = CrossFold();
   }
   return 0;
 }
diff --git a/comfyui-sdmatte_amd/csrc/sdm_hooks.h b/comfyui-sdmatte_amd/csrc/sdm_hooks.h
--- a/comfyui-sdmatte_amd/csrc/sdm_hooks.h
+++ b/comfyui-sdmatte_amd/csrc/sdm_hooks.h
@@ -380,6 +380,7 @@
   AttnParams p;
   memset(&p, 0, sizeof(p));
   p.q = (const half_t*)q.p; p.q_bs = (long)Lq * C; p.ldq = C; p.k = (const half_t*)k.p; p.k_bs = (long)Lk * C; p.ldk = C;
+  p.k_hs = 64;
   p.vt = (const half_t*)vt.p; p.vt_hs = (long)64 * ldvt; p.vt_bs = heads * p.vt_hs; p.ldvt = ldvt; p.o = (half_t*)o.p; p.o_bs = (long)Lq * C; p.ldo = C;
   p.Lq = Lq; p.Lk = Lk; p.scale_log2e = 0.125f * SDM_LOG2E; p.ablate = ablate;
   if (prec) { p.q_lo = (long)B * Lq * C; p.k_lo = (long)B * Lk * C; p.vt_lo = (long)B * p.vt_bs; p.o_f32 = 1; }
@@ -499,6 +500,69 @@
   });
 }
 
+int sdm_op_cross_patch_planes(sdm_ctx* e, const float* uin, int B, int H, int W, void* k_hi, void* k_pair, void* vt) {
+  if (e) dev_use(e->device);
+  if (!e || !uin || !k_hi || !k_pair || !vt || B < 1 || H < 1 || W < 1) return SDM_ERR_INVALID;
+  const int Lk = H * W, ldvt = rup(Lk, 64);
+  const long nthr = std::max((long)B * Lk * 8, (long)B * 64 * (ldvt / 8));
+  count_kernel("cross_patch_planes");
+  SDM_LAUNCH(cross_patch_planes_kernel, dim3((unsigned)((nthr + 255) / 256), 2, 1), dim3(256), 0, e->stream, uin, B, H, W, (half_t*)k_hi, (half_t*)k_pair, (half_t*)vt, ldvt);
+  SDM_CHECK_DEV(e, dev_sync(e->stream));
+  return 0;
+}
+
+int sdm_op_attention_shared(sdm_ctx* e, const float* q, const float* ks, const float* vs, int B, int heads, int Lq, int Lk, int q_prescaled, float* out) {
+  if (e) dev_use(e->device);
+  if (!e || !q || !ks || !vs || !out) return SDM_ERR_INVALID;
+  if (!attn_f8_enabled() || opt("attn_pv_split")) SDM_FAIL(e, SDM_ERR_INVALID, "sdm_op_attention_shared: the fp8-pair plane format only");
+  const int C = heads * 64, ldvt = rup(Lk, 64);
+  return run_two_pass(e, [&]() -> int {
+    T qp = talloc(e, B, 1, Lq, C, 3), kp = talloc(e, B, 1, Lk, 64, 3), vp = talloc(e, B, 1, Lk, 64, 2), vt = talloc(e, B, 1, 64, ldvt, 0);
+    const long nq = (long)B * Lq * C, nk = (long)B * Lk * 64;
+    if (!e->dry) {
+      SDM_LAUNCH(split_planes_kernel, dim3((unsigned)((nq / 4 + 255) / 256)), dim3(256), 0, e->stream, q, (half_t*)qp.p, (half_t*)qp.p + nq, nq,
+                 q_prescaled ? 1.0f : 0.125f * SDM_LOG2E, 3);
+      SDM_LAUNCH(split_planes_kernel, dim3((unsigned)((nk / 4 + 255) / 256)), dim3(256), 0, e->stream, ks, (half_t*)kp.p, (half_t*)kp.p + nk, nk, 1.0f, 3);
+      SDM_LAUNCH(split_planes_kernel, dim3((unsigned)((nk / 4 + 255) / 256)), dim3(256), 0, e->stream, vs, (half_t*)vp.p, (half_t*)vp.p + nk, nk, 1.0f, 2);
+      SDM_LAUNCH(transpose_v_kernel, dim3(ldvt / 64, 1, B), dim3(256), 0, e->stream, (const half_t*)vp.p, (long)Lk * 64, 64, (half_t*)vt.p, (long)64 * ldvt,
+                 (long)64 * ldvt, ldvt, Lk, 64);
+    }
+    AttnPrec ap; ap.prec = 2; ap.q_lo = nq; ap.k_lo = nk; ap.out_f32 = 1; ap.shared_kv = true;
+    TRY(op_attention_raw(e, (const half_t*)qp.p, C, (const half_t*)kp.p, 64, (const half_t*)vt.p, 64, nullptr, B, heads, Lq, Lk, 64, (void*)out, C, true, nullptr, ap));
+    tfree(e, vt); tfree(e, vp); tfree(e, kp); tfree(e, qp);
+    return 0;
+  });
+}
+
+int sdm_debug_cross_attention(sdm_ctx* e, const char* block, const float* x, int B, int H, int W, const float* uin, int h, int w, float* out) {
+  if (e) dev_use(e->device);
+  if (!e || !block || !x || !uin || !out) return SDM_ERR_INVALID;
+  if (!e->finalized) SDM_FAIL(e, SDM_ERR_STATE, "weights not finalised");
+  if (!e->act_f32 || e->cfg.stream_f32 != 1) SDM_FAIL(e, SDM_ERR_INVALID, "sdm_debug_cross_attention: fp32 activations and stream expected");
+  std::vector<const TfB*> blocks;
+  for (auto& v : e->u_down_tf) for (auto& t : v) blocks.push_back(&t);
+  blocks.push_back(&e->u_midtf);
+  for (auto& v : e->u_up_tf) for (auto& t : v) blocks.push_back(&t);
+  const TfB* tb = nullptr;
+  for (const TfB* t : blocks) if (e->convs[t->q2].name == std::string(block) + ".transformer_blocks.0.attn2.to_q") tb = t;
+  if (!tb) SDM_FAIL(e, SDM_ERR_INVALID, "no transformer block named %s", block);
+  const int C = tb->C;
+  return run_two_pass(e, [&]() -> int {
+    const int pf = unet_attn_plane_fmt(e);
+    const bool p3 = transformer_p3(e, *tb, pf), p3a = p3 && (H * W) % 32 == 0 && opt("gemm_p3_attn") != 0;
+    const T tu = view(uin, B, h, w, 16, 1), tx = view(x, B, H, W, C, 1);
+    CrossPlanes cp;
+    TRY(cross_planes_build(e, tu, &cp));
+    T n = tx, o;
+    if (p3) TRY(op_to_p3(e, tx, &n));
+    TRY(cross_attention(e, *tb, n, tu, cp, pf, p3, p3a, nullptr, &o));
+    if (!e->dry) SDM_CHECK_DEV(e, dev_memcpy_d2d(out, o.p, (size_t)B * H * W * C * 4, e->stream));
+    tfree(e, o);
+    cross_planes_free(e, &cp);
+    return 0;
+  });
+}
+
 int sdm_debug_attn_plan(int B, int heads, int Lq, int Lk, int D, int prec, int out_f32, int has_bias, int has_tiles, int cus, char* kernel, int cap,
                         int* nsplit) {
   if (B < 1 || heads < 1 || Lq < 1 || Lk < 1 || cus < 1 || prec < 0 || prec > 2 || !(D == 64 || (D == 512 && heads == 1 && !prec))) return SDM_ERR_INVALID;
diff --git a/comfyui-sdmatte_amd/engine.py b/comfyui-sdmatte_amd/engine.py
--- a/comfyui-sdmatte_amd/engine.py
+++ b/comfyui-sdmatte_amd/engine.py
@@ -74,7 +74,7 @@
     "sdm_make_trimap", "sdm_clean_mask", "sdm_apply_matte_mask", "sdm_subject_roi", "sdm_apply_matte_roi", "sdm_subject_boxes", "sdm_apply_matte_boxes", "sdm_estimate_foreground", "sdm_refine_alpha_guided", "sdm_compose_canvas",
     "sdm_synchronize", "sdm_release_memory", "sdm_resident_bytes", "sdm_weight_bytes", "sdm_last_forward_ms", "sdm_profile_enable", "sdm_profile_count", "sdm_profile_get", "sdm_profile_dump",
     "sdm_op_conv", "sdm_op_conv_ex", "sdm_op_conv_up_stats", "sdm_op_gemm_p3", "sdm_debug_run_layer", "sdm_debug_set_input_cmask", "sdm_debug_temb_row", "sdm_conv_num_cfgs", "sdm_bench_conv", "sdm_bench_attn", "sdm_bench_gemm_p3", "sdm_op_groupnorm", "sdm_op_layernorm", "sdm_op_attention", "sdm_op_attention_split", "sdm_op_attention_split_ex", "sdm_debug_attn_plan", "sdm_op_resize_aa",
-    "sdm_op_mask_bias",
+    "sdm_op_mask_bias", "sdm_op_cross_patch_planes", "sdm_op_attention_shared", "sdm_debug_cross_attention",
     "sdm_set_option", "sdm_get_option", "sdm_reset_options", "sdm_option_name", "sdm_option_help", "sdm_kernel_counts", "sdm_kernel_counts_reset",
 ]
 
@@ -145,6 +145,9 @@
             "sdm_debug_attn_plan": (i32, [i32] * 10 + [C.c_char_p, i32, C.POINTER(i32)]),
             "sdm_op_resize_aa": (i32, [vp, vp, i32, i32, i32, vp, i32, i32]),
             "sdm_op_mask_bias": (i32, [vp, vp, i32, i32, i32, vp]),
+            "sdm_op_cross_patch_planes": (i32, [vp, vp, i32, i32, i32, vp, vp, vp]),
+            "sdm_op_attention_shared": (i32, [vp, vp, vp, vp, i32, i32, i32, i32, i32, vp]),
+            "sdm_debug_cross_attention": (i32, [vp, C.c_char_p, vp, i32, i32, i32, vp, i32, i32, vp]),
             "sdm_set_option": (i32, [C.c_char_p, i32]),
             "sdm_get_option": (i32, [C.c_char_p, C.POINTER(i32)]),
             "sdm_reset_options": (None, []),
@@ -872,6 +875,32 @@
                                                        _ptr(out), _ptr(raw)), "sdm_op_attention_split_ex")
         return (out, raw) if raw is not None else out
 
+    def op_cross_patch_planes(self, uin):
+        B, H, W_, _ = uin.shape
+        L = H * W_
+        ldvt = (L + 63) // 64 * 64
+        x = uin.float().contiguous()
+        k_hi = torch.full((B, L, 64), 7.0, dtype=torch.float16, device=x.device)
+        k_pair = torch.full((B, L, 64, 2), 7, dtype=torch.uint8, device=x.device)
+        vt = torch.full((B, 64, ldvt), 7.0, dtype=torch.float16, device=x.device)
+        self._check(self.lib.sdm_op_cross_patch_planes(self.h, _ptr(x), B, H, W_, _ptr(k_hi), _ptr(k_pair), _ptr(vt)), "sdm_op_cross_patch_planes")
+        return k_hi, k_pair, vt
+
+    def op_attention_shared(self, q, ks, vs, heads, q_prescaled=False):
+        B, Lq, HD = q.shape
+        Lk = ks.shape[1]
+        qf, kf, vf = q.float().contiguous(), ks.float().contiguous(), vs.float().contiguous()
+        out = torch.empty(B, Lq, HD, dtype=torch.float32, device=q.device)
+        self._check(self.lib.sdm_op_attention_shared(self.h, _ptr(qf), _ptr(kf), _ptr(vf), B, heads, Lq, Lk, int(q_prescaled), _ptr(out)), "sdm_op_attention_shared")
+        return out
+
+    def debug_cross_attention(self, block, x_nhwc, uin):
+        B, H, W_, Cc = x_nhwc.shape
+        x, u = x_nhwc.float().contiguous(), uin.float().contiguous()
+        out = torch.empty(B, H, W_, Cc, dtype=torch.float32, device=x.device)
+        self._check(self.lib.sdm_debug_cross_attention(self.h, block.encode(), _ptr(x), B, H, W_, _ptr(u), u.shape[1], u.shape[2], _ptr(out)), "sdm_debug_cross_attention")
+        return out
+
     def op_resize_aa(self, planes, Hout, Wout):
         P, Hin, Win = planes.shape
         out = torch.empty(P, Hout, Wout, dtype=torch.float32, device=planes.device)
diff --git a/include/sdmatte.h b/include/sdmatte.h
--- a/include/sdmatte.h
+++ b/include/sdmatte.h
@@ -192,6 +192,9 @@
 int sdm_op_attention_split(sdm_ctx* ctx, const float* q, const float* k, const float* v, const float* bias, int B, int heads, int Lq, int Lk, float* out);
 int sdm_op_attention_split_ex(sdm_ctx* ctx, const float* q, const float* k, const float* v, const float* bias, const int* tiles, int B, int heads, int Lq,
                               int Lk, int out_p3, float* out, void* planes);
+int sdm_op_cross_patch_planes(sdm_ctx* ctx, const float* uin, int B, int H, int W, void* k_hi, void* k_pair, void* vt);
+int sdm_op_attention_shared(sdm_ctx* ctx, const float* q, const float* ks, const float* vs, int B, int heads, int Lq, int Lk, int q_prescaled, float* out);
+int sdm_debug_cross_attention(sdm_ctx* ctx, const char* block, const float* x, int B, int H, int W, const float* uin, int h, int w, float* out);
 int sdm_debug_attn_plan(int B, int heads, int Lq, int Lk, int D, int prec, int out_f32, int has_bias, int has_tiles, int cus, char* kernel, int cap,
                         int* nsplit);
 int sdm_op_resize_aa(sdm_ctx* ctx, const float* in, int P, int Hin, int Win, float* out, int Hout, int Wout);
```

New measurement: 21.88 (median of 6 runs). 2.3% higher.
